# liruiw/GA-DDPG

Measured on AMD Instinct MI355X. Metric: DDPG grad-steps/sec (B=256, N=1024 pts), higher is better.
Workload: dtype f32 (3xbf16-split products, f32 accumulate)

## Files before the change

ga-ddpg_amd/csrc/gemm.hip:

```cpp
#include "gemm_common.hpp"
#include <mutex>
#include <string.h>

GemmOptions g_opt;

bool split_on(int family) {
    return !g_opt.deterministic && (g_opt.mfma_split == GAD_SPLIT_ALL || (g_opt.mfma_split & family) != 0);
}

bool fits_i32_bytes(long long rows, int pitch_a, int pitch_b, int pitch_c, int pitch_d) {
    int p = pitch_a > pitch_b ? pitch_a : pitch_b;
    p = p > pitch_c ? p : pitch_c;
    p = p > pitch_d ? p : pitch_d;
    return rows * (long long)p * 4 <= (1ll << 31);
}

int gad_deterministic() { return g_opt.deterministic; }

namespace {
struct DetBuf { void* stream; int kind; void* p; size_t bytes; };
std::mutex g_det_mu;
DetBuf g_det_bufs[64];
int g_det_n = 0;
}

void* gad_det_scratch(void* stream, int kind, size_t bytes) {
    std::lock_guard<std::mutex> lk(g_det_mu);
    DetBuf* b = nullptr;
    for (int i = 0; i < g_det_n; ++i)
        if (g_det_bufs[i].stream == stream && g_det_bufs[i].kind == kind) b = &g_det_bufs[i];
    if (!b) {
        if (g_det_n == 64) { gad_set_error("deterministic mode: more than 64 scratch buffers (streams x kinds)"); return nullptr; }
        b = &g_det_bufs[g_det_n++];
        b->stream = stream; b->kind = kind; b->p = nullptr; b->bytes = 0;
    }
    if (b->bytes >= bytes) return b->p;
    if (b->p) {
        if (hipStreamSynchronize((hipStream_t)stream) != hipSuccess || hipFree(b->p) != hipSuccess) {
            gad_set_error("deterministic mode: releasing a scratch buffer failed");
            b->p = nullptr; b->bytes = 0;
            return nullptr;
        }
        b->p = nullptr; b->bytes = 0;
    }
    size_t want = bytes + bytes / 4;
    want = (want + 4095) & ~(size_t)4095;
    if (hipMalloc(&b->p, want) != hipSuccess) {
        (void)hipGetLastError();
        gad_set_error("deterministic mode: cannot allocate %zu bytes of scratch", want);
        b->p = nullptr;
        return nullptr;
    }
    b->bytes = want;
    return b->p;
}

static void det_scratch_release() {
    std::lock_guard<std::mutex> lk(g_det_mu);
    for (int i = 0; i < g_det_n; ++i)
        if (g_det_bufs[i].p) (void)hipFree(g_det_bufs[i].p);
    g_det_n = 0;
}

template <typename T>
__global__ __launch_bounds__(256) void ordered_reduce_kernel(const T* __restrict__ slots, long long slot_stride, int nslots,
                                                             long long ncols, double* __restrict__ out) {
    const long long c = (long long)blockIdx.x * 256 + threadIdx.x;
    if (c >= ncols) return;
    const T* p = slots + c;
    double s = 0.0;
    for (int i = 0; i < nslots; ++i) s += (double)p[(size_t)i * slot_stride];
    atomic_add_f64(out + c, s);
}

template <typename T>
__global__ __launch_bounds__(256) void ordered_reduce_tree_kernel(const T* __restrict__ slots, long long slot_stride, int nslots,
                                                                  double* __restrict__ out) {
    __shared__ double red[256];
    const long long c = blockIdx.x;
    double s = 0.0;
    for (int i = threadIdx.x; i < nslots; i += 256) s += (double)slots[(size_t)i * slot_stride + c];
    red[threadIdx.x] = s;
    __syncthreads();
    for (int w = 128; w > 0; w >>= 1) {
        if ((int)threadIdx.x < w) red[threadIdx.x] += red[threadIdx.x + w];
        __syncthreads();
    }
    if (threadIdx.x == 0) atomic_add_f64(out + c, red[0]);
}

template <typename T>
static int ordered_reduce_launch(const T* slots, long long slot_stride, int nslots, long long ncols, double* out, void* stream) {
    if (ncols <= 0 || nslots <= 0) return GAD_OK;
    if (ncols <= 4096 && nslots > 256)
        hipLaunchKernelGGL(ordered_reduce_tree_kernel<T>, dim3((unsigned)ncols), dim3(256), 0, (hipStream_t)stream, slots, slot_stride,
                           nslots, out);
    else
        hipLaunchKernelGGL(ordered_reduce_kernel<T>, dim3(gad_cdiv(ncols, 256)), dim3(256), 0, (hipStream_t)stream, slots, slot_stride,
                           nslots, ncols, out);
    GAD_CHECK_LAUNCH("ordered_reduce");
    return GAD_OK;
}
int gad_ordered_reduce(const float* slots, long long slot_stride, int nslots, long long ncols, double* out, void* stream) {
    return ordered_reduce_launch(slots, slot_stride, nslots, ncols, out, stream);
}
int gad_ordered_reduce(const double* slots, long long slot_stride, int nslots, long long ncols, double* out, void* stream) {
    return ordered_reduce_launch(slots, slot_stride, nslots, ncols, out, stream);
}

constexpr int ANY_LO = -2147483647 - 1, ANY_HI = 2147483647;
static const struct { const char* name; int GemmOptions::*member; int lo, hi, fallback; } k_options[] = {
    {"deterministic", &GemmOptions::deterministic, 0, 0, 1},
    {"mfma_split", &GemmOptions::mfma_split, ANY_LO, ANY_HI, 0},
    {"fwd_stream", &GemmOptions::fwd_stream, ANY_LO, ANY_HI, 0},
    {"fwd_wide", &GemmOptions::fwd_wide, ANY_LO, ANY_HI, 0},
    {"dx_wide", &GemmOptions::dx_wide, ANY_LO, ANY_HI, 0},
    {"dw_wide", &GemmOptions::dw_wide, ANY_LO, ANY_HI, 0},
    {"bwd_fused", &GemmOptions::bwd_fused, ANY_LO, ANY_HI, 0},
    {"bwd_wide", &GemmOptions::bwd_wide, ANY_LO, ANY_HI, 0},
    {"fwd_bn_prologue", &GemmOptions::fwd_bn_prologue, ANY_LO, ANY_HI, 0},
    {"fwd_skinny", &GemmOptions::fwd_skinny, ANY_LO, ANY_HI, 0},
    {"dx_skinny", &GemmOptions::dx_skinny, ANY_LO, ANY_HI, 0},
    {"dx_stream", &GemmOptions::dx_stream, ANY_LO, ANY_HI, 0},
    {"dw_skinny", &GemmOptions::dw_skinny, ANY_LO, ANY_HI, 0},
    {"dw_stream", &GemmOptions::dw_stream, ANY_LO, ANY_HI, 0},
    {"bwd_stream_wgs", &GemmOptions::bwd_stream_wgs, 1, DW_STREAM_SPLITS, DW_STREAM_SPLITS},
    {"fwd_stream_wgs", &GemmOptions::fwd_stream_wgs, 1, 2147483647, 256},
    {"fwd_stream_l1_wgs", &GemmOptions::fwd_stream_l1_wgs, 1, 2147483647, 256},
    {"dw_wide_wgs", &GemmOptions::dw_wide_wgs, 1, 2147483647, 256},
    {"bwd_wide_slab", &GemmOptions::bwd_wide_slab, 1, 2147483647, 4},
    {"skinny_nw", &GemmOptions::skinny_nw, 4, 4, SK_NW},
};

extern "C" int gad_set_option(const char* name, int value) {
    GAD_REQUIRE(name, GAD_ERR_NULL, "set_option: null name");
    for (const auto& o : k_options) {
        if (strcmp(name, o.name)) continue;
        const int v = (value >= o.lo && value <= o.hi) ? value : o.fallback;
        if (o.member == &GemmOptions::deterministic && !v && g_opt.deterministic) det_scratch_release();
        g_opt.*o.member = v;
        return GAD_OK;
    }
    int found = 0;
    gad_geometry_set_option(name, value, &found);
    if (found) return GAD_OK;
    GAD_REQUIRE(false, GAD_ERR_SHAPE, "set_option: unknown option '%s'", name);
    return GAD_OK;
}

int check_input(const gad_gemm_fwd_args& a, const char* who) {
    if (a.mode == 2) {
        GAD_REQUIRE(!g_opt.deterministic, GAD_ERR_UNSUPPORTED, "%s: mode 2 (recomputed 64-channel input) has no deterministic form "
                    "(option \"deterministic\"): store the 64-channel input instead", who);
        GAD_REQUIRE(a.src_xyz && a.row_pt && a.row_grp && a.feat && a.pre_W, GAD_ERR_NULL, "%s: recomputed input needs the gather inputs and pre_W", who);
        GAD_REQUIRE(a.act_c == 0 || a.action, GAD_ERR_NULL, "%s: action", who);
        GAD_REQUIRE(fwd_streamable(a), GAD_ERR_SHAPE, "%s: mode 2 (recomputed 64-channel input) is a streaming-kernel form: SA1 rows, "
                    "Kp = c_in = n_out = 64, rows >= 32768, pre_Kp 8 / 16, scale / shift, relu", who);
        return GAD_OK;
    }
    if (a.mode == 0) {
        GAD_REQUIRE(a.zin && a.c_in % 4 == 0 && a.c_in >= 4 && a.c_in <= VMAX && a.zin_pitch % 4 == 0, GAD_ERR_SHAPE,
                    "%s: ACT input needs 4 <= c_in <= %d, c_in and pitch multiples of 4", who, VMAX);
        for (int i = 0; i < a.n_groups; ++i)
            GAD_REQUIRE(a.zin_off[i] % 4 == 0, GAD_ERR_SHAPE, "%s: zin_off must be a multiple of 4", who);
    } else {
        GAD_REQUIRE(a.src_xyz && a.row_pt && a.row_grp && a.feat, GAD_ERR_NULL, "%s: gather inputs", who);
        GAD_REQUIRE(a.feat_c % 4 == 0 && a.feat_c >= 4, GAD_ERR_SHAPE, "%s: feat_c must be a positive multiple of 4", who);
        GAD_REQUIRE(a.act_c == 0 || a.action, GAD_ERR_NULL, "%s: action", who);
    }
    return GAD_OK;
}

int coef_fallback(gad_dz_src& dz, void* stream) {
    if (!dz.bn_dbeta) return GAD_OK;
    GAD_REQUIRE(dz.coefP && dz.coefQ && dz.coefS && dz.scale && dz.bn_dgamma && dz.bn_mean && dz.bn_istd, GAD_ERR_NULL,
                "BatchNorm-backward block on a route without a prologue needs coefP / Q / S scratch");
    if (int e = gad_bn_bwd_coef(dz.bn_dbeta, dz.bn_dgamma, dz.bn_stride, dz.scale, dz.bn_mean, dz.bn_istd, dz.c, dz.bn_count,
                                const_cast<float*>(dz.coefP), const_cast<float*>(dz.coefQ), const_cast<float*>(dz.coefS), dz.gacc_gamma,
                                dz.gacc_beta, stream)) return e;
    dz.bn_dbeta = nullptr; dz.bn_dgamma = nullptr; dz.gacc_gamma = nullptr; dz.gacc_beta = nullptr;
    return GAD_OK;
}

double* det_stat_slots(int gx, int ncol, void* stream) {
    const size_t n = 2 * (size_t)gx * ncol;
    double* p = static_cast<double*>(gad_det_scratch(stream, GAD_DET_SLOTS, n * sizeof(double)));
    if (p && hipMemsetAsync(p, 0, n * sizeof(double), (hipStream_t)stream) != hipSuccess) {
        gad_set_error("deterministic mode: clearing the statistic slots failed");
        return nullptr;
    }
    return p;
}
int det_stat_reduce(const double* slots, int gx, int ncol, double* sum, double* sq, void* stream) {
    if (int e = gad_ordered_reduce(slots, ncol, gx, ncol, sum, stream)) return e;
    return gad_ordered_reduce(slots + (size_t)gx * ncol, ncol, gx, ncol, sq, stream);
}
```

ga-ddpg_amd/csrc/gemm_common.hpp:

```cpp
#pragma once
#include "common.hpp"
#include <type_traits>

typedef float f32x16 __attribute__((ext_vector_type(16)));

__device__ __forceinline__ __attribute__((used)) int gad_cdiv_dev(int a, int b) { return (a + b - 1) / b; }

#ifndef GAD_STREAM_STORE_AUX
#define GAD_STREAM_STORE_AUX 0
#endif

#define KT 32

__device__ __forceinline__ float4 f4zero() { return make_float4(0.f, 0.f, 0.f, 0.f); }
__device__ __forceinline__ float4 f4sel(bool c, float4 a, float4 b) {
    return make_float4(c ? a.x : b.x, c ? a.y : b.y, c ? a.z : b.z, c ? a.w : b.w);
}
__device__ __forceinline__ float4 ldg4(const float* p) { return *reinterpret_cast<const float4*>(p); }

typedef unsigned gad_u32x4 __attribute__((ext_vector_type(4)));
__device__ __forceinline__ float4 buf_ld4(__amdgpu_buffer_rsrc_t r, int vo, int so) {
    const gad_u32x4 u = __builtin_amdgcn_raw_buffer_load_b128(r, vo, so, 0);
    return make_float4(__uint_as_float(u.x), __uint_as_float(u.y), __uint_as_float(u.z), __uint_as_float(u.w));
}
__device__ __forceinline__ float buf_ld(__amdgpu_buffer_rsrc_t r, int vo, int so) {
    return __uint_as_float(__builtin_amdgcn_raw_buffer_load_b32(r, vo, so, 0));
}
#define GAD_BUF_MAX ((int)0x80000000u)
__device__ __forceinline__ int gad_nbytes(int rows, int row_bytes) { return (int)((unsigned)rows * (unsigned)row_bytes); }

#define VMAX 1024

struct XSrc {
    int mode;
    const float* zin; int zin_pitch; int c_in;
    const float* scale; const float* shift; int relu;
    const float* extra; int ones_col;
    const float* src_xyz; const float* ctr_xyz; const float* feat; int feat_c;
    const float* action; int act_c; int gps;
    const int32_t* row_pt; const int32_t* row_grp;
    int affine;
    const float* pre_W; int pre_Kp;
    gad_bn_fin bn;
};

static XSrc make_xsrc(const gad_gemm_fwd_args& a) {
    XSrc x;
    x.mode = a.mode; x.zin = a.zin; x.zin_pitch = a.zin_pitch; x.c_in = a.c_in;
    x.scale = a.scale; x.shift = a.shift; x.relu = a.relu; x.extra = a.extra; x.ones_col = a.ones_col;
    x.src_xyz = a.src_xyz; x.ctr_xyz = a.ctr_xyz; x.feat = a.feat; x.feat_c = a.feat_c;
    x.action = a.action; x.act_c = a.act_c; x.gps = a.grp_per_sample > 0 ? a.grp_per_sample : 1;
    x.row_pt = a.row_pt; x.row_grp = a.row_grp;
    x.affine = (x.scale && x.shift) ? 1 : 0;
    x.pre_W = a.pre_W; x.pre_Kp = a.pre_Kp;
    x.bn.stat_sum = a.in_stat_sum; x.bn.stat_sq = a.in_stat_sq; x.bn.stat_stride = a.in_stat_stride; x.bn.count = a.in_count;
    x.bn.gamma = a.in_gamma; x.bn.beta = a.in_beta; x.bn.eps = a.in_eps; x.bn.momentum = a.in_momentum;
    x.bn.running_mean = a.in_running_mean; x.bn.running_var = a.in_running_var;
    x.bn.scale = const_cast<float*>(a.scale); x.bn.shift = const_cast<float*>(a.shift); x.bn.mean = a.in_mean; x.bn.istd = a.in_istd;
    return x;
}

template <int NT>
__device__ __forceinline__ void stage_affine(float* sv, float* tv, const XSrc& x, int off, int n) {
    for (int i = threadIdx.x; i < n; i += NT) { sv[i] = x.scale[off + i]; tv[i] = x.shift[off + i]; }
}

#ifdef GAD_X_PHASES
#define GAD_PH_STAMP(t) t = (long long)__builtin_readcyclecounter()
#else
#define GAD_PH_STAMP(t)
#endif
#ifdef GAD_W_PHASES
#define GAD_WPH_DECL long long wph_[6] = {0, 0, 0, 0, 0, 0}; wph_[0] = (long long)wall_clock64()
#define GAD_WPH(i) do { if (wph_[i] == 0) wph_[i] = (long long)wall_clock64(); } while (0)
#define GAD_WPH_STORE(ts)                                                                                                     \
    do {                                                                                                                      \
        unsigned long long* q_ = reinterpret_cast<unsigned long long*>(reinterpret_cast<size_t>(ts) & ~(size_t)7);            \
        const unsigned blk_ = blockIdx.x + gridDim.x * blockIdx.y;                                                            \
        if (q_ && threadIdx.x == 0 && blk_ < 4096) {                                                                          \
            auto c_ = [&](int i) { const long long d_ = wph_[i] ? wph_[i] - wph_[0] : 0; return (unsigned long long)(d_ > 65535 ? 65535 : d_); }; \
            q_[2 * (8192 + blk_)] = (unsigned long long)wph_[0];                                                              \
            q_[2 * (8192 + blk_) + 1] = c_(1) | (c_(2) << 16) | (c_(3) << 32) | (c_(4) << 48);                                \
            q_[2 * (12288 + blk_)] = c_(5);                                                                                    \
        }                                                                                                                     \
    } while (0)
#define GAD_WKL_DECL long long wkl_[4] = {0, 0, 0, 0}; long long wkt_ = 0, wkp_ = 0
#define GAD_WKL(i)                                                                   \
    do {                                                                             \
        wkt_ = (long long)__builtin_readcyclecounter();                              \
        if (i > 0) wkl_[i] += wkt_ - wkp_;                                           \
        wkp_ = wkt_;                                                                 \
    } while (0)
#define GAD_WKL_STORE(ts)                                                                                                     \
    do {                                                                                                                      \
        unsigned long long* q_ = reinterpret_cast<unsigned long long*>(reinterpret_cast<size_t>(ts) & ~(size_t)7);            \
        const unsigned blk_ = blockIdx.x + gridDim.x * blockIdx.y;                                                            \
        if (q_ && (threadIdx.x & 63) == 0 && blk_ < 512) {                                                                    \
            const unsigned e_ = 4096 + 8 * blk_ + (threadIdx.x >> 6);                                                         \
            q_[2 * e_] = ((unsigned long long)wkl_[1] << 32) | (unsigned long long)(wkl_[2] & 0xffffffffu);                   \
            q_[2 * e_ + 1] = (unsigned long long)wkl_[3];                                                                     \
        }                                                                                                                     \
    } while (0)
#else
#define GAD_WPH_DECL
#define GAD_WPH(i)
#define GAD_WPH_STORE(ts)
#define GAD_WKL_DECL
#define GAD_WKL(i)
#define GAD_WKL_STORE(ts)
#endif
struct XRaw { float4 a; float4 s; };

__device__ __forceinline__ int x_bulk(const XSrc& x) { return x.mode == 0 ? x.c_in : x.feat_c; }

template <int XM>
__device__ __forceinline__ XRaw x_raw(const XSrc& x, int r, bool valid, int zoff, int c, bool tail, int pt, int grp_pre = -1) {
    XRaw o;
    o.s = f4zero();
    const int rr = valid ? r : 0;
    if (XM == 0) {
        const int cc = c < x.c_in ? c : x.c_in - 4;
        o.a = ldg4(x.zin + (size_t)rr * x.zin_pitch + zoff + cc);
        if (tail) {
            float e = 0.f;
            if (x.extra) e = x.extra[rr];
            o.s.x = (c + 0 == x.c_in && x.extra) ? e : (c + 0 == x.ones_col ? 1.f : 0.f);
            o.s.y = (c + 1 == x.c_in && x.extra) ? e : (c + 1 == x.ones_col ? 1.f : 0.f);
            o.s.z = (c + 2 == x.c_in && x.extra) ? e : (c + 2 == x.ones_col ? 1.f : 0.f);
            o.s.w = (c + 3 == x.c_in && x.extra) ? e : (c + 3 == x.ones_col ? 1.f : 0.f);
        }
    } else {
        const int cc = c < x.feat_c ? c : x.feat_c - 4;
        o.a = ldg4(x.feat + (size_t)pt * x.feat_c + cc);
        if (tail) {
            const int grp = grp_pre >= 0 ? grp_pre : x.row_grp[rr];
            const float* p = x.src_xyz + (size_t)pt * 3;
            float q0 = p[0], q1 = p[1], q2 = p[2];
            if (x.ctr_xyz) {
                const float* cp = x.ctr_xyz + (size_t)grp * 3;
                q0 = __fsub_rn(q0, cp[0]); q1 = __fsub_rn(q1, cp[1]); q2 = __fsub_rn(q2, cp[2]);
            }
            float a[4] = {0.f, 0.f, 0.f, 0.f};
            const int t0 = c - x.feat_c;
            if (x.action) {
                const float* ap = x.action + (size_t)(grp / x.gps) * x.act_c;
#pragma unroll
                for (int j = 0; j < 4; ++j) {
                    const int ai = t0 + j - 3;
                    const int aic = ai < 0 ? 0 : (ai >= x.act_c ? x.act_c - 1 : ai);
                    const float av = ap[aic];
                    a[j] = (ai >= 0 && ai < x.act_c) ? av : 0.f;
                }
            }
            float* spv = &o.s.x;
#pragma unroll
            for (int j = 0; j < 4; ++j) {
                const int t = t0 + j;
                spv[j] = t == 0 ? q0 : (t == 1 ? q1 : (t == 2 ? q2 : a[j]));
            }
        }
    }
    return o;
}

template <int XM>
__device__ __forceinline__ float4 x_finish(const XSrc& x, const XRaw& raw, bool valid, int c, const float* sv,
                                           const float* tv) {
    const int bulk = XM == 0 ? x.c_in : x.feat_c;
    const bool inside = c < bulk;
    float4 v = raw.a;
    if (XM == 0) {
        const int cc = inside ? c : x.c_in - 4;
        if (x.affine) {
            const float4 s = *reinterpret_cast<const float4*>(sv + cc), t = *reinterpret_cast<const float4*>(tv + cc);
            v.x = fmaf(v.x, s.x, t.x); v.y = fmaf(v.y, s.y, t.y); v.z = fmaf(v.z, s.z, t.z); v.w = fmaf(v.w, s.w, t.w);
        }
        if (x.relu) { v.x = fmaxf(v.x, 0.f); v.y = fmaxf(v.y, 0.f); v.z = fmaxf(v.z, 0.f); v.w = fmaxf(v.w, 0.f); }
    }
    return f4sel(valid, f4sel(inside, v, raw.s), f4zero());
}

__device__ __forceinline__ void stage_vec(float* dst, const float* src, int off, int n, float fill) {
    for (int i = threadIdx.x; i < n; i += 256) dst[i] = src ? src[off + i] : fill;
}

struct DzSrc {
    const float* z; int z_pitch; const float* scale; const float* shift; int relu;
    const float* P; const float* Q; const float* S; const float* row_w;
    int gmode; const float* G; int g_pitch; const int32_t* argmax; const float* dout;
    const int32_t* row_grp; int c;
    int coef;
    int premasked;
    gad_bn_bwd bw;
};

static DzSrc make_dzsrc(const gad_dz_src& d) {
    DzSrc s;
    s.z = d.z; s.z_pitch = d.z_pitch; s.scale = d.scale; s.shift = d.shift; s.relu = d.relu;
    s.P = d.coefP; s.Q = d.coefQ; s.S = d.coefS; s.row_w = d.row_w;
    s.gmode = d.gmode; s.G = d.G; s.g_pitch = d.g_pitch; s.argmax = d.argmax; s.dout = d.dout;
    s.row_grp = d.row_grp; s.c = d.c;
    s.premasked = d.premasked;
    s.bw.dbeta = d.bn_dbeta; s.bw.dgamma = d.bn_dgamma; s.bw.stat_stride = d.bn_stride; s.bw.count = d.bn_count;
    s.bw.mean = d.bn_mean; s.bw.istd = d.bn_istd; s.bw.gacc_gamma = d.gacc_gamma; s.bw.gacc_beta = d.gacc_beta;
    s.bw.accumulate = (d.gacc_gamma || d.gacc_beta) ? 1 : 0;
    s.coef = (d.coefP != nullptr || d.bn_dbeta != nullptr) ? 1 : 0;
    return s;
}

__device__ __forceinline__ void dz_coef(const DzSrc& d, int ch, float& P, float& Q, float& S, bool writer = false) {
    if (d.bw.dbeta) gad_bn_bwd_channel(d.bw, d.scale, ch, writer, P, Q, S);
    else if (d.P) { P = d.P[ch]; Q = d.Q[ch]; S = d.S[ch]; }
    else { P = 1.f; Q = 0.f; S = 0.f; }
}
__device__ __forceinline__ bool first_workgroup() { return blockIdx.x == 0 && blockIdx.y == 0 && blockIdx.z == 0; }

struct DzRaw { float4 z; float4 g; int4 a; };

__device__ __forceinline__ float4 dz_scalar4(const DzSrc& d, int r, bool valid, int off, int n, int nmax) {
    float v[4];
#pragma unroll
    for (int j = 0; j < 4; ++j) {
        const int nn = n + j;
        const bool ok = valid && nn < nmax;
        const int rr = ok ? r : 0;
        const int ch = off + (ok ? nn : 0);
        float z = 0.f;
        if (d.z) z = d.z[(size_t)rr * d.z_pitch + ch];
        float g;
        if (d.gmode == 0) {
            g = d.G[(size_t)rr * d.g_pitch + ch];
        } else {
            const int grp = d.row_grp[rr];
            g = d.argmax[(size_t)grp * d.c + ch] == r ? d.dout[(size_t)grp * d.c + ch] : 0.f;
        }
        if (d.relu && !d.premasked) {
            const float y = d.scale ? fmaf(z, d.scale[ch], d.shift[ch]) : z;
            g = y > 0.f ? g : 0.f;
        }
        if (d.P) {
            const float w = d.row_w ? d.row_w[rr] : 1.f;
            g = d.P[ch] * g - w * fmaf(d.S[ch], z, d.Q[ch]);
        }
        v[j] = ok ? g : 0.f;
    }
    return make_float4(v[0], v[1], v[2], v[3]);
}

template <bool VEC>
__device__ __forceinline__ DzRaw dz_raw(const DzSrc& d, int r, bool valid, int off, int n, int nmax, int grp) {
    DzRaw o;
    o.z = f4zero(); o.a = make_int4(0, 0, 0, 0);
    if (!VEC) { o.g = dz_scalar4(d, r, valid, off, n, nmax); return o; }
    const int rr = valid ? r : 0;
    const int ch = off + (n < nmax ? n : 0);
    if (d.z) o.z = ldg4(d.z + (size_t)rr * d.z_pitch + ch);
    if (d.gmode == 0) {
        o.g = ldg4(d.G + (size_t)rr * d.g_pitch + ch);
    } else {
        o.a = *reinterpret_cast<const int4*>(d.argmax + (size_t)grp * d.c + ch);
        o.g = ldg4(d.dout + (size_t)grp * d.c + ch);
    }
    return o;
}

template <bool VEC, int VM = VMAX>
__device__ __forceinline__ float4 dz_finish(const DzSrc& d, const DzRaw& raw, int r, bool valid, int n, int nmax, float w,
                                            const float* vec) {
    if (!VEC) return raw.g;
    const bool inside = n < nmax;
    const int nn = inside ? n : 0;
    float4 g = raw.g;
    const float4 z = raw.z;
    if (d.gmode != 0) {
        g.x = raw.a.x == r ? g.x : 0.f; g.y = raw.a.y == r ? g.y : 0.f;
        g.z = raw.a.z == r ? g.z : 0.f; g.w = raw.a.w == r ? g.w : 0.f;
    }
    if (d.relu && !d.premasked) {
        float4 y = z;
        if (d.scale) {
            const float4 s = *reinterpret_cast<const float4*>(vec + nn), t = *reinterpret_cast<const float4*>(vec + VM + nn);
            y.x = fmaf(z.x, s.x, t.x); y.y = fmaf(z.y, s.y, t.y); y.z = fmaf(z.z, s.z, t.z); y.w = fmaf(z.w, s.w, t.w);
        }
        g.x = y.x > 0.f ? g.x : 0.f; g.y = y.y > 0.f ? g.y : 0.f;
        g.z = y.z > 0.f ? g.z : 0.f; g.w = y.w > 0.f ? g.w : 0.f;
    }
    if (d.coef) {
        const float4 P = *reinterpret_cast<const float4*>(vec + 2 * VM + nn);
        const float4 Q = *reinterpret_cast<const float4*>(vec + 3 * VM + nn);
        const float4 S = *reinterpret_cast<const float4*>(vec + 4 * VM + nn);
        g.x = P.x * g.x - w * fmaf(S.x, z.x, Q.x); g.y = P.y * g.y - w * fmaf(S.y, z.y, Q.y);
        g.z = P.z * g.z - w * fmaf(S.z, z.z, Q.z); g.w = P.w * g.w - w * fmaf(S.w, z.w, Q.w);
    }
    return f4sel(valid && inside, g, f4zero());
}

template <int VM = VMAX>
__device__ __forceinline__ void stage_dz_vecs(float* vec, const DzSrc& d, int off, int n) {
    if (!d.premasked) {
        stage_vec(vec, d.scale, off, n, 1.f);
        stage_vec(vec + VM, d.shift, off, n, 0.f);
    }
    for (int i = threadIdx.x; i < n; i += 256) {
        float P, Q, S;
        dz_coef(d, off + i, P, Q, S, first_workgroup());
        vec[2 * VM + i] = P; vec[3 * VM + i] = Q; vec[4 * VM + i] = S;
    }
}

static bool dz_vectorizable(const gad_dz_src& d, const int32_t* off, const int32_t* n_out, int ng) {
    bool ok = (d.z == nullptr || d.z_pitch % 4 == 0) && (d.gmode != 0 || d.g_pitch % 4 == 0) && (d.gmode == 0 || d.c % 4 == 0);
    for (int i = 0; i < ng; ++i) ok = ok && off[i] % 4 == 0 && n_out[i] % 4 == 0 && n_out[i] <= VMAX;
    return ok;
}

template <int DIM> struct PitchT { static constexpr int v = DIM + 1; };
template <int DIM> struct PitchD { static constexpr int v = DIM + 4; };

template <int DIM> __device__ __forceinline__ void unit_T(int u, int& i, int& kk) { i = u >> 3; kk = (u & 7) << 2; }
template <int DIM> __device__ __forceinline__ void unit_D(int u, int& kk, int& i) { kk = u / (DIM / 4); i = (u % (DIM / 4)) << 2; }

template <int DIM> __device__ __forceinline__ void store_T(float* t, int i, int kk, float4 v) {
    constexpr int P = PitchT<DIM>::v;
    t[(kk + 0) * P + i] = v.x; t[(kk + 1) * P + i] = v.y; t[(kk + 2) * P + i] = v.z; t[(kk + 3) * P + i] = v.w;
}
template <int DIM> __device__ __forceinline__ void store_D(float* t, int kk, int i, float4 v) {
    constexpr int P = PitchD<DIM>::v;
    *reinterpret_cast<float4*>(t + kk * P + i) = v;
}

template <int TM, int TN, int PA, int PB>
__device__ __forceinline__ void mfma_ktile(const float* __restrict__ As, const float* __restrict__ Bs, int am0,
                                           int bn0, int lane, f32x16 (&acc)[TM][TN]) {
    const int l31 = lane & 31, half = lane >> 5;
    constexpr int CH = 4, NCH = KT / 2 / CH;
    const float* ap = As + half * PA + am0 + l31;
    const float* bp = Bs + half * PB + bn0 + l31;
    float a[2][CH][TM], b[2][CH][TN];
    auto fetch = [&](int c, int buf) {
#pragma unroll
        for (int s = 0; s < CH; ++s) {
#pragma unroll
            for (int tm = 0; tm < TM; ++tm) a[buf][s][tm] = ap[(2 * (c * CH + s)) * PA + tm * 32];
#pragma unroll
            for (int tn = 0; tn < TN; ++tn) b[buf][s][tn] = bp[(2 * (c * CH + s)) * PB + tn * 32];
        }
    };
    fetch(0, 0);
#pragma unroll
    for (int c = 0; c < NCH; ++c) {
        if (c + 1 < NCH) fetch(c + 1, (c + 1) & 1);
        __builtin_amdgcn_sched_barrier(0);
#pragma unroll
        for (int s = 0; s < CH; ++s)
#pragma unroll
            for (int tm = 0; tm < TM; ++tm)
#pragma unroll
                for (int tn = 0; tn < TN; ++tn)
                    acc[tm][tn] = __builtin_amdgcn_mfma_f32_32x32x2f32(a[c & 1][s][tm], b[c & 1][s][tn], acc[tm][tn], 0, 0, 0);
    }
}

__device__ __forceinline__ int acc_row(int v, int half) { return (v & 3) + 8 * (v >> 2) + 4 * half; }

struct PoolEpi {
    unsigned long long* key;
    const int32_t* row_grp;
    const float* gamma;
    int C;
};

__device__ __forceinline__ unsigned pool_ord(float f) {
    const unsigned u = __float_as_uint(f);
    return u ^ ((unsigned)((int)u >> 31) | 0x80000000u);
}

__device__ __forceinline__ void pool_put(unsigned long long* keycol, int g, int C, float v, int row, bool partial) {
    const unsigned long long k = ((unsigned long long)pool_ord(v) << 32) | (unsigned long long)(0xffffffffu - (unsigned)row);
    if (partial) atomicMax(keycol + (size_t)g * C, k);
    else keycol[(size_t)g * C] = k;
}

struct PoolRun { int g; int part; float v; int row; };

template <int NC>
__device__ __forceinline__ void pool_rows(const float* zt, int pitch, int cstride, int i, int e, int row_base, const float (&sgn)[NC],
                                          float (&best)[NC], int (&brow)[NC]) {
    int r = i;
    for (; r + 2 <= e; r += 2) {
        float z0[NC], z1[NC];
#pragma unroll
        for (int c = 0; c < NC; ++c) { z0[c] = zt[r * pitch + c * cstride] * sgn[c]; z1[c] = zt[(r + 1) * pitch + c * cstride] * sgn[c]; }
#pragma unroll
        for (int c = 0; c < NC; ++c) {
            bool t = z0[c] > best[c]; best[c] = t ? z0[c] : best[c]; brow[c] = t ? row_base + r : brow[c];
            t = z1[c] > best[c]; best[c] = t ? z1[c] : best[c]; brow[c] = t ? row_base + r + 1 : brow[c];
        }
    }
    if (r < e) {
#pragma unroll
        for (int c = 0; c < NC; ++c) {
            const float z0 = zt[r * pitch + c * cstride] * sgn[c];
            const bool t = z0 > best[c]; best[c] = t ? z0 : best[c]; brow[c] = t ? row_base + r : brow[c];
        }
    }
}

__device__ __forceinline__ void pool_scan32(const float* zt, int pitch, int gl, int row_base, float sgn, PoolRun& c,
                                            unsigned long long* keycol, int C) {
    const int lane = threadIdx.x & 63;
    const int prev = __shfl_up(gl, 1, 64);
    const bool st = lane == 0 ? gl != c.g : gl != prev;
    const unsigned m = (unsigned)__ballot(st);
    int i = 0;
    while (i < 32) {
        if ((m >> i) & 1u) {
            if (c.g >= 0) pool_put(keycol, c.g, C, c.v, c.row, c.part != 0);
            c.g = __builtin_amdgcn_readlane(gl, i); c.part = 0; c.v = -INFINITY; c.row = row_base + i;
        }
        const unsigned rest = i < 31 ? m >> (i + 1) : 0u;
        const int e = rest ? i + 1 + __builtin_ctz(rest) : 32;
        if (c.g >= 0) {
            const float sg1[1] = {sgn};
            float bv[1] = {c.v};
            int br[1] = {c.row};
            pool_rows<1>(zt, pitch, 0, i, e, row_base, sg1, bv, br);
            c.v = bv[0]; c.row = br[0];
        }
        i = e;
    }
}

template <int NC>
__device__ __forceinline__ void pool_tile64(const float* zt, int pitch, int cstride, int gl, int row0, int n_live,
                                            const float (&sgn)[NC], int wave, int nw, int g_before, int g_after,
                                            unsigned long long* keycol, int C) {
    const int lane = threadIdx.x & 63;
    const int prev = __shfl_up(gl, 1, 64);
    const bool st = (lane == 0 || gl != prev) && lane < n_live;
    unsigned long long m = __ballot(st);
    int k = 0;
    while (m) {
        const int i = __builtin_ctzll(m);
        m &= m - 1;
        const int e = m ? __builtin_ctzll(m) : n_live;
        if ((k++ % nw) != wave) continue;
        const int g = __builtin_amdgcn_readlane(gl, i);
        float best[NC];
        int brow[NC];
#pragma unroll
        for (int c = 0; c < NC; ++c) { best[c] = -INFINITY; brow[c] = row0 + i; }
        pool_rows<NC>(zt, pitch, cstride, i, e, row0, sgn, best, brow);
        const bool partial = (i == 0 && g == g_before) || (e == n_live && g == g_after);
#pragma unroll
        for (int c = 0; c < NC; ++c) pool_put(keycol + c * cstride, g, C, best[c], brow[c], partial);
    }
}

struct Groups {
    int n; int aoff[GAD_MAX_GROUPS]; int woff[GAD_MAX_GROUPS]; int ooff[GAD_MAX_GROUPS]; int nout[GAD_MAX_GROUPS];
};

template <int WM, int WN, int TN, bool STORE = false>
__device__ __forceinline__ void block_column_atomics(float* red, const float (&c0)[TN], const float (&c1)[TN], int lane,
                                                     int wm, int wn, int col0, int col_limit, double* out0,
                                                     double* out1) {
    constexpr int BN = WN * TN * 32;
    __syncthreads();
#pragma unroll
    for (int tn = 0; tn < TN; ++tn) {
        const float s0 = c0[tn] + __shfl_xor(c0[tn], 32, 64);
        const float s1 = c1[tn] + __shfl_xor(c1[tn], 32, 64);
        if (lane < 32) {
            const int cl = wn * TN * 32 + tn * 32 + lane;
            red[wm * BN + cl] = s0;
            red[(WM + wm) * BN + cl] = s1;
        }
    }
    __syncthreads();
    const int tid = threadIdx.x;
    if (tid < BN && col0 + tid < col_limit) {
        float s0 = 0.f, s1 = 0.f;
#pragma unroll
        for (int w = 0; w < WM; ++w) { s0 += red[w * BN + tid]; s1 += red[(WM + w) * BN + tid]; }
        if (STORE) {
            out0[col0 + tid] = (double)s0;
            out1[col0 + tid] = (double)s1;
        } else {
            atomic_add_f64(out0 + col0 + tid, (double)s0);
            atomic_add_f64(out1 + col0 + tid, (double)s1);
        }
    }
}

typedef float f32x2 __attribute__((ext_vector_type(2)));

typedef __bf16 gad_bf16x8 __attribute__((ext_vector_type(8)));
__device__ __forceinline__ unsigned gad_cvt_pk_bf16(float lo, float hi) {
    unsigned r;
    __asm__("v_cvt_pk_bf16_f32 %0, %1, %2" : "=v"(r) : "v"(lo), "v"(hi));
    return r;
}
__device__ __forceinline__ void gad_split2(float a, float b, unsigned& H, unsigned& M, unsigned& L) {
    H = gad_cvt_pk_bf16(a, b);
    const f32x2 r = f32x2{a, b} - f32x2{__uint_as_float(H << 16), __uint_as_float(H & 0xffff0000u)};
    M = gad_cvt_pk_bf16(r.x, r.y);
    const f32x2 q = r - f32x2{__uint_as_float(M << 16), __uint_as_float(M & 0xffff0000u)};
    L = gad_cvt_pk_bf16(q.x, q.y);
}
__device__ __forceinline__ gad_bf16x8 gad_as_bf16x8(gad_u32x4 u) { return *reinterpret_cast<gad_bf16x8*>(&u); }

namespace spw {
constexpr int APL = 64 * 64, BPL = 128 * 64, STAGE = 3 * (APL + BPL);
struct BRegs { gad_u32x4 r[2][3]; };
__device__ __forceinline__ void load_b(BRegs& b, __amdgpu_buffer_rsrc_t rs, const int (&vb)[2], int plane_bytes, int kt) {
#pragma unroll
    for (int u = 0; u < 2; ++u)
#pragma unroll
        for (int p = 0; p < 3; ++p) b.r[u][p] = __builtin_amdgcn_raw_buffer_load_b128(rs, vb[u], p * plane_bytes + kt * 64, 0);
}
__device__ __forceinline__ void store_b(unsigned char* stage, const BRegs& b, int tid) {
    const int row = tid >> 2;
    unsigned char* q = stage + 3 * APL + row * 64 + ((((tid & 3) ^ ((row >> 2) & 3))) << 4);
#pragma unroll
    for (int u = 0; u < 2; ++u)
#pragma unroll
        for (int p = 0; p < 3; ++p) *reinterpret_cast<gad_u32x4*>(q + p * BPL + u * (64 * 64)) = b.r[u][p];
}
__device__ __forceinline__ void store_a4(unsigned char* stage, int row, int tid, float4 v, unsigned sg) {
    unsigned h0, m0, l0, h1, m1, l1;
    gad_split2(__uint_as_float(__float_as_uint(v.x) ^ sg), __uint_as_float(__float_as_uint(v.y) ^ sg), h0, m0, l0);
    gad_split2(__uint_as_float(__float_as_uint(v.z) ^ sg), __uint_as_float(__float_as_uint(v.w) ^ sg), h1, m1, l1);
    unsigned char* q = stage + row * 64 + (((((tid & 7) >> 1) ^ ((row >> 2) & 3))) << 4) + ((tid & 1) << 3);
    *reinterpret_cast<uint2*>(q) = make_uint2(h0, h1);
    *reinterpret_cast<uint2*>(q + APL) = make_uint2(m0, m1);
    *reinterpret_cast<uint2*>(q + 2 * APL) = make_uint2(l0, l1);
}
__device__ __forceinline__ void ktile(const unsigned char* stage, int arow, int brow, int fo, f32x16 (&acc)[2], f32x16 (&an)[2]) {
#pragma unroll
    for (int s = 0; s < 2; ++s) {
        const int off = fo ^ (s << 5);
        const unsigned char* ap = stage + arow + off;
        const unsigned char* bp = stage + 3 * APL + brow + off;
        const gad_u32x4 AH = *reinterpret_cast<const gad_u32x4*>(ap), AM = *reinterpret_cast<const gad_u32x4*>(ap + APL);
        const gad_u32x4 AL = *reinterpret_cast<const gad_u32x4*>(ap + 2 * APL);
        gad_u32x4 BH[2], BM[2], BL[2];
#pragma unroll
        for (int t = 0; t < 2; ++t) {
            BH[t] = *reinterpret_cast<const gad_u32x4*>(bp + t * (32 * 64));
            BM[t] = *reinterpret_cast<const gad_u32x4*>(bp + BPL + t * (32 * 64));
            BL[t] = *reinterpret_cast<const gad_u32x4*>(bp + 2 * BPL + t * (32 * 64));
        }
#define GAD_SPW(A, B)                                                                                                          \
        _Pragma("unroll") for (int t = 0; t < 2; ++t) {                                                                        \
            if (s) an[t] = __builtin_amdgcn_mfma_f32_32x32x16_bf16(gad_as_bf16x8(A), gad_as_bf16x8(B[t]), an[t], 0, 0, 0);     \
            else acc[t] = __builtin_amdgcn_mfma_f32_32x32x16_bf16(gad_as_bf16x8(A), gad_as_bf16x8(B[t]), acc[t], 0, 0, 0);     \
        }
        GAD_SPW(AL, BH) GAD_SPW(AH, BL) GAD_SPW(AM, BM) GAD_SPW(AM, BH) GAD_SPW(AH, BM) GAD_SPW(AH, BH)
#undef GAD_SPW
    }
}
}

#define SK_NW 8
#define SK_CH 6
#define SK_SP 36
#define SK_KCAP (8 * SK_NW * SK_CH * SK_MAXCH)
#define SK_MAXCH 3
#define GAD_GX_CAP 2048
#define DW_STREAM_SPLITS 256

struct GemmOptions {
    int mfma_split = 0;
    int deterministic = 0;
    int fwd_wide = 1, dx_wide = 1, dw_wide = 1;
    int bwd_fused = 1;
    int fwd_bn_prologue = 1;
    int bwd_wide = 0;
    int bwd_wide_slab = 4;
    int dw_wide_wgs = 256;
    int skinny_nw = SK_NW;
    int fwd_skinny = 1, dx_skinny = 1, dx_stream = 1, dw_skinny = 1, dw_stream = 1, fwd_stream = 1;
    int bwd_stream_wgs = DW_STREAM_SPLITS;
    int fwd_stream_wgs = 256;
    int fwd_stream_l1_wgs = 256;
};
extern GemmOptions g_opt;
bool split_on(int family);

#define GAD_LAUNCH_SKINNY(kernel, grid, st, ...)                                                                               \
    do {                                                                                                                       \
        if (g_opt.skinny_nw == 4) hipLaunchKernelGGL(kernel<4>, grid, dim3(64 * 4), 0, st, __VA_ARGS__);                       \
        else hipLaunchKernelGGL(kernel<SK_NW>, grid, dim3(64 * SK_NW), 0, st, __VA_ARGS__);                                    \
    } while (0)

static Groups make_groups(int n, const int32_t* a, const int32_t* w, const int32_t* o, const int32_t* no) {
    Groups g;
    g.n = n;
    for (int i = 0; i < GAD_MAX_GROUPS; ++i) {
        g.aoff[i] = (i < n && a) ? a[i] : 0; g.woff[i] = (i < n && w) ? w[i] : 0;
        g.ooff[i] = (i < n && o) ? o[i] : 0; g.nout[i] = i < n ? no[i] : 0;
    }
    return g;
}

static int max_nout(const Groups& g) { int m = 0; for (int i = 0; i < g.n; ++i) m = g.nout[i] > m ? g.nout[i] : m; return m; }

struct DxEpi {
    int mode; float* gout; int gout_pitch; int k_valid;
    const float* zprev; int zprev_pitch; const float* ps; const float* pt; const float* pm; const float* pi;
    double* dbeta; double* dgamma; int stat_stride; int store_masked;
    float* dfeat; int feat_c; const int32_t* row_pt; const int32_t* row_grp; double* daction; int act_c; int gps;
};

static DxEpi make_dxepi(const gad_gemm_dx_args& a) {
    DxEpi e;
    e.mode = a.epilogue; e.gout = a.gout; e.gout_pitch = a.gout_pitch; e.k_valid = a.k_valid;
    e.zprev = a.zprev; e.zprev_pitch = a.zprev_pitch; e.ps = a.prev_scale; e.pt = a.prev_shift;
    e.pm = a.prev_mean; e.pi = a.prev_istd; e.dbeta = a.prev_dbeta; e.dgamma = a.prev_dgamma;
    e.stat_stride = a.stat_stride;
    e.store_masked = (a.store_masked && a.prev_dbeta) ? 1 : 0;
    e.dfeat = a.dfeat; e.feat_c = a.feat_c; e.row_pt = a.row_pt; e.row_grp = a.row_grp;
    e.daction = a.daction; e.act_c = a.act_c; e.gps = a.grp_per_sample > 0 ? a.grp_per_sample : 1;
    return e;
}

int check_input(const gad_gemm_fwd_args& a, const char* who);
int coef_fallback(gad_dz_src& dz, void* stream);
bool fits_i32_bytes(long long rows, int pitch_a, int pitch_b, int pitch_c, int pitch_d);
double* det_stat_slots(int gx, int ncol, void* stream);
int det_stat_reduce(const double* slots, int gx, int ncol, double* sum, double* sq, void* stream);
bool fwd_streamable(const gad_gemm_fwd_args& a);
bool dx_streamable(const gad_gemm_dx_args& a, bool vec);
int dx_stream_launch(const gad_gemm_dx_args* a, const DzSrc& d, const DxEpi& e, unsigned long long* ts, void* stream);
bool dw_streamable(const gad_gemm_dw_args& a, int k_used);
int dw_reduce_launch(const float* partial, const Groups& gr, int nmax, const int32_t* n_rows_dev, int rows, int splits, int Kp,
                     int k_used, double* gacc, int all_active, hipStream_t st);
```

ga-ddpg_amd/csrc/gemm_dx.hip:

```cpp
#include "gemm_common.hpp"

template <int WM, int WN, int TM, int TN, bool VEC, int VM, bool DET = false>
__global__ __launch_bounds__(256) __attribute__((amdgpu_waves_per_eu(4, 4))) void gemm_dx_kernel(DzSrc d, Groups gr, const int32_t* __restrict__ n_rows_dev,
                                                       int n_rows_static, const float* __restrict__ W, int Kp,
                                                       DxEpi e, unsigned long long* __restrict__ ts) {
    KTimer kt(ts);
    constexpr int BM = WM * TM * 32, BN = WN * TN * 32;
    constexpr int PA = PitchT<BM>::v, PB = PitchD<BN>::v;
    constexpr int UA = BM * 8 / 256, UB = BN * 8 / 256;
    constexpr int OFFB = (KT * PA + 3) & ~3;
    constexpr int TILE = OFFB + KT * PB;
    constexpr int SM = TILE + 3 * BM + (VEC ? 5 * VM : 4);
    static_assert(TILE >= 2 * WM * BN, "reduction scratch must fit in the tile LDS");
    __shared__ __attribute__((aligned(16))) float smem[SM];
    float* As = smem;
    float* Bs = smem + OFFB;
    int32_t* ptS = reinterpret_cast<int32_t*>(smem + TILE);
    int32_t* grS = ptS + BM;
    float* wS = reinterpret_cast<float*>(grS + BM);
    float* vec = wS + BM;

    const int tid = threadIdx.x, lane = tid & 63, wave = tid >> 6;
    const int wm = wave / WN, wn = wave % WN;
    const int g = blockIdx.z;
    const int doff = gr.aoff[g], n_out = gr.nout[g], goff = gr.ooff[g];
    const float* Wg = W + gr.woff[g];
    const int k0out = blockIdx.y * BN;
    if (k0out >= e.k_valid) return;
    const int n_rows = n_rows_dev ? min(*n_rows_dev, n_rows_static) : n_rows_static;
    if ((int)(blockIdx.x * BM) >= n_rows) return;
    const int nk = gad_cdiv_dev(n_out, KT);
    if (VEC) stage_dz_vecs<VM>(vec, d, doff, n_out);
    const bool need_grp = e.mode == 1 || d.gmode != 0;

    float cb[TN], cg[TN];
#pragma unroll
    for (int t = 0; t < TN; ++t) { cb[t] = 0.f; cg[t] = 0.f; }

    for (int row0 = blockIdx.x * BM; row0 < n_rows; row0 += gridDim.x * BM) {
        f32x16 acc[TM][TN];
#pragma unroll
        for (int a = 0; a < TM; ++a)
#pragma unroll
            for (int b = 0; b < TN; ++b)
#pragma unroll
                for (int v = 0; v < 16; ++v) acc[a][b][v] = 0.f;
        if (tid < BM) {
            const int r = row0 + tid;
            const bool ok = r < n_rows;
            wS[tid] = (ok && d.row_w) ? d.row_w[r] : 1.f;
            if (e.mode == 1) ptS[tid] = ok ? e.row_pt[r] : 0;
            if (need_grp) grS[tid] = ok ? (e.mode == 1 ? e.row_grp[r] : d.row_grp[r]) : 0;
        }
        __syncthreads();

        DzRaw ra[UA];
        float4 rb[UB];
        auto load_tile = [&](int kt) {
            const int nb = kt * KT;
#pragma unroll
            for (int it = 0; it < UA; ++it) {
                int i, kk; unit_T<BM>(it * 256 + tid, i, kk);
                const int r = row0 + i;
                ra[it] = dz_raw<VEC>(d, r, r < n_rows, doff, nb + kk, n_out, need_grp ? grS[i] : 0);
            }
#pragma unroll
            for (int it = 0; it < UB; ++it) {
                int kk, j; unit_D<BN>(it * 256 + tid, kk, j);
                const int n = nb + kk, k = k0out + j;
                const bool ok = n < n_out && k < Kp;
                rb[it] = ldg4(Wg + (size_t)(ok ? n : 0) * Kp + (ok ? k : 0));
            }
        };
        auto store_tile = [&](int kt) {
            const int nb = kt * KT;
#pragma unroll
            for (int it = 0; it < UA; ++it) {
                int i, kk; unit_T<BM>(it * 256 + tid, i, kk);
                const int r = row0 + i;
                store_T<BM>(As, i, kk, dz_finish<VEC, VM>(d, ra[it], r, r < n_rows, nb + kk, n_out, wS[i], vec));
            }
#pragma unroll
            for (int it = 0; it < UB; ++it) {
                int kk, j; unit_D<BN>(it * 256 + tid, kk, j);
                const bool ok = (nb + kk) < n_out && (k0out + j) < Kp;
                store_D<BN>(Bs, kk, j, f4sel(ok, rb[it], f4zero()));
            }
        };
        load_tile(0);
        for (int kt = 0; kt < nk; ++kt) {
            store_tile(kt);
            __syncthreads();
            if (kt + 1 < nk) load_tile(kt + 1);
            mfma_ktile<TM, TN, PA, PB>(As, Bs, wm * TM * 32, wn * TN * 32, lane, acc);
            __syncthreads();
        }
        const int l31 = lane & 31, half = lane >> 5;
#pragma unroll
        for (int tn = 0; tn < TN; ++tn) {
            const int k = k0out + wn * TN * 32 + tn * 32 + l31;
            const bool kok = k < e.k_valid;
            float sc = 0.f, sh = 0.f, mu = 0.f, is = 0.f;
            const bool stats = e.dbeta != nullptr && kok;
            if (stats) { sc = e.ps[goff + k]; sh = e.pt[goff + k]; mu = e.pm[goff + k]; is = e.pi[goff + k]; }
            float sb = 0.f, sg = 0.f;
            int run_smp = -1;
            double run_sum = 0.0;
#pragma unroll
            for (int tm = 0; tm < TM; ++tm)
#pragma unroll
                for (int v = 0; v < 16; ++v) {
                    const int il = wm * TM * 32 + tm * 32 + acc_row(v, half);
                    const int r = row0 + il;
                    if (r >= n_rows || !kok) continue;
                    const float gv = acc[tm][tn][v];
                    if (e.mode == 0) {
                        float outv = gv;
                        if (stats) {
                            const float zp = e.zprev[(size_t)r * e.zprev_pitch + goff + k];
                            if (fmaf(zp, sc, sh) > 0.f) { sb += gv; sg = fmaf(gv, (zp - mu) * is, sg); }
                            else if (e.store_masked) outv = 0.f;
                        }
                        e.gout[(size_t)r * e.gout_pitch + goff + k] = outv;
                    } else {
                        if (k < e.feat_c) {
                            if (e.dfeat) atomic_add_f32(e.dfeat + (size_t)ptS[il] * e.feat_c + k, gv);
                        } else if (k >= e.feat_c + 3 && k < e.feat_c + 3 + e.act_c) {
                            if (e.daction) {
                                const int smp = grS[il] / e.gps;
                                if (smp != run_smp) {
                                    if (run_smp >= 0) atomic_add_f64(e.daction + (size_t)run_smp * e.act_c + (k - e.feat_c - 3), run_sum);
                                    run_smp = smp; run_sum = 0.0;
                                }
                                run_sum += (double)gv;
                            }
                        }
                    }
                }
            if (run_smp >= 0) atomic_add_f64(e.daction + (size_t)run_smp * e.act_c + (k - e.feat_c - 3), run_sum);
            cb[tn] += sb; cg[tn] += sg;
        }
        __syncthreads();
    }
    if (e.dbeta) {
        const int rep = DET ? blockIdx.x : blockIdx.x % GAD_STAT_REPLICAS;
        block_column_atomics<WM, WN, TN, DET>(smem, cb, cg, lane, wm, wn, k0out, e.k_valid,
                                              e.dbeta + (size_t)rep * e.stat_stride + goff,
                                              e.dgamma + (size_t)rep * e.stat_stride + goff);
    }
}

template <int GM, int SC, bool SP = false>
__global__ __launch_bounds__(256, 2) void gemm_dx_wide_kernel(DzSrc d, const int32_t* __restrict__ n_rows_dev, int n_rows_static,
                                                              const float* __restrict__ W, int Kp, int n_out, DxEpi e,
                                                              const uint16_t* __restrict__ wsp, int wsp_plane,
                                                              unsigned long long* __restrict__ ts) {
    KTimer kt_(ts);
    constexpr int BM = 64, BN = 128, P = KT + 4, PB = BN + 4, STAGE = SP ? spw::STAGE / 4 : BM * P + KT * PB, VM = 512;
    __shared__ __attribute__((aligned(16))) float smem[2 * STAGE + 3 * VM + BM];
    __shared__ int32_t ptS[BM];
    float* vP = smem + 2 * STAGE;
    float* wS = vP + 3 * VM;
    int32_t* grS = reinterpret_cast<int32_t*>(wS);
    const int tid = threadIdx.x, lane = tid & 63;
    const int wave = __builtin_amdgcn_readfirstlane(tid >> 6);
    const int wm = wave >> 1, wn = wave & 1;
    const int l31 = lane & 31, half = lane >> 5;
    const int k0out = blockIdx.y * BN;
    const int n_rows = n_rows_dev ? min(*n_rows_dev, n_rows_static) : n_rows_static;
    if ((int)(blockIdx.x * BM) >= n_rows) return;
    const int nk = n_out / KT;
    const int gpitch = GM == 0 ? d.g_pitch : d.c;
    const __amdgpu_buffer_rsrc_t zr = __builtin_amdgcn_make_buffer_rsrc(const_cast<float*>(d.z), 0, GAD_BUF_MAX, 0x00020000);
    const __amdgpu_buffer_rsrc_t gr_ = __builtin_amdgcn_make_buffer_rsrc(const_cast<float*>(GM == 0 ? d.G : d.dout), 0, GAD_BUF_MAX, 0x00020000);
    const __amdgpu_buffer_rsrc_t ar = __builtin_amdgcn_make_buffer_rsrc(const_cast<int32_t*>(GM == 0 ? d.row_grp : d.argmax), 0, GAD_BUF_MAX, 0x00020000);
    const __amdgpu_buffer_rsrc_t wr = __builtin_amdgcn_make_buffer_rsrc(const_cast<float*>(W), 0, GAD_BUF_MAX, 0x00020000);
    const int zp_pitch4 = SC ? 0 : e.zprev_pitch * 4, go_pitch4 = SC ? 0 : e.gout_pitch * 4;
    const __amdgpu_buffer_rsrc_t pr = __builtin_amdgcn_make_buffer_rsrc(const_cast<float*>(SC ? W : e.zprev), 0, SC ? 0 : gad_nbytes(n_rows, zp_pitch4), 0x00020000);
    const __amdgpu_buffer_rsrc_t or_ = __builtin_amdgcn_make_buffer_rsrc(SC ? const_cast<float*>(W) : e.gout, 0, SC ? 0 : gad_nbytes(n_rows, go_pitch4), 0x00020000);
    const int c4 = (tid & 7) * 4, ur = tid >> 3;
    const int bk4 = (tid & 31) * 4, bn = tid >> 5;
    int vw[4];
#pragma unroll
    for (int u = 0; u < 4; ++u) vw[u] = ((bn + 8 * u) * Kp + k0out + bk4) * 4;
    const __amdgpu_buffer_rsrc_t ws_ = __builtin_amdgcn_make_buffer_rsrc(const_cast<uint16_t*>(SP ? wsp : reinterpret_cast<const uint16_t*>(W)), 0, GAD_BUF_MAX, 0x00020000);
    int vbs[2];
#pragma unroll
    for (int u = 0; u < 2; ++u) vbs[u] = ((k0out + (tid >> 2) + 64 * u) * n_out + (tid & 3) * 8) * 2;
    unsigned char* const smem_b = reinterpret_cast<unsigned char*>(smem);
    const int sp_fo = ((half ^ ((l31 >> 2) & 3)) << 4);
    for (int i = tid; i < n_out; i += 256) {
        float Pc, Qc, Sc;
        dz_coef(d, i, Pc, Qc, Sc, first_workgroup());
        vP[i] = Pc; vP[VM + i] = Qc; vP[2 * VM + i] = Sc;
    }
    (void)grS;
    float ps[2] = {0.f, 0.f}, pt[2] = {0.f, 0.f}, pm[2] = {0.f, 0.f}, pi[2] = {0.f, 0.f};
#pragma unroll
    for (int t = 0; t < 2; ++t) {
        const int k = k0out + wn * 64 + t * 32 + l31;
        if (!SC) { ps[t] = e.ps[k]; pt[t] = e.pt[k]; pm[t] = e.pm[k]; pi[t] = e.pi[k]; }
    }
    float cb[2] = {0.f, 0.f}, cg[2] = {0.f, 0.f};
    for (int row0 = blockIdx.x * BM; row0 < n_rows; row0 += gridDim.x * BM) {
        f32x16 acc[2];
        f32x16 an[2];
#pragma unroll
        for (int t = 0; t < 2; ++t)
#pragma unroll
            for (int v = 0; v < 16; ++v) { acc[t][v] = 0.f; if (SP) an[t][v] = 0.f; }
        int vz[2], vg[2];
        float wrow[2];
        bool live[2];
#pragma unroll
        for (int u = 0; u < 2; ++u) {
            const int r = row0 + ur + 32 * u;
            live[u] = r < n_rows;
            const int rr = live[u] ? r : max(n_rows - 1, 0);
            wrow[u] = d.row_w ? d.row_w[rr] : 1.f;
            vz[u] = (rr * d.z_pitch + c4) * 4;
            vg[u] = ((GM == 1 ? d.row_grp[rr] : rr) * gpitch + c4) * 4;
        }
        float4 rz[2], rg[2], rb[SP ? 1 : 4];
        gad_u32x4 ra[2];
        spw::BRegs rbs;
        auto load_regs = [&](int kt) {
#pragma unroll
            for (int u = 0; u < 2; ++u) {
                rz[u] = buf_ld4(zr, vz[u], kt * (KT * 4));
                rg[u] = buf_ld4(gr_, vg[u], kt * (KT * 4));
                if (GM == 1) ra[u] = __builtin_amdgcn_raw_buffer_load_b128(ar, vg[u], kt * (KT * 4), 0);
            }
            if (SP) { spw::load_b(rbs, ws_, vbs, wsp_plane * 2, kt); return; }
#pragma unroll
            for (int u = 0; u < (SP ? 1 : 4); ++u) rb[u] = buf_ld4(wr, vw[u], kt * (KT * 4) * Kp);
        };
        auto write_lds = [&](int kt) {
            float* As = smem + (kt & 1) * STAGE;
            float* Bs = As + BM * P;
            const int nb = kt * KT + c4;
            const float4 P4 = *reinterpret_cast<const float4*>(vP + nb), Q4 = *reinterpret_cast<const float4*>(vP + VM + nb);
            const float4 S4 = *reinterpret_cast<const float4*>(vP + 2 * VM + nb);
#pragma unroll
            for (int u = 0; u < 2; ++u) {
                float4 g = rg[u];
                const float4 z = rz[u];
                if (GM == 1) {
                    const unsigned r = row0 + ur + 32 * u;
                    g.x = ra[u].x == r ? g.x : 0.f; g.y = ra[u].y == r ? g.y : 0.f;
                    g.z = ra[u].z == r ? g.z : 0.f; g.w = ra[u].w == r ? g.w : 0.f;
                }
                const float w = wrow[u];
                float4 v;
                v.x = P4.x * g.x - w * fmaf(S4.x, z.x, Q4.x); v.y = P4.y * g.y - w * fmaf(S4.y, z.y, Q4.y);
                v.z = P4.z * g.z - w * fmaf(S4.z, z.z, Q4.z); v.w = P4.w * g.w - w * fmaf(S4.w, z.w, Q4.w);
                if (!live[u]) v = f4zero();
                if (SP) spw::store_a4(smem_b + (kt & 1) * spw::STAGE, ur + 32 * u, tid, v, (ur & 1) ? 0x80000000u : 0u);
                else *reinterpret_cast<float4*>(As + (ur + 32 * u) * P + c4) = v;
            }
            if (SP) { spw::store_b(smem_b + (kt & 1) * spw::STAGE, rbs, tid); return; }
#pragma unroll
            for (int u = 0; u < (SP ? 1 : 4); ++u)
                *reinterpret_cast<float4*>(Bs + (bn + 8 * u) * PB + bk4) = rb[u];
        };
        load_regs(0);
        __syncthreads();
        if (SC && tid < BM) ptS[tid] = e.row_pt[min(row0 + tid, max(n_rows - 1, 0))];
        write_lds(0);
        if (nk > 1) load_regs(1);
        __syncthreads();
        for (int kt = 0; kt < nk; ++kt) {
            if (SP) {
                spw::ktile(smem_b + (kt & 1) * spw::STAGE, (wm * 32 + l31) * 64, (wn * 64 + l31) * 64, sp_fo, acc, an);
                if (kt + 1 < nk) write_lds(kt + 1);
                if (kt + 2 < nk) load_regs(kt + 2);
                __syncthreads();
                continue;
            }
            const float* As = smem + (kt & 1) * STAGE + (wm * 32 + l31) * P + 4 * half;
            const float* Bs = smem + (kt & 1) * STAGE + BM * P + (4 * half) * PB + wn * 64 + l31;
            float4 a4 = *reinterpret_cast<const float4*>(As);
            float4 b0 = make_float4(Bs[0], Bs[PB], Bs[2 * PB], Bs[3 * PB]);
            float4 b1 = make_float4(Bs[32], Bs[PB + 32], Bs[2 * PB + 32], Bs[3 * PB + 32]);
#pragma unroll
            for (int j = 0; j < KT / 8; ++j) {
                float4 an = a4, bn0 = b0, bn1 = b1;
                if (j + 1 < KT / 8) {
                    an = *reinterpret_cast<const float4*>(As + 8 * (j + 1));
                    const float* bq = Bs + 8 * (j + 1) * PB;
                    bn0 = make_float4(bq[0], bq[PB], bq[2 * PB], bq[3 * PB]);
                    bn1 = make_float4(bq[32], bq[PB + 32], bq[2 * PB + 32], bq[3 * PB + 32]);
                }
                acc[0] = __builtin_amdgcn_mfma_f32_32x32x2f32(a4.x, b0.x, acc[0], 0, 0, 0);
                acc[1] = __builtin_amdgcn_mfma_f32_32x32x2f32(a4.x, b1.x, acc[1], 0, 0, 0);
                acc[0] = __builtin_amdgcn_mfma_f32_32x32x2f32(a4.y, b0.y, acc[0], 0, 0, 0);
                acc[1] = __builtin_amdgcn_mfma_f32_32x32x2f32(a4.y, b1.y, acc[1], 0, 0, 0);
                acc[0] = __builtin_amdgcn_mfma_f32_32x32x2f32(a4.z, b0.z, acc[0], 0, 0, 0);
                acc[1] = __builtin_amdgcn_mfma_f32_32x32x2f32(a4.z, b1.z, acc[1], 0, 0, 0);
                acc[0] = __builtin_amdgcn_mfma_f32_32x32x2f32(a4.w, b0.w, acc[0], 0, 0, 0);
                acc[1] = __builtin_amdgcn_mfma_f32_32x32x2f32(a4.w, b1.w, acc[1], 0, 0, 0);
                a4 = an; b0 = bn0; b1 = bn1;
            }
            if (kt + 1 < nk) write_lds(kt + 1);
            if (kt + 2 < nk) load_regs(kt + 2);
            __syncthreads();
        }
        if (SP) {
#pragma unroll
            for (int t = 0; t < 2; ++t)
#pragma unroll
                for (int v = 0; v < 16; ++v) acc[t][v] = (v & 1) ? an[t][v] - acc[t][v] : acc[t][v] - an[t][v];
        }
        if (SC) {
#pragma unroll
            for (int t = 0; t < 2; ++t) {
                const int k = k0out + wn * 64 + t * 32 + l31;
#pragma unroll
                for (int v = 0; v < 16; ++v) {
                    const int il = wm * 32 + acc_row(v, half);
                    if (row0 + il < n_rows) atomic_add_f32(e.dfeat + (size_t)ptS[il] * e.feat_c + k, acc[t][v]);
                }
            }
            continue;
        }
        const int rb0 = row0 + wm * 32;
#pragma unroll
        for (int t = 0; t < 2; ++t) {
            const int kcol = k0out + wn * 64 + t * 32 + l31;
            const int vzp = (4 * half * e.zprev_pitch + kcol) * 4, vgo = (4 * half * e.gout_pitch + kcol) * 4;
            float zp[16];
#pragma unroll
            for (int v = 0; v < 16; ++v) zp[v] = buf_ld(pr, vzp, (rb0 + (v & 3) + 8 * (v >> 2)) * zp_pitch4);
            const float npm = -pm[t] * pi[t];
            float sb = 0.f, sg = 0.f;
#pragma unroll
            for (int v = 0; v < 16; ++v) {
                const float ga = fmaf(zp[v], ps[t], pt[t]) > 0.f ? acc[t][v] : 0.f;
                __builtin_amdgcn_raw_buffer_store_b32(__float_as_uint(ga), or_, vgo, (rb0 + (v & 3) + 8 * (v >> 2)) * go_pitch4, 0);
                sb += ga;
                sg = fmaf(ga, fmaf(zp[v], pi[t], npm), sg);
            }
            cb[t] += sb; cg[t] += sg;
        }
    }
    if (SC) return;
    const int rep = blockIdx.x % GAD_STAT_REPLICAS;
    block_column_atomics<2, 2, 2>(smem, cb, cg, lane, wm, wn, k0out, e.k_valid, e.dbeta + (size_t)rep * e.stat_stride,
                                  e.dgamma + (size_t)rep * e.stat_stride);
}

__global__ __launch_bounds__(256) void dx_action_stream_kernel(DzSrc d, const int32_t* __restrict__ n_rows_dev, int n_rows_static,
                                                               const float* __restrict__ W, int Kp, int c0, DxEpi e,
                                                               unsigned long long* __restrict__ ts) {
    KTimer kt(ts);
    const int tid = threadIdx.x, lane = tid & 63;
    const int n_rows = n_rows_dev ? min(*n_rows_dev, n_rows_static) : n_rows_static;
    const int n_waves = gridDim.x * 4;
    const int gw = blockIdx.x * 4 + (tid >> 6);
    int chunk = (n_rows + n_waves - 1) / n_waves;
    chunk = (chunk + 3) & ~3;
    const int r0 = gw * chunk, r1 = min(n_rows, r0 + chunk);
    if (r0 >= r1) return;
    const int sub = lane >> 4, c4 = (lane & 15) * 4;
    float4 P, Q, S;
    dz_coef(d, c4 + 0, P.x, Q.x, S.x); dz_coef(d, c4 + 1, P.y, Q.y, S.y);
    dz_coef(d, c4 + 2, P.z, Q.z, S.z); dz_coef(d, c4 + 3, P.w, Q.w, S.w);
    float4 wa[6];
#pragma unroll
    for (int a = 0; a < 6; ++a)
        wa[a] = make_float4(W[(size_t)(c4 + 0) * Kp + c0 + a], W[(size_t)(c4 + 1) * Kp + c0 + a], W[(size_t)(c4 + 2) * Kp + c0 + a],
                            W[(size_t)(c4 + 3) * Kp + c0 + a]);
    double run[6] = {0.0, 0.0, 0.0, 0.0, 0.0, 0.0};
    int cur = -1;
    auto flush = [&]() {
        if (cur >= 0 && lane == 0)
#pragma unroll
            for (int a = 0; a < 6; ++a) atomic_add_f64(e.daction + (size_t)cur * 6 + a, run[a]);
#pragma unroll
        for (int a = 0; a < 6; ++a) run[a] = 0.0;
    };
    for (int rb = r0; rb < r1; rb += 4) {
        const int r = rb + sub;
        const bool live = r < r1;
        const int rr = live ? r : r1 - 1;
        const float4 z = ldg4(d.z + (size_t)rr * d.z_pitch + c4);
        const float4 g = ldg4(d.G + (size_t)rr * d.g_pitch + c4);
        const float w = d.row_w ? d.row_w[rr] : 1.f;
        const int smp = e.row_grp[rr] / e.gps;
        float4 dz;
        dz.x = P.x * g.x - w * fmaf(S.x, z.x, Q.x); dz.y = P.y * g.y - w * fmaf(S.y, z.y, Q.y);
        dz.z = P.z * g.z - w * fmaf(S.z, z.z, Q.z); dz.w = P.w * g.w - w * fmaf(S.w, z.w, Q.w);
        float p[6];
#pragma unroll
        for (int a = 0; a < 6; ++a) {
            p[a] = fmaf(dz.x, wa[a].x, fmaf(dz.y, wa[a].y, fmaf(dz.z, wa[a].z, dz.w * wa[a].w)));
            p[a] = live ? p[a] : 0.f;
#pragma unroll
            for (int m = 8; m >= 1; m >>= 1) p[a] += __shfl_xor(p[a], m, 16);
        }
        const int s0 = __builtin_amdgcn_readlane(smp, 0), s1 = __builtin_amdgcn_readlane(smp, 16);
        const int s2 = __builtin_amdgcn_readlane(smp, 32), s3 = __builtin_amdgcn_readlane(smp, 48);
        if (s0 == s1 && s1 == s2 && s2 == s3) {
            if (s0 != cur) { flush(); cur = s0; }
#pragma unroll
            for (int a = 0; a < 6; ++a) {
                float t = p[a] + __shfl_xor(p[a], 16, 64);
                t += __shfl_xor(t, 32, 64);
                run[a] += (double)t;
            }
        } else {
            flush();
            cur = -1;
            if ((lane & 15) == 0 && live)
#pragma unroll
                for (int a = 0; a < 6; ++a) atomic_add_f64(e.daction + (size_t)smp * 6 + a, (double)p[a]);
        }
    }
    flush();
}

static bool dx_action_streamable(const gad_gemm_dx_args& a, bool vec) {
    if (g_opt.deterministic || !g_opt.dx_stream || !vec || a.n_groups != 1 || a.dz_off[0] != 0 || a.w_off[0] != 0) return false;
    if (a.epilogue != 1 || a.dfeat || !a.daction || a.act_c != 6 || !a.row_grp || a.n_rows < 32768 || a.n_out[0] != 64) return false;
    const gad_dz_src& d = a.dz;
    return d.gmode == 0 && d.G && d.z && d.z_pitch % 4 == 0 && d.g_pitch % 4 == 0 && d.premasked && d.coefP && d.coefQ && d.coefS &&
           a.feat_c + 3 + a.act_c <= a.Kp;
}

static bool dx_wideable(const gad_gemm_dx_args& a, bool vec) {
    if (g_opt.deterministic || !g_opt.dx_wide || !vec || a.n_groups != 1 || a.dz_off[0] != 0 || a.w_off[0] != 0 || a.gout_off[0] != 0) return false;
    if (a.n_rows < 2048 || a.k_valid % 128 != 0 || a.k_valid > a.Kp) return false;
    if (a.n_out[0] % 32 != 0 || a.n_out[0] < 32 || a.n_out[0] > 512) return false;
    if (a.epilogue == 1) {
        if (g_opt.dx_wide == 2 || !a.dfeat || a.daction || !a.row_pt || a.k_valid != a.feat_c || a.prev_dbeta) return false;
    } else if (!a.prev_dbeta || !a.store_masked || !(a.zprev && a.prev_scale && a.prev_shift && a.prev_mean && a.prev_istd && a.prev_dgamma)) return false;
    const gad_dz_src& d = a.dz;
    if (!d.z || d.z_pitch % 4 != 0 || !d.relu || !d.premasked || !(d.coefP && d.coefQ && d.coefS)) return false;
    if (!fits_i32_bytes(a.n_rows, d.z_pitch, d.gmode == 0 ? d.g_pitch : d.c, a.epilogue == 0 ? a.gout_pitch : 0, a.epilogue == 0 ? a.zprev_pitch : 0)) return false;
    return d.gmode == 0 ? (d.g_pitch % 4 == 0 && d.G) : (d.c % 4 == 0);
}

template <int NW>
__global__ __launch_bounds__(64 * NW) void gemm_dx_skinny_kernel(DzSrc d, Groups gr, int n_rows,
                                                                    const float* __restrict__ W, int Kp, DxEpi e, unsigned long long* __restrict__ ts) {
    KTimer kt(ts);
    __shared__ __attribute__((aligned(16))) float stZ[NW * 32 * SK_SP], stG[NW * 32 * SK_SP];
    float* const part = stZ;
    __shared__ __attribute__((aligned(16))) float vec[5 * VMAX];
    const int tid = threadIdx.x, lane = tid & 63;
    const int wave = __builtin_amdgcn_readfirstlane(tid >> 6);
    const int l31 = lane & 31, half = lane >> 5;
    const int g = blockIdx.z;
    const int doff = gr.aoff[g], n_out = gr.nout[g], goff = gr.ooff[g];
    const int k0 = blockIdx.x * 32, row0 = blockIdx.y * 32;
    for (int i = tid; i < n_out; i += 64 * NW) {
        vec[i] = d.scale ? d.scale[doff + i] : 1.f;
        vec[VMAX + i] = d.shift ? d.shift[doff + i] : 0.f;
        float P, Q, S;
        dz_coef(d, doff + i, P, Q, S, first_workgroup());
        vec[2 * VMAX + i] = P; vec[3 * VMAX + i] = Q; vec[4 * VMAX + i] = S;
    }
    __syncthreads();
    const int r = min(row0 + l31, max(n_rows - 1, 0));
    const int k = min(k0 + l31, Kp - 1);
    const float* Wg = W + gr.woff[g] + k;
    const float wrow = d.row_w ? d.row_w[r] : 1.f;
    const int nj = (n_out + 7) >> 3;
    const int per = (nj + NW - 1) / NW;
    const int j0 = wave * per, j1 = min(nj, j0 + per);

    f32x16 acc;
#pragma unroll
    for (int v = 0; v < 16; ++v) acc[v] = 0.f;
    float* const myZ = stZ + wave * (32 * SK_SP);
    float* const myG = stG + wave * (32 * SK_SP);
    const int rsub = lane >> 3, chunk = lane & 7;
    const float* pz[4];
    const float* pg[4];
#pragma unroll
    for (int i = 0; i < 4; ++i) {
        const size_t rr = (size_t)min(row0 + rsub + 8 * i, max(n_rows - 1, 0));
        pz[i] = d.z ? d.z + rr * d.z_pitch + doff + 4 * chunk : nullptr;
        pg[i] = d.G + rr * d.g_pitch + doff + 4 * chunk;
    }
    auto staged = [&](int jb) { return d.z != nullptr && jb + 4 <= j1 && 8 * (jb + 4) <= n_out; };
    float4 gz[4], gg[4], rb[2][4];
    auto load_blk = [&](int jb) {
#pragma unroll
        for (int i = 0; i < 4; ++i) { gz[i] = ldg4(pz[i] + 8 * jb); gg[i] = ldg4(pg[i] + 8 * jb); }
    };
    auto load_w = [&](int jb, auto bufc) {
        constexpr int B = decltype(bufc)::value;
#pragma unroll
        for (int u = 0; u < 4; ++u) {
            const int n = 8 * min(jb + u, nj - 1) + 4 * half;
            const int nc = n < n_out ? n : 0;
            const float* wp = Wg + (size_t)nc * Kp;
            rb[B][u] = make_float4(wp[0], wp[Kp], wp[2 * (size_t)Kp], wp[3 * (size_t)Kp]);
        }
    };
    auto block = [&](int jb, auto bufc) {
        constexpr int B = decltype(bufc)::value;
        const bool more = jb + 4 < j1;
        float4 rz[4], rg[4];
        const bool st = staged(jb);
        if (st) {
#pragma unroll
            for (int i = 0; i < 4; ++i) {
                *reinterpret_cast<float4*>(myZ + (rsub + 8 * i) * SK_SP + 4 * chunk) = gz[i];
                *reinterpret_cast<float4*>(myG + (rsub + 8 * i) * SK_SP + 4 * chunk) = gg[i];
            }
        } else {
#pragma unroll
            for (int u = 0; u < 4; ++u) {
                const int n = 8 * min(jb + u, nj - 1) + 4 * half;
                const int nc = n < n_out ? n : 0;
                rz[u] = d.z ? ldg4(d.z + (size_t)r * d.z_pitch + doff + nc) : f4zero();
                rg[u] = ldg4(d.G + (size_t)r * d.g_pitch + doff + nc);
            }
        }
        if (more) {
            if (staged(jb + 4)) load_blk(jb + 4);
            load_w(jb + 4, std::integral_constant<int, B ^ 1>{});
        }
        if (st) {
            __builtin_amdgcn_fence(__ATOMIC_RELEASE, "wavefront");
            __builtin_amdgcn_wave_barrier();
            __builtin_amdgcn_fence(__ATOMIC_ACQUIRE, "wavefront");
#pragma unroll
            for (int u = 0; u < 4; ++u) {
                rz[u] = *reinterpret_cast<const float4*>(myZ + l31 * SK_SP + 8 * u + 4 * half);
                rg[u] = *reinterpret_cast<const float4*>(myG + l31 * SK_SP + 8 * u + 4 * half);
            }
        }
        const int je = min(jb + 4, j1);
#pragma unroll
        for (int u = 0; u < 4; ++u) {
            if (jb + u < je) {
                DzRaw raw;
                raw.z = rz[u]; raw.g = rg[u]; raw.a = make_int4(0, 0, 0, 0);
                const float4 a4 = dz_finish<true>(d, raw, r, true, 8 * (jb + u) + 4 * half, n_out, wrow, vec);
                const float4 b4 = rb[B][u];
                acc = __builtin_amdgcn_mfma_f32_32x32x2f32(a4.x, b4.x, acc, 0, 0, 0);
                acc = __builtin_amdgcn_mfma_f32_32x32x2f32(a4.y, b4.y, acc, 0, 0, 0);
                acc = __builtin_amdgcn_mfma_f32_32x32x2f32(a4.z, b4.z, acc, 0, 0, 0);
                acc = __builtin_amdgcn_mfma_f32_32x32x2f32(a4.w, b4.w, acc, 0, 0, 0);
            }
        }
        if (st) {
            __builtin_amdgcn_fence(__ATOMIC_RELEASE, "wavefront");
            __builtin_amdgcn_wave_barrier();
        }
    };
    if (j0 < j1) {
        if (staged(j0)) load_blk(j0);
        load_w(j0, std::integral_constant<int, 0>{});
    }
    for (int jb = j0; jb < j1; jb += 8) {
        block(jb, std::integral_constant<int, 0>{});
        if (jb + 4 < j1) block(jb + 4, std::integral_constant<int, 1>{});
    }
#pragma unroll
    for (int v = 0; v < 16; ++v) part[wave * (32 * SK_SP) + v * 64 + lane] = acc[v];
    __syncthreads();
    if (wave != 0) return;
#pragma unroll
    for (int w = 1; w < NW; ++w)
#pragma unroll
        for (int v = 0; v < 16; ++v) acc[v] += part[w * (32 * SK_SP) + v * 64 + lane];
    const int kk = k0 + l31;
    const bool kok = kk < e.k_valid;
    const bool stats = e.dbeta != nullptr && kok;
    float sc = 0.f, sh = 0.f, mu = 0.f, is = 0.f;
    if (stats) { sc = e.ps[goff + kk]; sh = e.pt[goff + kk]; mu = e.pm[goff + kk]; is = e.pi[goff + kk]; }
    float sb = 0.f, sg = 0.f;
#pragma unroll
    for (int v = 0; v < 16; ++v) {
        const int rr = row0 + acc_row(v, half);
        if (rr >= n_rows || !kok) continue;
        const float gv = acc[v];
        float outv = gv;
        if (stats) {
            const float zp = e.zprev[(size_t)rr * e.zprev_pitch + goff + kk];
            if (fmaf(zp, sc, sh) > 0.f) { sb += gv; sg = fmaf(gv, (zp - mu) * is, sg); }
            else if (e.store_masked) outv = 0.f;
        }
        e.gout[(size_t)rr * e.gout_pitch + goff + kk] = outv;
    }
    if (e.dbeta) {
        sb += __shfl_xor(sb, 32, 64);
        sg += __shfl_xor(sg, 32, 64);
        if (lane < 32 && kok) {
            const int rep = blockIdx.y % GAD_STAT_REPLICAS;
            atomic_add_f64(e.dbeta + (size_t)rep * e.stat_stride + goff + kk, (double)sb);
            atomic_add_f64(e.dgamma + (size_t)rep * e.stat_stride + goff + kk, (double)sg);
        }
    }
}

__device__ __forceinline__ int rows_lower_bound(const int32_t* __restrict__ row_grp, int n, int key) {
    int lo = 0, hi = n;
    while (lo < hi) {
        const int mid = (lo + hi) >> 1;
        if (row_grp[mid] < key) lo = mid + 1; else hi = mid;
    }
    return lo;
}

__global__ __launch_bounds__(256) void scatter_group_bounds_kernel(const int32_t* __restrict__ row_pt, const int32_t* __restrict__ row_grp,
                                                                   const int32_t* __restrict__ n_rows_dev, int n_rows_static, int gcap,
                                                                   int32_t* __restrict__ gmin, int32_t* __restrict__ gmax) {
    const int n_rows = n_rows_dev ? min(*n_rows_dev, n_rows_static) : n_rows_static;
    if (n_rows <= 0) return;
    const int G = min(row_grp[n_rows - 1] + 1, gcap);
    const int g = blockIdx.x * 256 + threadIdx.x;
    if (g >= G) return;
    const int r0 = rows_lower_bound(row_grp, n_rows, g), r1 = rows_lower_bound(row_grp, n_rows, g + 1);
    int lo = INT_MAX, hi = -1;
    for (int r = r0; r < r1; ++r) { const int p = row_pt[r]; lo = min(lo, p); hi = max(hi, p); }
    gmin[g] = lo;
    gmax[g] = hi;
}
__global__ __launch_bounds__(256) void scatter_run_heads_kernel(const int32_t* __restrict__ row_grp, const int32_t* __restrict__ n_rows_dev,
                                                                int n_rows_static, int gcap, const int32_t* __restrict__ gmin,
                                                                const int32_t* __restrict__ gmax, int32_t* __restrict__ head) {
    __shared__ int32_t lmax[256], lmin[256];
    const int n_rows = n_rows_dev ? min(*n_rows_dev, n_rows_static) : n_rows_static;
    if (n_rows <= 0) return;
    const int Gall = row_grp[n_rows - 1] + 1;
    const int G = min(Gall, gcap);
    const int t = threadIdx.x, chunk = (G + 255) / 256;
    const int g0 = min(G, t * chunk), g1 = min(G, g0 + chunk);
    int mx = -1, mn = INT_MAX;
    for (int g = g0; g < g1; ++g) { mx = max(mx, gmax[g]); mn = min(mn, gmin[g]); }
    lmax[t] = mx; lmin[t] = mn;
    __syncthreads();
    if (t == 0) {
        int run = -1;
        for (int i = 0; i < 256; ++i) { const int v = lmax[i]; lmax[i] = run; run = max(run, v); }
        run = INT_MAX;
        for (int i = 255; i >= 0; --i) { const int v = lmin[i]; lmin[i] = run; run = min(run, v); }
    }
    __syncthreads();
    int sm = lmin[t];
    for (int g = g1 - 1; g >= g0; --g) { sm = min(sm, gmin[g]); head[g] = sm; }
    int pm = lmax[t];
    for (int g = g0; g < g1; ++g) {
        const int suf = head[g];
        head[g] = (g == 0 || pm < suf) && Gall <= gcap ? 1 : 0;
        pm = max(pm, gmax[g]);
    }
    if (Gall > gcap && t == 0) head[0] = 1;
}
__global__ __launch_bounds__(256) void scatter_runs_kernel(const float* __restrict__ rowbuf, int pitch, const int32_t* __restrict__ row_pt,
                                                           const int32_t* __restrict__ row_grp, const int32_t* __restrict__ n_rows_dev,
                                                           int n_rows_static, int gcap, const int32_t* __restrict__ head, int feat_c,
                                                           float* dfeat) {
    const int n_rows = n_rows_dev ? min(*n_rows_dev, n_rows_static) : n_rows_static;
    if (n_rows <= 0) return;
    const int Gall = row_grp[n_rows - 1] + 1;
    const int G = min(Gall, gcap);
    for (int g = blockIdx.x; g < G; g += gridDim.x) {
        if (!head[g]) continue;
        int ge = g + 1;
        while (ge < G && !head[ge]) ++ge;
        const int r0 = rows_lower_bound(row_grp, n_rows, g);
        const int r1 = ge < G ? rows_lower_bound(row_grp, n_rows, ge) : n_rows;
        for (int c = threadIdx.x; c < feat_c; c += 256)
            for (int r = r0; r < r1; ++r) {
                float* p = dfeat + (size_t)row_pt[r] * feat_c + c;
                *p = *p + rowbuf[(size_t)r * pitch + c];
            }
    }
}

__global__ __launch_bounds__(256) void gather_action_ordered_kernel(const float* __restrict__ rowbuf, int pitch,
                                                                    const int32_t* __restrict__ row_grp, const int32_t* __restrict__ n_rows_dev,
                                                                    int n_rows_static, int gps, int act_off, int act_c, double* daction) {
    const int n_rows = n_rows_dev ? min(*n_rows_dev, n_rows_static) : n_rows_static;
    if (n_rows <= 0) return;
    const int n_smp = row_grp[n_rows - 1] / gps + 1;
    for (int s = blockIdx.x; s < n_smp; s += gridDim.x) {
        const int r0 = rows_lower_bound(row_grp, n_rows, s * gps), r1 = rows_lower_bound(row_grp, n_rows, (s + 1) * gps);
        for (int j = threadIdx.x; j < act_c; j += 256) {
            double acc = 0.0;
            for (int r = r0; r < r1; ++r) acc += (double)rowbuf[(size_t)r * pitch + act_off + j];
            daction[(size_t)s * act_c + j] += acc;
        }
    }
}

template <int WM, int WN, int TM, int TN, bool V>
static int det_dx_launch(const gad_gemm_dx_args* a, const DzSrc& d, Groups gr, DxEpi e, int gx, int nmax_dx, unsigned long long* ts,
                         void* stream) {
    constexpr int BN = WN * TN * 32;
    hipStream_t st = (hipStream_t)stream;
    const int rows = a->n_rows, kv = a->k_valid;
    const dim3 grid(gx, gad_cdiv(kv, BN), gr.n);
    double* slots = nullptr;
    int ncol = 0;
    if (e.mode == 1) {
        GAD_REQUIRE(gr.n == 1 && !e.dbeta, GAD_ERR_UNSUPPORTED, "gemm_dx: the deterministic scatter epilogue takes one group and no "
                    "previous-layer statistics");
        GAD_REQUIRE(kv >= (a->daction && a->act_c > 0 ? a->feat_c + 3 + a->act_c : a->feat_c), GAD_ERR_SHAPE,
                    "gemm_dx: k_valid=%d does not cover the scattered columns", kv);
        float* rowbuf = static_cast<float*>(gad_det_scratch(stream, GAD_DET_ROWS, (size_t)rows * kv * sizeof(float)));
        if (!rowbuf) return GAD_ERR_LAUNCH;
        e.mode = 0; e.gout = rowbuf; e.gout_pitch = kv; e.store_masked = 0;
        gr.ooff[0] = 0;
    } else if (e.dbeta) {
        for (int i = 0; i < gr.n; ++i) ncol = gr.ooff[i] + kv > ncol ? gr.ooff[i] + kv : ncol;
        slots = det_stat_slots(gx, ncol, stream);
        if (!slots) return GAD_ERR_LAUNCH;
        e.dbeta = slots; e.dgamma = slots + (size_t)gx * ncol; e.stat_stride = ncol;
    }
    if (slots) {
        if (nmax_dx <= 512) hipLaunchKernelGGL((gemm_dx_kernel<WM, WN, TM, TN, V, 512, true>), grid, dim3(256), 0, st, d, gr, a->n_rows_dev, rows, a->W, a->Kp, e, ts);
        else                hipLaunchKernelGGL((gemm_dx_kernel<WM, WN, TM, TN, V, VMAX, true>), grid, dim3(256), 0, st, d, gr, a->n_rows_dev, rows, a->W, a->Kp, e, ts);
    } else {
        if (nmax_dx <= 512) hipLaunchKernelGGL((gemm_dx_kernel<WM, WN, TM, TN, V, 512>), grid, dim3(256), 0, st, d, gr, a->n_rows_dev, rows, a->W, a->Kp, e, ts);
        else                hipLaunchKernelGGL((gemm_dx_kernel<WM, WN, TM, TN, V, VMAX>), grid, dim3(256), 0, st, d, gr, a->n_rows_dev, rows, a->W, a->Kp, e, ts);
    }
    GAD_CHECK_LAUNCH("gemm_dx");
    if (slots) return det_stat_reduce(slots, gx, ncol, a->prev_dbeta, a->prev_dgamma, stream);
    if (a->epilogue == 1 && a->dfeat) {
        const int gcap = rows;
        int32_t* b = static_cast<int32_t*>(gad_det_scratch(stream, GAD_DET_RUNS, 3 * (size_t)gcap * sizeof(int32_t)));
        if (!b) return GAD_ERR_LAUNCH;
        int32_t *gmin = b, *gmax = b + gcap, *head = b + 2 * (size_t)gcap;
        hipLaunchKernelGGL(scatter_group_bounds_kernel, dim3(gad_cdiv(gcap, 256)), dim3(256), 0, st, a->row_pt, a->row_grp, a->n_rows_dev,
                           rows, gcap, gmin, gmax);
        hipLaunchKernelGGL(scatter_run_heads_kernel, dim3(1), dim3(256), 0, st, a->row_grp, a->n_rows_dev, rows, gcap, gmin, gmax, head);
        hipLaunchKernelGGL(scatter_runs_kernel, dim3(1024), dim3(256), 0, st, e.gout, kv, a->row_pt, a->row_grp, a->n_rows_dev, rows, gcap,
                           head, a->feat_c, a->dfeat);
        GAD_CHECK_LAUNCH("scatter_runs");
    }
    if (a->epilogue == 1 && a->daction && a->act_c > 0) {
        hipLaunchKernelGGL(gather_action_ordered_kernel, dim3(1024), dim3(256), 0, st, e.gout, kv, a->row_grp, a->n_rows_dev, rows, e.gps,
                           a->feat_c + 3, a->act_c, a->daction);
        GAD_CHECK_LAUNCH("gather_action_ordered");
    }
    return GAD_OK;
}

extern "C" int gad_gemm_dx(const gad_gemm_dx_args* a, void* stream) {
    unsigned long long* ts = gad_take_timing_slot(stream);
    const int rows_hint = gad_take_grid_rows();
    GAD_REQUIRE(a && a->W, GAD_ERR_NULL, "gemm_dx: null pointer");
    GAD_REQUIRE(a->n_groups >= 1 && a->n_groups <= GAD_MAX_GROUPS, GAD_ERR_SHAPE, "gemm_dx: n_groups");
    GAD_REQUIRE(a->Kp % 8 == 0, GAD_ERR_SHAPE, "gemm_dx: Kp must be a multiple of 8");
    GAD_REQUIRE(a->epilogue == 1 || a->gout, GAD_ERR_NULL, "gemm_dx: gout");
    GAD_REQUIRE(a->accumulate == 0 || a->n_groups == 1, GAD_ERR_UNSUPPORTED, "gemm_dx: accumulate=%d with %d groups is not implemented "
                "(groups store, they do not add: concatenate the groups into one, or give each its own gout_off)", a->accumulate, a->n_groups);
    GAD_REQUIRE(a->dz.gmode == 0 ? a->dz.G != nullptr : (a->dz.argmax && a->dz.dout && a->dz.row_grp), GAD_ERR_NULL,
                "gemm_dx: gradient source");
    if (a->n_rows <= 0) return GAD_OK;
    DzSrc d = make_dzsrc(a->dz);
    Groups gr = make_groups(a->n_groups, a->dz_off, a->w_off, a->gout_off, a->n_out);
    DxEpi e = make_dxepi(*a);
    GAD_REQUIRE(e.mode == 0 || (e.row_pt && e.row_grp), GAD_ERR_NULL, "gemm_dx: scatter epilogue needs row maps");
    GAD_REQUIRE(!e.dbeta || (e.zprev && e.ps && e.pt && e.pm && e.pi && e.dgamma), GAD_ERR_NULL, "gemm_dx: prev BN stats inputs");
    hipStream_t st = (hipStream_t)stream;
    const int rows = a->n_rows, kv = a->k_valid;
    const int grid_rows = (a->n_rows_dev && rows_hint > 0 && rows_hint < rows) ? rows_hint : rows;
    const bool vec = dz_vectorizable(a->dz, a->dz_off, a->n_out, a->n_groups);
    if (dx_streamable(*a, vec)) return dx_stream_launch(a, d, e, ts, stream);
    if (dx_action_streamable(*a, vec)) {
        if (a->dz.bn_dbeta) {
            gad_dz_src dz2 = a->dz;
            if (int e2 = coef_fallback(dz2, stream)) return e2;
            d = make_dzsrc(dz2);
        }
        hipLaunchKernelGGL(dx_action_stream_kernel, dim3(1024), dim3(256), 0, st, d, a->n_rows_dev, rows, a->W, a->Kp, a->feat_c + 3, e, ts);
        GAD_CHECK_LAUNCH("gemm_dx(action stream)");
        return GAD_OK;
    }
    if (dx_wideable(*a, vec)) {
        int gx = gad_cdiv(grid_rows, 64); if (gx > GAD_GX_CAP) gx = GAD_GX_CAP;
        const dim3 grid(gx, kv / 128);
        const bool sp = split_on(GAD_SPLIT_DX_WIDE) && a->W_split_t && a->W_split_t_pitch == a->n_out[0] && a->n_out[0] % 32 == 0 &&
                        a->W_split_t_plane >= kv * a->n_out[0];
#define LAUNCH_DXW(GM, SC, SP)                                                                                                 \
        hipLaunchKernelGGL((gemm_dx_wide_kernel<GM, SC, SP>), grid, dim3(256), 0, st, d, a->n_rows_dev, rows, a->W, a->Kp, a->n_out[0], e, \
                           a->W_split_t, a->W_split_t_plane, ts)
        if (a->epilogue == 1 && a->dz.gmode == 0) { if (sp) LAUNCH_DXW(0, 1, true); else LAUNCH_DXW(0, 1, false); }
        else if (a->dz.gmode == 0) { if (sp) LAUNCH_DXW(0, 0, true); else LAUNCH_DXW(0, 0, false); }
        else { if (sp) LAUNCH_DXW(1, 0, true); else LAUNCH_DXW(1, 0, false); }
#undef LAUNCH_DXW
        if (sp) GAD_CHECK_LAUNCH("gemm_dx(wide split)"); else GAD_CHECK_LAUNCH("gemm_dx(wide)");
        return GAD_OK;
    }
    int nmax_dx = 0;
    for (int i = 0; i < a->n_groups; ++i) nmax_dx = a->n_out[i] > nmax_dx ? a->n_out[i] : nmax_dx;
    if (!g_opt.deterministic && g_opt.dx_skinny && vec && e.mode == 0 && a->dz.gmode == 0 && !a->n_rows_dev && rows <= 1024 &&
        nmax_dx <= VMAX) {
        GAD_LAUNCH_SKINNY(gemm_dx_skinny_kernel, dim3(gad_cdiv(kv, 32), gad_cdiv(rows, 32), gr.n), st, d, gr, rows, a->W, a->Kp, e, ts);
        GAD_CHECK_LAUNCH("gemm_dx(skinny)");
        return GAD_OK;
    }
#define LAUNCH_DX2(WM, WN, TM, TN, V)                                                                    \
    do {                                                                                                 \
        constexpr int BM = WM * TM * 32, BN = WN * TN * 32;                                              \
        int gx = gad_cdiv(grid_rows, BM); if (gx > GAD_GX_CAP) gx = GAD_GX_CAP;                                      \
        if (g_opt.deterministic) {                                                                       \
            if (int e_ = det_dx_launch<WM, WN, TM, TN, V>(a, d, gr, e, gx, nmax_dx, ts, stream)) return e_; \
            return GAD_OK;                                                                               \
        }                                                                                                \
        if (nmax_dx <= 512)                                                                              \
            hipLaunchKernelGGL((gemm_dx_kernel<WM, WN, TM, TN, V, 512>), dim3(gx, gad_cdiv(kv, BN), gr.n), dim3(256), 0, \
                               st, d, gr, a->n_rows_dev, rows, a->W, a->Kp, e, ts);                          \
        else                                                                                             \
            hipLaunchKernelGGL((gemm_dx_kernel<WM, WN, TM, TN, V, VMAX>), dim3(gx, gad_cdiv(kv, BN), gr.n), dim3(256), 0, \
                               st, d, gr, a->n_rows_dev, rows, a->W, a->Kp, e, ts);                          \
    } while (0)
#define LAUNCH_DX(WM, WN, TM, TN) do { if (vec) LAUNCH_DX2(WM, WN, TM, TN, true); else LAUNCH_DX2(WM, WN, TM, TN, false); } while (0)
    if (kv <= 32) LAUNCH_DX(4, 1, 1, 1); else LAUNCH_DX(2, 2, 1, 1);
#undef LAUNCH_DX
#undef LAUNCH_DX2
    GAD_CHECK_LAUNCH("gemm_dx");
    return GAD_OK;
}
```

ga-ddpg_amd/csrc/gemm_fwd.hip:

```cpp
#include "gemm_common.hpp"

template <int WM, int WN, int TM, int TN, int XM, bool POOL, bool DET = false>
__global__ __launch_bounds__(256) void gemm_fwd_kernel(XSrc x, Groups gr, const int32_t* __restrict__ n_rows_dev,
                                                        int n_rows_static, const float* __restrict__ row_w,
                                                        const float* __restrict__ W, int Kp,
                                                        float* __restrict__ zout, int zout_pitch,
                                                        double* __restrict__ stat_sum,
                                                        double* __restrict__ stat_sq, int stat_stride, PoolEpi pe,
                                                        unsigned long long* __restrict__ ts) {
    KTimer kt(ts);
    constexpr int BM = WM * TM * 32, BN = WN * TN * 32;
    constexpr int PA = PitchT<BM>::v, PB = PitchT<BN>::v;
    constexpr int UA = BM * 8 / 256, UB = BN * 8 / 256;
    constexpr int TILE = KT * PA + KT * PB;
    constexpr int SM = ((TILE + 3) & ~3) + 2 * BM + 2 * VMAX;
    static_assert(TILE >= 2 * WM * BN, "reduction scratch must fit in the tile LDS");
    __shared__ __attribute__((aligned(16))) float smem[SM];
    float* As = smem;
    float* Bs = smem + KT * PA;
    float* wS = smem + ((TILE + 3) & ~3);
    int32_t* ptS = reinterpret_cast<int32_t*>(wS + BM);
    float* sv = wS + 2 * BM;
    float* tv = sv + VMAX;

    const int tid = threadIdx.x, lane = tid & 63, wave = tid >> 6;
    const int wm = wave / WN, wn = wave % WN;
    const int g = blockIdx.z;
    const int zoff = gr.aoff[g], n_out = gr.nout[g], ooff = gr.ooff[g];
    const float* Wg = W + gr.woff[g];
    const int n0 = blockIdx.y * BN;
    if (n0 >= n_out) return;
    const int n_rows = n_rows_dev ? min(*n_rows_dev, n_rows_static) : n_rows_static;
    if ((int)(blockIdx.x * BM) >= n_rows) return;
    const int nk = (Kp + KT - 1) / KT;
    const int bulk = XM == 0 ? x.c_in : x.feat_c;

    float csum[TN], csq[TN];
#pragma unroll
    for (int t = 0; t < TN; ++t) { csum[t] = 0.f; csq[t] = 0.f; }

    int row0 = blockIdx.x * BM;
    XRaw ra[UA];
    float4 rb[UB];
    auto load_tile = [&](int kt) {
        const int k0 = kt * KT;
        const bool tail = k0 + KT > bulk;
#pragma unroll
        for (int it = 0; it < UA; ++it) {
            int i, kk; unit_T<BM>(it * 256 + tid, i, kk);
            const int r = row0 + i;
            const bool ok = r < n_rows && (k0 + kk < Kp);
            ra[it] = x_raw<XM>(x, r, ok, zoff, k0 + kk, tail, XM == 1 ? ptS[i] : 0);
        }
#pragma unroll
        for (int it = 0; it < UB; ++it) {
            int j, kk; unit_T<BN>(it * 256 + tid, j, kk);
            const int n = n0 + j;
            const bool ok = n < n_out && (k0 + kk < Kp);
            rb[it] = ldg4(Wg + (size_t)(ok ? n : 0) * Kp + (ok ? k0 + kk : 0));
        }
    };
    auto store_tile = [&](int kt) {
        const int k0 = kt * KT;
#pragma unroll
        for (int it = 0; it < UA; ++it) {
            int i, kk; unit_T<BM>(it * 256 + tid, i, kk);
            const int r = row0 + i;
            const bool ok = r < n_rows && (k0 + kk < Kp);
            store_T<BM>(As, i, kk, x_finish<XM>(x, ra[it], ok, k0 + kk, sv, tv));
        }
#pragma unroll
        for (int it = 0; it < UB; ++it) {
            int j, kk; unit_T<BN>(it * 256 + tid, j, kk);
            const bool ok = (n0 + j) < n_out && (k0 + kk < Kp);
            store_T<BN>(Bs, j, kk, f4sel(ok, rb[it], f4zero()));
        }
    };
    bool preloaded = false;
    if (XM == 0) { load_tile(0); preloaded = true; }
    if (XM == 0 && x.affine) stage_affine<256>(sv, tv, x, zoff, x.c_in);
    for (; row0 < n_rows; row0 += gridDim.x * BM) {
        f32x16 acc[TM][TN];
#pragma unroll
        for (int a = 0; a < TM; ++a)
#pragma unroll
            for (int b = 0; b < TN; ++b)
#pragma unroll
                for (int v = 0; v < 16; ++v) acc[a][b][v] = 0.f;
        if (tid < BM) {
            const int r = row0 + tid;
            wS[tid] = r < n_rows ? (row_w ? row_w[r] : 1.f) : 0.f;
            if (XM == 1) ptS[tid] = r < n_rows ? x.row_pt[r] : 0;
        }
        int pgl = -1, pg_before = -1, pg_after = -1;
        float psgn = 1.f;
        if (POOL) {
            const int r = row0 + lane;
            pgl = r < n_rows ? pe.row_grp[r] : -1;
            pg_before = row0 > 0 ? pe.row_grp[row0 - 1] : -1;
            pg_after = row0 + BM < n_rows ? pe.row_grp[row0 + BM] : -1;
            psgn = pe.gamma[n0 + lane] < 0.f ? -1.f : 1.f;
        }
        __syncthreads();
        if (!preloaded) load_tile(0);
        preloaded = false;
        for (int kt = 0; kt < nk; ++kt) {
            store_tile(kt);
            __syncthreads();
            if (kt + 1 < nk) load_tile(kt + 1);
            mfma_ktile<TM, TN, PA, PB>(As, Bs, wm * TM * 32, wn * TN * 32, lane, acc);
            __syncthreads();
        }
        const int l31 = lane & 31, half = lane >> 5;
        if (POOL) {
            static_assert(!POOL || (BM == 64 && BN == 64 && TM == 1 && TN == 1 && TILE >= 64 * 65), "pooled epilogue: 64 x 64 tiles");
            float* zt = smem;
#pragma unroll
            for (int v = 0; v < 16; ++v) zt[(wm * 32 + acc_row(v, half)) * 65 + wn * 32 + l31] = acc[0][0][v];
            __syncthreads();
            {
                const float sg1[1] = {psgn};
                pool_tile64<1>(zt + lane, 65, 0, pgl, row0, min(64, n_rows - row0), sg1, __builtin_amdgcn_readfirstlane(wave), 4,
                               __builtin_amdgcn_readfirstlane(pg_before), __builtin_amdgcn_readfirstlane(pg_after),
                               pe.key + n0 + lane, pe.C);
            }
        }
#pragma unroll
        for (int tn = 0; tn < TN; ++tn) {
            const int n = n0 + wn * TN * 32 + tn * 32 + l31;
            float s1 = 0.f, s2 = 0.f;
#pragma unroll
            for (int tm = 0; tm < TM; ++tm)
#pragma unroll
                for (int v = 0; v < 16; ++v) {
                    const int il = wm * TM * 32 + tm * 32 + acc_row(v, half);
                    const int r = row0 + il;
                    const float zv = acc[tm][tn][v];
                    if (zout && r < n_rows && n < n_out) zout[(size_t)r * zout_pitch + ooff + n] = zv;
                    const float w = wS[il];
                    s1 = fmaf(w, zv, s1);
                    s2 = fmaf(w * zv, zv, s2);
                }
            csum[tn] += s1;
            csq[tn] += s2;
        }
        __syncthreads();
    }
    if (stat_sum) {
        const int rep = DET ? blockIdx.x : blockIdx.x % GAD_STAT_REPLICAS;
        block_column_atomics<WM, WN, TN, DET>(smem, csum, csq, lane, wm, wn, n0, n_out,
                                              stat_sum + (size_t)rep * stat_stride + ooff,
                                              stat_sq + (size_t)rep * stat_stride + ooff);
    }
}
template <int XM, bool POOL, bool SP = false>
__global__ __launch_bounds__(256, 2) void gemm_fwd_wide_kernel(XSrc x, const int32_t* __restrict__ n_rows_dev, int n_rows_static,
                                                               const float* __restrict__ row_w, const float* __restrict__ W,
                                                               int Kp, int n_out, float* __restrict__ zout, int zout_pitch,
                                                               double* __restrict__ stat_sum, double* __restrict__ stat_sq,
                                                               int stat_stride, PoolEpi pe, const uint16_t* __restrict__ wsp,
                                                               int wsp_pitch, int wsp_plane, unsigned long long* __restrict__ ts) {
    KTimer kt_(ts);
    GAD_WPH_DECL;
    GAD_WKL_DECL;
    constexpr int BM = 64, BN = 128, P = KT + 4, STAGE = SP ? spw::STAGE / 4 : (BM + BN) * P, VM = 512;
    static_assert(2 * STAGE >= 64 * 129, "the pooled epilogue's tile lives in the operand buffers");
    __shared__ __attribute__((aligned(16))) float smem[2 * STAGE + 2 * VM + BM + 4 * BM];
    float* sv = smem + 2 * STAGE;
    float* tv = sv + VM;
    float* wS = tv + VM;
    float* dxS = wS + BM;
    const int tid = threadIdx.x, lane = tid & 63;
    const int wave = __builtin_amdgcn_readfirstlane(tid >> 6);
    const int wm = wave >> 1, wn = wave & 1;
    const int l31 = lane & 31, half = lane >> 5;
    const int n0 = blockIdx.y * BN;
    const int n_rows = n_rows_dev ? min(*n_rows_dev, n_rows_static) : n_rows_static;
    if ((int)(blockIdx.x * BM) >= n_rows) return;
    const int nk = (XM == 0 ? Kp : x.feat_c) / KT;
    const int c4 = (tid & 7) * 4;
    const int ur = tid >> 3;
    const __amdgpu_buffer_rsrc_t ar_ = __builtin_amdgcn_make_buffer_rsrc(const_cast<float*>(XM == 0 ? x.zin : x.feat), 0, GAD_BUF_MAX, 0x00020000);
    const __amdgpu_buffer_rsrc_t wr_ = __builtin_amdgcn_make_buffer_rsrc(const_cast<float*>(W), 0, GAD_BUF_MAX, 0x00020000);
    const int zo_pitch4 = zout_pitch * 4;
    const __amdgpu_buffer_rsrc_t zo_ = __builtin_amdgcn_make_buffer_rsrc(zout ? zout : const_cast<float*>(W), 0, zout ? gad_nbytes(n_rows, zo_pitch4) : 0, 0x00020000);
    int vb[4];
#pragma unroll
    for (int u = 0; u < 4; ++u) vb[u] = ((n0 + ur + 32 * u) * Kp + c4) * 4;
    const __amdgpu_buffer_rsrc_t ws_ = __builtin_amdgcn_make_buffer_rsrc(const_cast<uint16_t*>(SP ? wsp : reinterpret_cast<const uint16_t*>(W)), 0, GAD_BUF_MAX, 0x00020000);
    int vbs[2];
#pragma unroll
    for (int u = 0; u < 2; ++u) vbs[u] = ((n0 + (tid >> 2) + 64 * u) * wsp_pitch + (tid & 3) * 8) * 2;
    unsigned char* const smem_b = reinterpret_cast<unsigned char*>(smem);
    const int sp_fo = ((half ^ ((l31 >> 2) & 3)) << 4);
    if (XM == 0) {
        if (x.bn.stat_sum) {
            const bool writer = blockIdx.x == 0 && blockIdx.y == 0;
            for (int i = tid; i < Kp; i += 256) {
                float sc, sh;
                gad_bn_fin_channel(x.bn, i, writer, sc, sh);
                sv[i] = sc; tv[i] = sh;
            }
        } else {
            stage_affine<256>(sv, tv, x, 0, Kp);
        }
    }

    float csum[2] = {0.f, 0.f}, csq[2] = {0.f, 0.f};
    for (int row0 = blockIdx.x * BM; row0 < n_rows; row0 += gridDim.x * BM) {
        f32x16 acc[2];
        f32x16 an[2];
#pragma unroll
        for (int t = 0; t < 2; ++t)
#pragma unroll
            for (int v = 0; v < 16; ++v) { acc[t][v] = 0.f; if (SP) an[t][v] = 0.f; }
        int pgl = -1, pg_before = -1, pg_after = -1;
        float psgn[2] = {1.f, 1.f};
        if (POOL) {
            const int r = row0 + lane;
            pgl = r < n_rows ? pe.row_grp[r] : -1;
            pg_before = row0 > 0 ? pe.row_grp[row0 - 1] : -1;
            pg_after = row0 + BM < n_rows ? pe.row_grp[row0 + BM] : -1;
            psgn[0] = pe.gamma[n0 + lane] < 0.f ? -1.f : 1.f;
            psgn[1] = pe.gamma[n0 + 64 + lane] < 0.f ? -1.f : 1.f;
        }
        const int ra0 = min(row0 + ur, max(n_rows - 1, 0)), ra1 = min(row0 + ur + 32, max(n_rows - 1, 0));
        const int va0 = ((XM == 0 ? ra0 * x.zin_pitch : x.row_pt[ra0] * x.feat_c) + c4) * 4;
        const int va1 = ((XM == 0 ? ra1 * x.zin_pitch : x.row_pt[ra1] * x.feat_c) + c4) * 4;
        float4 ra2[2][2], rb2[2][SP ? 1 : 4];
        spw::BRegs rbs[SP ? 2 : 1];
        auto load_regs = [&](int kt, auto setc) {
            constexpr int S = decltype(setc)::value;
            const int k0 = kt * (KT * 4);
            ra2[S][0] = buf_ld4(ar_, va0, k0); ra2[S][1] = buf_ld4(ar_, va1, k0);
            if (SP) { spw::load_b(rbs[SP ? S : 0], ws_, vbs, wsp_plane * 2, kt); return; }
#pragma unroll
            for (int u = 0; u < (SP ? 1 : 4); ++u) rb2[S][u] = buf_ld4(wr_, vb[u], k0);
        };
        auto write_lds = [&](int kt, auto setc) {
            constexpr int S = decltype(setc)::value;
            const float4* ra = ra2[S];
            const float4* rb = rb2[S];
            float* As = smem + (kt & 1) * STAGE;
            float* Bs = As + BM * P;
            float4 s4 = make_float4(1.f, 1.f, 1.f, 1.f), t4 = f4zero();
            if (XM == 0) {
                s4 = *reinterpret_cast<const float4*>(sv + kt * KT + c4);
                t4 = *reinterpret_cast<const float4*>(tv + kt * KT + c4);
            }
#pragma unroll
            for (int u = 0; u < 2; ++u) {
                float4 v = ra[u];
                if (XM == 0) {
                    v.x = fmaxf(fmaf(v.x, s4.x, t4.x), 0.f); v.y = fmaxf(fmaf(v.y, s4.y, t4.y), 0.f);
                    v.z = fmaxf(fmaf(v.z, s4.z, t4.z), 0.f); v.w = fmaxf(fmaf(v.w, s4.w, t4.w), 0.f);
                }
                if (SP) spw::store_a4(smem_b + (kt & 1) * spw::STAGE, ur + 32 * u, tid, v, (ur & 1) ? 0x80000000u : 0u);
                else *reinterpret_cast<float4*>(As + (ur + 32 * u) * P + c4) = v;
            }
            if (SP) { spw::store_b(smem_b + (kt & 1) * spw::STAGE, rbs[SP ? S : 0], tid); return; }
#pragma unroll
            for (int u = 0; u < (SP ? 1 : 4); ++u) *reinterpret_cast<float4*>(Bs + (ur + 32 * u) * P + c4) = rb[u];
        };
        const std::integral_constant<int, 0> S0;
        const std::integral_constant<int, 1> S1;
        load_regs(0, S0);
        if (nk > 1) load_regs(1, S1);
        __syncthreads();
        if (tid < BM) {
            const int r = row0 + tid;
            wS[tid] = r < n_rows ? (row_w ? row_w[r] : 1.f) : 0.f;
            if (XM == 1) {
                const int rr = min(r, max(n_rows - 1, 0));
                const float* p = x.src_xyz + (size_t)x.row_pt[rr] * 3;
                float q0 = p[0], q1 = p[1], q2 = p[2];
                if (x.ctr_xyz) {
                    const float* cp = x.ctr_xyz + (size_t)x.row_grp[rr] * 3;
                    q0 = __fsub_rn(q0, cp[0]); q1 = __fsub_rn(q1, cp[1]); q2 = __fsub_rn(q2, cp[2]);
                }
                *reinterpret_cast<float4*>(dxS + 4 * tid) = make_float4(q0, q1, q2, 0.f);
            }
        }
        GAD_WPH(1);
        write_lds(0, S0);
        if (nk > 2) load_regs(2, S0);
        __syncthreads();
        GAD_WPH(2);
        auto ktile = [&](int kt, auto nxtc) {
            if (SP) {
                GAD_WKL(0);
                spw::ktile(smem_b + (kt & 1) * spw::STAGE, (wm * 32 + l31) * 64, (wn * 64 + l31) * 64, sp_fo, acc, an);
                GAD_WKL(1);
                if (kt + 1 < nk) write_lds(kt + 1, nxtc);
                if (kt + 3 < nk) load_regs(kt + 3, nxtc);
                GAD_WKL(2);
                __syncthreads();
                GAD_WKL(3);
                return;
            }
            const float* As = smem + (kt & 1) * STAGE + (wm * 32 + l31) * P + 4 * half;
            const float* Bs = smem + (kt & 1) * STAGE + BM * P + (wn * 64 + l31) * P + 4 * half;
            float4 a4 = *reinterpret_cast<const float4*>(As);
            float4 b0 = *reinterpret_cast<const float4*>(Bs), b1 = *reinterpret_cast<const float4*>(Bs + 32 * P);
#pragma unroll
            for (int j = 0; j < KT / 8; ++j) {
                float4 an = a4, bn0 = b0, bn1 = b1;
                if (j + 1 < KT / 8) {
                    an = *reinterpret_cast<const float4*>(As + 8 * (j + 1));
                    bn0 = *reinterpret_cast<const float4*>(Bs + 8 * (j + 1));
                    bn1 = *reinterpret_cast<const float4*>(Bs + 32 * P + 8 * (j + 1));
                }
                acc[0] = __builtin_amdgcn_mfma_f32_32x32x2f32(a4.x, b0.x, acc[0], 0, 0, 0);
                acc[1] = __builtin_amdgcn_mfma_f32_32x32x2f32(a4.x, b1.x, acc[1], 0, 0, 0);
                acc[0] = __builtin_amdgcn_mfma_f32_32x32x2f32(a4.y, b0.y, acc[0], 0, 0, 0);
                acc[1] = __builtin_amdgcn_mfma_f32_32x32x2f32(a4.y, b1.y, acc[1], 0, 0, 0);
                acc[0] = __builtin_amdgcn_mfma_f32_32x32x2f32(a4.z, b0.z, acc[0], 0, 0, 0);
                acc[1] = __builtin_amdgcn_mfma_f32_32x32x2f32(a4.z, b1.z, acc[1], 0, 0, 0);
                acc[0] = __builtin_amdgcn_mfma_f32_32x32x2f32(a4.w, b0.w, acc[0], 0, 0, 0);
                acc[1] = __builtin_amdgcn_mfma_f32_32x32x2f32(a4.w, b1.w, acc[1], 0, 0, 0);
                a4 = an; b0 = bn0; b1 = bn1;
            }
            if (kt + 1 < nk) write_lds(kt + 1, nxtc);
            if (kt + 3 < nk) load_regs(kt + 3, nxtc);
            __syncthreads();
        };
        for (int kt = 0; kt < nk; kt += 2) {
            ktile(kt, S1);
            if (kt + 1 < nk) ktile(kt + 1, S0);
        }
        GAD_WPH(3);
        if (SP) {
#pragma unroll
            for (int t = 0; t < 2; ++t)
#pragma unroll
                for (int v = 0; v < 16; ++v) acc[t][v] = (v & 1) ? an[t][v] - acc[t][v] : acc[t][v] - an[t][v];
        }
        if (XM == 1) {
#pragma unroll
            for (int t = 0; t < 2; ++t) {
                const float* wx = W + (size_t)(n0 + wn * 64 + t * 32 + l31) * Kp + x.feat_c;
                const float w0 = wx[0], w1 = wx[1], w2 = wx[2];
#pragma unroll
                for (int v = 0; v < 16; ++v) {
                    const float4 q = *reinterpret_cast<const float4*>(dxS + 4 * (wm * 32 + acc_row(v, half)));
                    acc[t][v] = fmaf(q.x, w0, fmaf(q.y, w1, fmaf(q.z, w2, acc[t][v])));
                }
            }
        }
        if (POOL) {
            float* zt = smem;
#pragma unroll
            for (int t = 0; t < 2; ++t)
#pragma unroll
                for (int v = 0; v < 16; ++v) zt[(wm * 32 + acc_row(v, half)) * 129 + wn * 64 + t * 32 + l31] = acc[t][v];
            __syncthreads();
            const int gb = __builtin_amdgcn_readfirstlane(pg_before), ga = __builtin_amdgcn_readfirstlane(pg_after);
            pool_tile64<2>(zt + lane, 129, 64, pgl, row0, min(64, n_rows - row0), psgn, wave, 4, gb, ga, pe.key + n0 + lane, pe.C);
        }
        if (SP) {
#pragma unroll
        for (int t = 0; t < 2; ++t) {
            const int n = n0 + wn * 64 + t * 32 + l31;
            const int vzo = (4 * half * zout_pitch + n) * 4;
#pragma unroll
            for (int v = 0; v < 16; ++v)
                __builtin_amdgcn_raw_buffer_store_b32(__float_as_uint(acc[t][v]), zo_, vzo, (row0 + wm * 32 + (v & 3) + 8 * (v >> 2)) * zo_pitch4, 0);
        }
        __builtin_amdgcn_sched_barrier(0);
#pragma unroll
        for (int t = 0; t < 2; ++t) {
            float s1 = 0.f, s2 = 0.f;
#pragma unroll
            for (int v = 0; v < 16; ++v) {
                const float w = wS[wm * 32 + acc_row(v, half)];
                const float zv = acc[t][v];
                s1 = fmaf(w, zv, s1);
                s2 = fmaf(w * zv, zv, s2);
            }
            csum[t] += s1;
            csq[t] += s2;
        }
        } else {
#pragma unroll
        for (int t = 0; t < 2; ++t) {
            const int n = n0 + wn * 64 + t * 32 + l31;
            const int vzo = (4 * half * zout_pitch + n) * 4;
            float s1 = 0.f, s2 = 0.f;
#pragma unroll
            for (int v = 0; v < 16; ++v) {
                const int il = wm * 32 + acc_row(v, half);
                const float zv = acc[t][v];
                __builtin_amdgcn_raw_buffer_store_b32(__float_as_uint(zv), zo_, vzo, (row0 + wm * 32 + (v & 3) + 8 * (v >> 2)) * zo_pitch4, 0);
                const float w = wS[il];
                s1 = fmaf(w, zv, s1);
                s2 = fmaf(w * zv, zv, s2);
            }
            csum[t] += s1;
            csq[t] += s2;
        }
        }
        GAD_WPH(4);
    }
    if (stat_sum) {
        const int rep = blockIdx.x % GAD_STAT_REPLICAS;
        block_column_atomics<2, 2, 2>(smem, csum, csq, lane, wm, wn, n0, n_out, stat_sum + (size_t)rep * stat_stride,
                                      stat_sq + (size_t)rep * stat_stride);
    }
#ifdef GAD_W_PHASES
    __asm__ volatile("s_waitcnt vmcnt(0)" ::: "memory");
    GAD_WPH(5);
    GAD_WPH_STORE(ts);
    GAD_WKL_STORE(ts);
#endif
}

static bool fwd_wideable(const gad_gemm_fwd_args& a) {
    if (g_opt.deterministic || !g_opt.fwd_wide || a.n_groups != 1 || a.zin_off[0] != 0 || a.w_off[0] != 0 || a.out_off[0] != 0) return false;
    if (!fits_i32_bytes(a.n_rows, a.mode == 1 ? a.feat_c : a.zin_pitch, a.zout ? a.zout_pitch : 0, 0, 0)) return false;
    if (a.n_rows < 2048 || a.n_out[0] % 128 != 0 || a.ones_col >= 0) return false;
    if (a.mode == 2) return false;
    if (a.mode == 1)
        return g_opt.fwd_wide != 2 && !a.pool_key && a.act_c == 0 && a.feat_c % 32 == 0 && a.feat_c >= 32 && a.feat_c <= 512 &&
               a.Kp == ((a.feat_c + 3 + 7) & ~7);
    if (a.Kp % 32 != 0 || a.Kp > 512 || a.Kp != a.c_in) return false;
    return !a.extra && a.scale && a.shift && a.relu;
}

template <int KJ, int TN, int XM, bool POOL, bool SP = false>
__global__ __launch_bounds__(512, 2) void gemm_fwd_stream_kernel(XSrc x, const int32_t* __restrict__ n_rows_dev,
                                                                  int n_rows_static, const float* __restrict__ row_w,
                                                                  const float* __restrict__ W, float* __restrict__ zout,
                                                                  double* __restrict__ stat_sum,
                                                                  double* __restrict__ stat_sq, int stat_stride, PoolEpi pe,
                                                                  unsigned long long* __restrict__ ts) {
#ifdef GAD_X_PHASES
    const long long kt_start = __builtin_readcyclecounter();
#else
    KTimer kt(ts);
#endif
    constexpr int KP = 8 * KJ, NO = 32 * TN, PW = KP + 4;
    constexpr bool RE = XM >= 2;
    constexpr int PK = RE ? XM - 1 : 0;
    constexpr bool ACT = XM == 0 || RE, GATHER = XM == 1 || RE;
    constexpr int NG = RE ? PK : KJ;
    static_assert(!RE || (KJ == 8 && !POOL), "recomputed input: 64 channels");
    static_assert(!SP || (XM == 0 && KJ == 8), "split-bf16: ACT input, 64 channels");
    constexpr int PB = 2 * KP + 16;
    __shared__ __attribute__((aligned(16))) float Ws[SP ? 3 * NO * PB / 4 : NO * PW];
    __shared__ __attribute__((aligned(16))) float sv[KP], tv[KP];
    __shared__ float red[2 * 8 * NO];
    __shared__ float pz[POOL ? 8 * 32 * 64 : 1];
    static_assert(!POOL || TN == 4, "pooled epilogue: 128 output columns");
    const int tid = threadIdx.x, lane = tid & 63;
    const int wave = __builtin_amdgcn_readfirstlane(tid >> 6);
    const int l31 = lane & 31, half = lane >> 5;
    const int n_rows = n_rows_dev ? min(*n_rows_dev, n_rows_static) : n_rows_static;
    const int n_slabs = (n_rows + 31) >> 5;
#if GAD_X_PHASES == 2
    long long st1, st2, st3, st4;
    __asm__ volatile("s_waitcnt lgkmcnt(0)" ::: "memory");
    GAD_PH_STAMP(st1);
#endif
    int stride = gridDim.x * 8;
    int slab = wave * gridDim.x + blockIdx.x;
    int slab_end = n_slabs;
    if (POOL) {
        const int nw = gridDim.x * 8, base = n_slabs / nw, rem = n_slabs - base * nw;
        slab_end = slab * base + min(slab, rem) + base + (slab < rem ? 1 : 0);
        slab = slab * base + min(slab, rem);
        stride = 1;
    }
    const bool store_z = zout != nullptr;
    const __amdgpu_buffer_rsrc_t zrsrc =
        __builtin_amdgcn_make_buffer_rsrc(store_z ? zout : const_cast<float*>(W), 0, store_z ? gad_nbytes(n_rows, NO * 4) : 0, 0x00020000);
    const int zlane = (4 * half * NO + l31) * 4;
    float psgn[2];
    PoolRun prun[2];
    const int range0 = slab * 32;
    int g_after = -1;
    if (POOL && slab < slab_end) {
        const int g0 = pe.row_grp[range0];
        const int part0 = range0 > 0 && pe.row_grp[range0 - 1] == g0;
        if (slab_end * 32 < n_rows) g_after = pe.row_grp[slab_end * 32];
#pragma unroll
        for (int p = 0; p < 2; ++p) {
            psgn[p] = pe.gamma[p * 64 + lane] < 0.f ? -1.f : 1.f;
            prun[p].g = g0; prun[p].part = part0; prun[p].v = -INFINITY; prun[p].row = range0;
        }
    }

    f32x2 csum[TN], csq[TN];
#pragma unroll
    for (int t = 0; t < TN; ++t) { csum[t] = f32x2{0.f, 0.f}; csq[t] = f32x2{0.f, 0.f}; }

    XRaw ra[NG], rn[NG];
    float4 w1f[RE ? 2 : 1][RE ? PK : 1];
    if (RE) {
#pragma unroll
        for (int b = 0; b < 2; ++b)
#pragma unroll
            for (int j = 0; j < PK; ++j) w1f[b][j] = ldg4(x.pre_W + (size_t)(32 * b + l31) * x.pre_Kp + 8 * j + 4 * half);
    }
    int pt_nxt = 0;
    auto load_pt = [&](int sl) {
        const int r = min(sl * 32 + l31, max(n_rows - 1, 0));
        return (GATHER && sl < n_slabs) ? x.row_pt[r] : 0;
    };
    auto load_slab = [&](int sl, int pt, XRaw (&dst)[NG]) {
        const int r = min(sl < n_slabs ? sl * 32 + l31 : 0, max(n_rows - 1, 0));
        if (GATHER) {
            struct F3 { float x, y, z; } __attribute__((packed, aligned(4)));
            const float4 f = ldg4(x.feat + (size_t)pt * 4);
            const F3 p = *reinterpret_cast<const F3*>(x.src_xyz + (size_t)pt * 3);
            const int grp = x.row_grp[r];
            float q0 = p.x, q1 = p.y, q2 = p.z;
            if (x.ctr_xyz) {
                const F3 c = *reinterpret_cast<const F3*>(x.ctr_xyz + (size_t)grp * 3);
                q0 = __fsub_rn(q0, c.x); q1 = __fsub_rn(q1, c.y); q2 = __fsub_rn(q2, c.z);
            }
            float a0 = 0.f, a1 = 0.f, a2 = 0.f, a3 = 0.f, a4 = 0.f, a5 = 0.f;
            if (x.action) {
                const float* ap = x.action + (size_t)(grp / x.gps) * 6;
                const F3 u = *reinterpret_cast<const F3*>(ap), v = *reinterpret_cast<const F3*>(ap + 3);
                a0 = u.x; a1 = u.y; a2 = u.z; a3 = v.x; a4 = v.y; a5 = v.z;
            }
#pragma unroll
            for (int j = 0; j < NG; ++j) {
                dst[j].a = f;
                if (j == 0) dst[j].s = make_float4(q0, q1, q2, a0);
                else dst[j].s = half ? make_float4(a5, 0.f, 0.f, 0.f) : make_float4(a1, a2, a3, a4);
            }
            return;
        }
#pragma unroll
        for (int j = 0; j < NG; ++j)
            dst[j] = x_raw<GATHER ? 1 : 0>(x, r, true, 0, SP ? 16 * (j >> 1) + 8 * half + 4 * (j & 1) : 8 * j + 4 * half, GATHER, pt);
    };
    auto lds_b = [&](int j, float4 (&b4)[TN]) {
#pragma unroll
        for (int t = 0; t < TN; ++t) b4[t] = *reinterpret_cast<const float4*>(Ws + (t * 32 + l31) * PW + 8 * j + 4 * half);
    };
    {
        const int pt0 = load_pt(slab);
        load_slab(slab, pt0, ra);
        pt_nxt = load_pt(slab + stride);
    }
    {
        constexpr int UNITS = NO * KJ * 2, UW = (UNITS + 511) / 512;
        float4 wr[UW];
#pragma unroll
        for (int it = 0; it < UW; ++it) {
            const int u = it * 512 + tid;
            wr[it] = ldg4(W + (size_t)(u < UNITS ? u : 0) * 4);
        }
#if GAD_X_PHASES == 2
        GAD_PH_STAMP(st2);
        __asm__ volatile("s_waitcnt vmcnt(0)" ::: "memory");
        GAD_PH_STAMP(st3);
#endif
        if (ACT && tid < KP) {
            float sc, sh;
            if (x.bn.stat_sum) gad_bn_fin_channel(x.bn, tid, blockIdx.x == 0, sc, sh);
            else { sc = x.scale[tid]; sh = x.shift[tid]; }
            sv[tid] = sc; tv[tid] = sh;
        }
#pragma unroll
        for (int it = 0; it < UW; ++it) {
            const int u = it * 512 + tid;
            const int n = u / (KJ * 2), c = (u % (KJ * 2)) * 4;
            if (SP) {
                unsigned h0, m0, l0, h1, m1, l1;
                gad_split2(wr[it].x, wr[it].y, h0, m0, l0);
                gad_split2(wr[it].z, wr[it].w, h1, m1, l1);
                unsigned char* wp = reinterpret_cast<unsigned char*>(Ws) + n * PB + c * 2;
                if (u < UNITS) {
                    *reinterpret_cast<uint2*>(wp) = make_uint2(h0, h1);
                    *reinterpret_cast<uint2*>(wp + NO * PB) = make_uint2(m0, m1);
                    *reinterpret_cast<uint2*>(wp + 2 * NO * PB) = make_uint2(l0, l1);
                }
            } else if (u < UNITS) *reinterpret_cast<float4*>(Ws + n * PW + c) = wr[it];
        }
    }
    __syncthreads();
#if GAD_X_PHASES == 2
    GAD_PH_STAMP(st4);
    if (ts && lane == 0) {
        auto c16 = [&](long long t) { const long long d = (t - kt_start) >> 2; return (unsigned long long)(d > 65535 ? 65535 : d); };
        ts[2 * (blockIdx.x * 8 + wave)] = c16(st1) | (c16(st2) << 16) | (c16(st3) << 32) | (c16(st4) << 48);
    }
#endif

#ifdef GAD_X_PHASES
    long long tA = 0, tB = 0, tC = 0, ph_top = 0, ph_mfma = 0, ph_epi = 0;
    int ph_n = 0;
    long long tP, tS;
    GAD_PH_STAMP(tP);
    tS = (long long)kt_start;
#endif
    for (; slab < slab_end; slab += stride) {
        load_slab(slab + stride, pt_nxt, rn);
        pt_nxt = load_pt(slab + 2 * stride);
        float4 w4[4];
#pragma unroll
        for (int q = 0; q < 4; ++q) {
            const int r0 = slab * 32 + 8 * q + 4 * half;
            w4[q] = row_w ? ldg4(row_w + (r0 + 3 < n_rows_static ? r0 : 0)) : make_float4(1.f, 1.f, 1.f, 1.f);
        }
        if (slab * 32 + 32 > n_rows) {
#pragma unroll
            for (int q = 0; q < 4; ++q) {
                float* wq = &w4[q].x;
#pragma unroll
                for (int e = 0; e < 4; ++e) wq[e] = (slab * 32 + 8 * q + 4 * half + e < n_rows) ? wq[e] : 0.f;
            }
        }
        int gl = -1;
        if (POOL) { const int rr = slab * 32 + l31; gl = rr < n_rows ? pe.row_grp[rr] : -1; }
        __asm__ volatile("" ::: "memory");
        f32x16 acc[TN];
#pragma unroll
        for (int t = 0; t < TN; ++t)
#pragma unroll
            for (int v = 0; v < 16; ++v) acc[t][v] = 0.f;
        float4 bn[TN];
        if (!SP) lds_b(0, bn);
        GAD_PH_STAMP(tA);
        if (SP) {
            const unsigned char* wp = reinterpret_cast<const unsigned char*>(Ws) + l31 * PB + 16 * half;
            constexpr int NS = SP ? KJ / 2 : 1;
            gad_u32x4 AH[NS], AM[NS], AL[NS];
#pragma unroll
            for (int sg = 0; sg < NS; ++sg) {
                unsigned ah[4], am[4], al[4];
#pragma unroll
                for (int e = 0; e < 2; ++e) {
                    const int c = 16 * sg + 8 * half + 4 * e;
                    const float4 s4 = *reinterpret_cast<const float4*>(sv + c), t4 = *reinterpret_cast<const float4*>(tv + c);
                    const float4 zr = ra[SP ? 2 * sg + e : 0].a;
                    const float a0 = __builtin_fmaxf(fmaf(zr.x, s4.x, t4.x), 0.f), a1 = __builtin_fmaxf(fmaf(zr.y, s4.y, t4.y), 0.f);
                    const float a2 = __builtin_fmaxf(fmaf(zr.z, s4.z, t4.z), 0.f), a3 = __builtin_fmaxf(fmaf(zr.w, s4.w, t4.w), 0.f);
                    gad_split2(a0, a1, ah[2 * e], am[2 * e], al[2 * e]);
                    gad_split2(a2, a3, ah[2 * e + 1], am[2 * e + 1], al[2 * e + 1]);
                }
                const unsigned sgn = ((sg ^ l31) & 1) ? 0x80008000u : 0u;
                AH[sg] = gad_u32x4{ah[0] ^ sgn, ah[1] ^ sgn, ah[2] ^ sgn, ah[3] ^ sgn};
                AM[sg] = gad_u32x4{am[0] ^ sgn, am[1] ^ sgn, am[2] ^ sgn, am[3] ^ sgn};
                AL[sg] = gad_u32x4{al[0] ^ sgn, al[1] ^ sgn, al[2] ^ sgn, al[3] ^ sgn};
            }
#pragma unroll
            for (int pp = 0; pp < TN / 2; ++pp) {
                f32x16 an[2];
#pragma unroll
                for (int i = 0; i < 2; ++i)
#pragma unroll
                    for (int v = 0; v < 16; ++v) an[i][v] = 0.f;
#pragma unroll
                for (int sg = 0; sg < NS; ++sg) {
                    gad_u32x4 BH[2], BM[2], BL[2];
#pragma unroll
                    for (int i = 0; i < 2; ++i) {
                        const unsigned char* q = wp + (2 * pp + i) * 32 * PB + 32 * sg;
                        BH[i] = *reinterpret_cast<const gad_u32x4*>(q);
                        BM[i] = *reinterpret_cast<const gad_u32x4*>(q + NO * PB);
                        BL[i] = *reinterpret_cast<const gad_u32x4*>(q + 2 * NO * PB);
                    }
#define GAD_SPLIT_MFMA(A, B)                                                                                                   \
                    _Pragma("unroll") for (int i = 0; i < 2; ++i) {                                                             \
                        if (sg & 1) an[i] = __builtin_amdgcn_mfma_f32_32x32x16_bf16(gad_as_bf16x8(A[sg]), gad_as_bf16x8(B[i]), an[i], 0, 0, 0); \
                        else acc[2 * pp + i] = __builtin_amdgcn_mfma_f32_32x32x16_bf16(gad_as_bf16x8(A[sg]), gad_as_bf16x8(B[i]), acc[2 * pp + i], 0, 0, 0); \
                    }
                    GAD_SPLIT_MFMA(AL, BH) GAD_SPLIT_MFMA(AH, BL) GAD_SPLIT_MFMA(AM, BM)
                    GAD_SPLIT_MFMA(AM, BH) GAD_SPLIT_MFMA(AH, BM) GAD_SPLIT_MFMA(AH, BH)
#undef GAD_SPLIT_MFMA
                }
#pragma unroll
                for (int i = 0; i < 2; ++i)
#pragma unroll
                    for (int v = 0; v < 16; ++v) acc[2 * pp + i][v] = (v & 1) ? an[i][v] - acc[2 * pp + i][v] : acc[2 * pp + i][v] - an[i][v];
            }
        }
        f32x16 zacc[RE ? 2 : 1];
        if (RE) {
#pragma unroll
            for (int b = 0; b < 2; ++b)
#pragma unroll
                for (int v = 0; v < 16; ++v) zacc[b][v] = 0.f;
#pragma unroll
            for (int j = 0; j < PK; ++j) {
                const float4 xb = x_finish<1>(x, ra[j], true, 8 * j + 4 * half, sv, tv);
#pragma unroll
                for (int b = 0; b < 2; ++b) zacc[b] = __builtin_amdgcn_mfma_f32_32x32x2f32(w1f[b][j].x, xb.x, zacc[b], 0, 0, 0);
#pragma unroll
                for (int b = 0; b < 2; ++b) zacc[b] = __builtin_amdgcn_mfma_f32_32x32x2f32(w1f[b][j].y, xb.y, zacc[b], 0, 0, 0);
#pragma unroll
                for (int b = 0; b < 2; ++b) zacc[b] = __builtin_amdgcn_mfma_f32_32x32x2f32(w1f[b][j].z, xb.z, zacc[b], 0, 0, 0);
#pragma unroll
                for (int b = 0; b < 2; ++b) zacc[b] = __builtin_amdgcn_mfma_f32_32x32x2f32(w1f[b][j].w, xb.w, zacc[b], 0, 0, 0);
            }
        }
#pragma unroll
        for (int j = 0; j < (SP ? 0 : KJ); ++j) {
            float4 b4[TN];
#pragma unroll
            for (int t = 0; t < TN; ++t) b4[t] = bn[t];
            float4 a4;
            if (ACT) {
                const float4 s4 = *reinterpret_cast<const float4*>(sv + 8 * j + 4 * half);
                const float4 t4 = *reinterpret_cast<const float4*>(tv + 8 * j + 4 * half);
                float4 zr;
                if (RE) zr = make_float4(zacc[j >> 2][4 * (j & 3)], zacc[j >> 2][4 * (j & 3) + 1], zacc[j >> 2][4 * (j & 3) + 2],
                                         zacc[j >> 2][4 * (j & 3) + 3]);
                else zr = ra[RE ? 0 : j].a;
                const f32x2 lo = f32x2{zr.x, zr.y} * f32x2{s4.x, s4.y} + f32x2{t4.x, t4.y};
                const f32x2 hi = f32x2{zr.z, zr.w} * f32x2{s4.z, s4.w} + f32x2{t4.z, t4.w};
                a4 = make_float4(__builtin_fmaxf(lo.x, 0.f), __builtin_fmaxf(lo.y, 0.f), __builtin_fmaxf(hi.x, 0.f),
                                 __builtin_fmaxf(hi.y, 0.f));
            } else {
                a4 = x_finish<1>(x, ra[RE ? 0 : j], true, 8 * j + 4 * half, sv, tv);
            }
            if (j + 1 < KJ) lds_b(j + 1, bn);
#pragma unroll
            for (int t = 0; t < TN; ++t) acc[t] = __builtin_amdgcn_mfma_f32_32x32x2f32(a4.x, b4[t].x, acc[t], 0, 0, 0);
#pragma unroll
            for (int t = 0; t < TN; ++t) acc[t] = __builtin_amdgcn_mfma_f32_32x32x2f32(a4.y, b4[t].y, acc[t], 0, 0, 0);
#pragma unroll
            for (int t = 0; t < TN; ++t) acc[t] = __builtin_amdgcn_mfma_f32_32x32x2f32(a4.z, b4[t].z, acc[t], 0, 0, 0);
#pragma unroll
            for (int t = 0; t < TN; ++t) acc[t] = __builtin_amdgcn_mfma_f32_32x32x2f32(a4.w, b4[t].w, acc[t], 0, 0, 0);
        }
        GAD_PH_STAMP(tB);
        const int zrow = slab * 32 * NO * 4;
        if (POOL) {
            float* zt = pz + wave * (32 * 64);
#pragma unroll
            for (int p = 0; p < 2; ++p) {
#pragma unroll
                for (int v = 0; v < 16; ++v) {
                    zt[acc_row(v, half) * 64 + l31] = acc[2 * p][v];
                    zt[acc_row(v, half) * 64 + 32 + l31] = acc[2 * p + 1][v];
                }
                pool_scan32(zt + lane, 64, gl, slab * 32, psgn[p], prun[p], pe.key + p * 64 + lane, pe.C);
            }
        }
#pragma unroll
        for (int v = 0; v < 16; v += 2) {
            const int rb = ((v & 3) + 8 * (v >> 2)) * NO * 4;
            const f32x2 wr = f32x2{(&w4[v >> 2].x)[v & 3], (&w4[v >> 2].x)[(v & 3) + 1]};
#pragma unroll
            for (int t = 0; t < TN; ++t) {
                const f32x2 zv = f32x2{acc[t][v], acc[t][v + 1]};
                if (store_z) {
                    __builtin_amdgcn_raw_buffer_store_b32(__float_as_uint(acc[t][v]), zrsrc, zlane + t * 128, zrow + rb, GAD_STREAM_STORE_AUX);
                    __builtin_amdgcn_raw_buffer_store_b32(__float_as_uint(acc[t][v + 1]), zrsrc, zlane + t * 128, zrow + rb + NO * 4, GAD_STREAM_STORE_AUX);
                }
                const f32x2 wz = wr * zv;
                csum[t] += wz;
                csq[t] += wz * zv;
            }
        }
#pragma unroll
        for (int j = 0; j < NG; ++j) ra[j] = rn[j];
#ifdef GAD_X_PHASES
        GAD_PH_STAMP(tC);
        ph_top += tA - tP; ph_mfma += tB - tA; ph_epi += tC - tB; tP = tC; ++ph_n;
#endif
    }
#ifdef GAD_X_PHASES
    if (ts && lane == 0) {
        const unsigned w = blockIdx.x * 8 + wave;
        if (GAD_X_PHASES != 2) ts[2 * w] = ((unsigned long long)ph_mfma << 32) | (unsigned long long)(ph_epi & 0xffffffffu);
        ts[2 * w + 1] = ((unsigned long long)ph_top << 32) | ((unsigned long long)(tP - tS) & 0xffffff00u) | (unsigned long long)ph_n;
    }
#endif
    if (POOL && range0 < slab_end * 32) {
#pragma unroll
        for (int p = 0; p < 2; ++p)
            if (prun[p].g >= 0)
                pool_put(pe.key + p * 64 + lane, prun[p].g, pe.C, prun[p].v, prun[p].row, prun[p].part != 0 || prun[p].g == g_after);
    }
    if (stat_sum) {
#pragma unroll
        for (int t = 0; t < TN; ++t) {
            const float c0 = csum[t].x + csum[t].y, c1 = csq[t].x + csq[t].y;
            const float s0 = c0 + __shfl_xor(c0, 32, 64);
            const float s1 = c1 + __shfl_xor(c1, 32, 64);
            if (lane < 32) { red[wave * NO + t * 32 + lane] = s0; red[(8 + wave) * NO + t * 32 + lane] = s1; }
        }
        __syncthreads();
        if (tid < NO) {
            float s0 = 0.f, s1 = 0.f;
#pragma unroll
            for (int w = 0; w < 8; ++w) { s0 += red[w * NO + tid]; s1 += red[(8 + w) * NO + tid]; }
            const int rep = blockIdx.x % GAD_STAT_REPLICAS;
            atomic_add_f64(stat_sum + (size_t)rep * stat_stride + tid, (double)s0);
            atomic_add_f64(stat_sq + (size_t)rep * stat_stride + tid, (double)s1);
        }
    }
}

template <int NW>
__global__ __launch_bounds__(64 * NW) void gemm_fwd_skinny_kernel(XSrc x, Groups gr, int n_rows,
                                                                     const float* __restrict__ row_w,
                                                                     const float* __restrict__ W, int Kp,
                                                                     float* __restrict__ zout, int zout_pitch,
                                                                     double* __restrict__ stat_sum,
                                                                     double* __restrict__ stat_sq, int stat_stride, unsigned long long* __restrict__ ts) {
    KTimer kt(ts);
    __shared__ __attribute__((aligned(16))) float stA[NW * 32 * SK_SP], stW[NW * 32 * SK_SP];
    __shared__ __attribute__((aligned(16))) float sv[SK_KCAP], tv[SK_KCAP];
    float* const part = stA;
    static_assert(32 * SK_SP >= 16 * 64, "partial tile must fit the wavefront's stage");
    const int tid = threadIdx.x, lane = tid & 63;
    const int wave = __builtin_amdgcn_readfirstlane(tid >> 6);
    const int l31 = lane & 31, half = lane >> 5;
    const int g = blockIdx.z;
    const int zoff = gr.aoff[g], n_out = gr.nout[g], ooff = gr.ooff[g];
    const int n0 = blockIdx.x * 32, row0 = blockIdx.y * 32;
    if (n0 >= n_out) return;
    const float* Wg = W + gr.woff[g] + (size_t)min(n0 + l31, n_out - 1) * Kp + 4 * half;
    const int r = min(row0 + l31, max(n_rows - 1, 0));
    const int nj = Kp >> 3;
    const int per = (nj + NW - 1) / NW;
    const int j0 = wave * per, j1 = min(nj, j0 + per);

    f32x16 acc;
#pragma unroll
    for (int v = 0; v < 16; ++v) acc[v] = 0.f;
    float* const myA = stA + wave * (32 * SK_SP);
    float* const myW = stW + wave * (32 * SK_SP);
    const int rsub = lane >> 3, chunk = lane & 7;
    const float* pa[4];
    const float* pw[4];
#pragma unroll
    for (int i = 0; i < 4; ++i) {
        pa[i] = x.zin + (size_t)min(row0 + rsub + 8 * i, max(n_rows - 1, 0)) * x.zin_pitch + zoff + 4 * chunk;
        pw[i] = W + gr.woff[g] + (size_t)min(n0 + rsub + 8 * i, n_out - 1) * Kp + 4 * chunk;
    }
    auto staged = [&](int jb) { return jb + 4 <= j1 && 8 * (jb + 4) <= x.c_in; };
    float4 ga[4], gw[4];
    auto load_blk = [&](int jb) {
#pragma unroll
        for (int i = 0; i < 4; ++i) { ga[i] = ldg4(pa[i] + 8 * jb); gw[i] = ldg4(pw[i] + 8 * jb); }
    };
    if (j0 < j1 && staged(j0)) load_blk(j0);
    if (x.bn.stat_sum) {
        const bool writer = blockIdx.x == 0 && blockIdx.y == 0;
        for (int i = tid; i < x.c_in; i += 64 * NW) {
            float sc, sh;
            gad_bn_fin_channel(x.bn, i, writer, sc, sh);
            sv[i] = sc;
            tv[i] = sh;
        }
    } else if (x.affine) stage_affine<64 * NW>(sv, tv, x, zoff, x.c_in);
    __syncthreads();
    for (int jb = j0; jb < j1; jb += 4) {
        if (staged(jb)) {
#pragma unroll
            for (int i = 0; i < 4; ++i) {
                *reinterpret_cast<float4*>(myA + (rsub + 8 * i) * SK_SP + 4 * chunk) = ga[i];
                *reinterpret_cast<float4*>(myW + (rsub + 8 * i) * SK_SP + 4 * chunk) = gw[i];
            }
            if (jb + 4 < j1 && staged(jb + 4)) load_blk(jb + 4);
            __builtin_amdgcn_fence(__ATOMIC_RELEASE, "wavefront");
            __builtin_amdgcn_wave_barrier();
            __builtin_amdgcn_fence(__ATOMIC_ACQUIRE, "wavefront");
#pragma unroll
            for (int u = 0; u < 4; ++u) {
                XRaw raw;
                raw.a = *reinterpret_cast<const float4*>(myA + l31 * SK_SP + 8 * u + 4 * half);
                raw.s = f4zero();
                const float4 a4 = x_finish<0>(x, raw, true, 8 * (jb + u) + 4 * half, sv, tv);
                const float4 b4 = *reinterpret_cast<const float4*>(myW + l31 * SK_SP + 8 * u + 4 * half);
                acc = __builtin_amdgcn_mfma_f32_32x32x2f32(a4.x, b4.x, acc, 0, 0, 0);
                acc = __builtin_amdgcn_mfma_f32_32x32x2f32(a4.y, b4.y, acc, 0, 0, 0);
                acc = __builtin_amdgcn_mfma_f32_32x32x2f32(a4.z, b4.z, acc, 0, 0, 0);
                acc = __builtin_amdgcn_mfma_f32_32x32x2f32(a4.w, b4.w, acc, 0, 0, 0);
            }
            __builtin_amdgcn_fence(__ATOMIC_RELEASE, "wavefront");
            __builtin_amdgcn_wave_barrier();
        } else {
            const int je = min(jb + 4, j1);
            XRaw ra[4];
            float4 rb[4];
#pragma unroll
            for (int u = 0; u < 4; ++u) {
                const int j = min(jb + u, nj - 1);
                const int col = 8 * j + 4 * half;
                ra[u] = x_raw<0>(x, r, true, zoff, col, col + 4 > x.c_in, 0);
                rb[u] = ldg4(Wg + 8 * j);
            }
            if (jb + 4 < j1 && staged(jb + 4)) load_blk(jb + 4);
#pragma unroll
            for (int u = 0; u < 4; ++u) {
                if (jb + u < je) {
                    const float4 a4 = x_finish<0>(x, ra[u], true, 8 * (jb + u) + 4 * half, sv, tv);
                    const float4 b4 = rb[u];
                    acc = __builtin_amdgcn_mfma_f32_32x32x2f32(a4.x, b4.x, acc, 0, 0, 0);
                    acc = __builtin_amdgcn_mfma_f32_32x32x2f32(a4.y, b4.y, acc, 0, 0, 0);
                    acc = __builtin_amdgcn_mfma_f32_32x32x2f32(a4.z, b4.z, acc, 0, 0, 0);
                    acc = __builtin_amdgcn_mfma_f32_32x32x2f32(a4.w, b4.w, acc, 0, 0, 0);
                }
            }
        }
    }
#pragma unroll
    for (int v = 0; v < 16; ++v) part[wave * (32 * SK_SP) + v * 64 + lane] = acc[v];
    __syncthreads();
    if (wave != 0) return;
#pragma unroll
    for (int w = 1; w < NW; ++w)
#pragma unroll
        for (int v = 0; v < 16; ++v) acc[v] += part[w * (32 * SK_SP) + v * 64 + lane];
    const int n = n0 + l31;
    float s1 = 0.f, s2 = 0.f;
#pragma unroll
    for (int v = 0; v < 16; ++v) {
        const int rr = row0 + acc_row(v, half);
        const float zv = acc[v];
        const bool live = rr < n_rows;
        if (live && n < n_out) zout[(size_t)rr * zout_pitch + ooff + n] = zv;
        const float w = live ? (row_w ? row_w[rr] : 1.f) : 0.f;
        s1 = fmaf(w, zv, s1);
        s2 = fmaf(w * zv, zv, s2);
    }
    if (stat_sum) {
        s1 += __shfl_xor(s1, 32, 64);
        s2 += __shfl_xor(s2, 32, 64);
        if (lane < 32 && n < n_out) {
            const int rep = blockIdx.y % GAD_STAT_REPLICAS;
            atomic_add_f64(stat_sum + (size_t)rep * stat_stride + ooff + n, (double)s1);
            atomic_add_f64(stat_sq + (size_t)rep * stat_stride + ooff + n, (double)s2);
        }
    }
}

static bool fwd_skinny(const gad_gemm_fwd_args& a) {
    return !g_opt.deterministic && g_opt.fwd_skinny && a.mode == 0 && !a.n_rows_dev && a.n_rows <= 1024 && a.Kp <= SK_KCAP;
}

bool fwd_streamable(const gad_gemm_fwd_args& a) {
    if (g_opt.deterministic || !g_opt.fwd_stream) return false;
    if (a.pool_key && !(a.mode == 0 && a.n_out[0] == 128)) return false;
    if (a.n_groups != 1 || a.zin_off[0] != 0 || a.w_off[0] != 0 || a.out_off[0] != 0) return false;
    if (a.n_rows < 32768 || (a.n_out[0] != 64 && a.n_out[0] != 128) || (a.zout && a.zout_pitch != a.n_out[0])) return false;
    if ((long long)a.n_rows * a.n_out[0] * 4 > (1ll << 31)) return false;
    if (a.mode == 0) return a.Kp == 64 && a.c_in == 64 && a.ones_col < 0 && !a.extra && (a.scale && a.shift) && a.relu;
    const bool sa1_rows = a.feat_c == 4 && (a.action ? a.act_c == 6 : a.act_c == 0);
    if (a.mode == 2)
        return a.Kp == 64 && a.c_in == 64 && a.n_out[0] == 64 && !a.pool_key && a.ones_col < 0 && !a.extra && a.scale && a.shift && a.relu &&
               a.pre_W && (a.pre_Kp == 8 || a.pre_Kp == 16) && sa1_rows && a.feat_c + 3 + a.act_c <= a.pre_Kp;
    return (a.Kp == 16 || a.Kp == 8) && a.feat_c == 4 && (a.action ? a.act_c == 6 : a.act_c == 0) && a.feat_c + 3 + a.act_c <= a.Kp;
}

extern "C" int gad_gemm_fwd(const gad_gemm_fwd_args* a, void* stream) {
    unsigned long long* ts = gad_take_timing_slot(stream);
    const int rows_hint = gad_take_grid_rows();
    GAD_REQUIRE(a && a->W && (a->zout || a->pool_key || a->stat_sum), GAD_ERR_NULL, "gemm_fwd: null pointer");
    GAD_REQUIRE(a->n_groups >= 1 && a->n_groups <= GAD_MAX_GROUPS, GAD_ERR_SHAPE, "gemm_fwd: n_groups");
    GAD_REQUIRE(a->Kp % 8 == 0 && a->Kp >= 8, GAD_ERR_SHAPE, "gemm_fwd: Kp=%d must be a multiple of 8", a->Kp);
    if (int e = check_input(*a, "gemm_fwd")) return e;
    if (a->n_rows <= 0) return GAD_OK;
    XSrc x = make_xsrc(*a);
    Groups gr = make_groups(a->n_groups, a->zin_off, a->w_off, a->out_off, a->n_out);
    const int nmax = max_nout(gr);
    hipStream_t st = (hipStream_t)stream;
    const int rows = a->n_rows;
    PoolEpi pe;
    pe.key = reinterpret_cast<unsigned long long*>(a->pool_key); pe.row_grp = a->pool_row_grp; pe.gamma = a->pool_gamma;
    pe.C = a->n_out[0];
    if (pe.key) {
        GAD_REQUIRE(pe.row_grp && pe.gamma, GAD_ERR_NULL, "gemm_fwd: fused max-pool needs pool_row_grp and pool_gamma");
        GAD_REQUIRE(a->mode == 0 && a->n_groups == 1 && a->out_off[0] == 0 && a->n_out[0] % 64 == 0 && rows % 4 == 0,
                    GAD_ERR_SHAPE, "gemm_fwd: fused max-pool needs an ACT input, one group, n_out %% 64 == 0, rows %% 4 == 0 (got n_out=%d rows=%d)",
                    a->n_out[0], rows);
    }
    const int grid_rows = (a->n_rows_dev && rows_hint > 0 && rows_hint < rows) ? rows_hint : rows;
    int ncol_stats = 0;
    for (int i = 0; i < gr.n; ++i) ncol_stats = gr.ooff[i] + gr.nout[i] > ncol_stats ? gr.ooff[i] + gr.nout[i] : ncol_stats;
    if (a->in_stat_sum) {
        GAD_REQUIRE(a->mode != 1 && a->n_groups == 1 && a->zin_off[0] == 0 && a->in_stat_sq && a->in_gamma && a->in_beta && a->scale && a->shift,
                    GAD_ERR_NULL, "gemm_fwd: input-layer BatchNorm block needs an ACT input, one group, in_stat_sq, in_gamma, in_beta, scale, shift");
        const bool has_prologue = fwd_wideable(*a) || (fwd_streamable(*a) && a->mode != 1) || (!pe.key && fwd_skinny(*a));
        if (!(has_prologue && g_opt.fwd_bn_prologue)) {
            if (int e = gad_bn_finalize(a->in_stat_sum, a->in_stat_sq, a->in_stat_stride, a->in_gamma, a->in_beta, a->c_in, a->in_count,
                                        a->in_eps, a->in_momentum, a->in_running_mean, a->in_running_var, const_cast<float*>(a->scale),
                                        const_cast<float*>(a->shift), a->in_mean, a->in_istd, stream)) return e;
            x.bn.stat_sum = nullptr;
        }
    }
    if (!pe.key && fwd_skinny(*a)) {
        GAD_REQUIRE(a->zout, GAD_ERR_NULL, "gemm_fwd: zout == NULL is not supported for small-M (skinny) shapes");
        GAD_LAUNCH_SKINNY(gemm_fwd_skinny_kernel, dim3(gad_cdiv(nmax, 32), gad_cdiv(rows, 32), gr.n), st, x, gr, rows, a->row_w, a->W,
                          a->Kp, a->zout, a->zout_pitch, a->stat_sum, a->stat_sq, a->stat_stride, ts);
        GAD_CHECK_LAUNCH("gemm_fwd(skinny)");
        return GAD_OK;
    }
#define LAUNCH_FWD2(WM, WN, TM, TN, XM, POOL)                                                                  \
    do {                                                                                                   \
        constexpr int BM = WM * TM * 32, BN = WN * TN * 32;                                                \
        int gx = gad_cdiv(grid_rows, BM); if (gx > GAD_GX_CAP) gx = GAD_GX_CAP;                                        \
        if (g_opt.deterministic && a->stat_sum) {                                                          \
            double* slots = det_stat_slots(gx, ncol_stats, stream);                                        \
            if (!slots) return GAD_ERR_LAUNCH;                                                             \
            hipLaunchKernelGGL((gemm_fwd_kernel<WM, WN, TM, TN, XM, POOL, true>), dim3(gx, gad_cdiv(nmax, BN), gr.n), dim3(256), \
                               0, st, x, gr, a->n_rows_dev, rows, a->row_w, a->W, a->Kp, a->zout, a->zout_pitch, \
                               slots, slots + (size_t)gx * ncol_stats, ncol_stats, pe, ts);                \
            GAD_CHECK_LAUNCH("gemm_fwd");                                                                  \
            if (int e_ = det_stat_reduce(slots, gx, ncol_stats, a->stat_sum, a->stat_sq, stream)) return e_; \
        } else                                                                                             \
            hipLaunchKernelGGL((gemm_fwd_kernel<WM, WN, TM, TN, XM, POOL>), dim3(gx, gad_cdiv(nmax, BN), gr.n), dim3(256), \
                               0, st, x, gr, a->n_rows_dev, rows, a->row_w, a->W, a->Kp, a->zout, a->zout_pitch, \
                               a->stat_sum, a->stat_sq, a->stat_stride, pe, ts);                           \
    } while (0)
#define LAUNCH_FWD(WM, WN, TM, TN) do { if (a->mode == 0) LAUNCH_FWD2(WM, WN, TM, TN, 0, false); else LAUNCH_FWD2(WM, WN, TM, TN, 1, false); } while (0)
    if (fwd_streamable(*a)) {
        const int slabs = gad_cdiv(rows, 32);
        const int gcap = a->mode == 1 ? g_opt.fwd_stream_l1_wgs : g_opt.fwd_stream_wgs;
        int gx = gad_cdiv(slabs, 8); if (gx > gcap) gx = gcap;
#define LAUNCH_STREAM(KJ, TN, XM, POOL, ...)                                                               \
        hipLaunchKernelGGL((gemm_fwd_stream_kernel<KJ, TN, XM, POOL, ##__VA_ARGS__>), dim3(gx), dim3(512), 0, st, x, a->n_rows_dev, rows, \
                           a->row_w, a->W, a->zout, a->stat_sum, a->stat_sq, a->stat_stride, pe, ts)
        if (split_on(GAD_SPLIT_FWD_STREAM) && a->mode == 0) {
            if (pe.key) LAUNCH_STREAM(8, 4, 0, true, true);
            else if (a->n_out[0] == 64) LAUNCH_STREAM(8, 2, 0, false, true);
            else LAUNCH_STREAM(8, 4, 0, false, true);
        } else if (pe.key) {
            LAUNCH_STREAM(8, 4, 0, true);
        } else {
            if (a->mode == 2) { if (a->pre_Kp == 8) LAUNCH_STREAM(8, 2, 2, false); else LAUNCH_STREAM(8, 2, 3, false); }
            else if (a->mode == 0) { if (a->n_out[0] == 64) LAUNCH_STREAM(8, 2, 0, false); else LAUNCH_STREAM(8, 4, 0, false); }
            else if (a->Kp == 8) { if (a->n_out[0] == 64) LAUNCH_STREAM(1, 2, 1, false); else LAUNCH_STREAM(1, 4, 1, false); }
            else { if (a->n_out[0] == 64) LAUNCH_STREAM(2, 2, 1, false); else LAUNCH_STREAM(2, 4, 1, false); }
        }
#undef LAUNCH_STREAM
        if (split_on(GAD_SPLIT_FWD_STREAM) && a->mode == 0) GAD_CHECK_LAUNCH("gemm_fwd(stream split)"); else GAD_CHECK_LAUNCH("gemm_fwd(stream)");
        return GAD_OK;
    }
    if (fwd_wideable(*a)) {
        int gx = gad_cdiv(grid_rows, 64); if (gx > GAD_GX_CAP) gx = GAD_GX_CAP;
        const dim3 grid(gx, a->n_out[0] / 128);
        const bool sp = split_on(GAD_SPLIT_FWD_WIDE) && a->W_split && a->W_split_pitch == (a->mode == 1 ? a->feat_c : a->Kp) &&
                        a->W_split_plane >= a->n_out[0] * a->W_split_pitch;
#define LAUNCH_WIDE(XM, POOL, SP)                                                                                              \
        hipLaunchKernelGGL((gemm_fwd_wide_kernel<XM, POOL, SP>), grid, dim3(256), 0, st, x, a->n_rows_dev, rows, a->row_w, a->W, a->Kp, \
                           a->n_out[0], a->zout, a->zout_pitch, a->stat_sum, a->stat_sq, a->stat_stride, pe, a->W_split, a->W_split_pitch, \
                           a->W_split_plane, ts)
        if (a->mode == 1) { if (sp) LAUNCH_WIDE(1, false, true); else LAUNCH_WIDE(1, false, false); }
        else if (pe.key) { if (sp) LAUNCH_WIDE(0, true, true); else LAUNCH_WIDE(0, true, false); }
        else { if (sp) LAUNCH_WIDE(0, false, true); else LAUNCH_WIDE(0, false, false); }
#undef LAUNCH_WIDE
        if (sp) GAD_CHECK_LAUNCH("gemm_fwd(wide split)"); else GAD_CHECK_LAUNCH("gemm_fwd(wide)");
        return GAD_OK;
    }
    if (pe.key) LAUNCH_FWD2(2, 2, 1, 1, 0, true);
    else if (nmax <= 32) LAUNCH_FWD(4, 1, 1, 1); else LAUNCH_FWD(2, 2, 1, 1);
#undef LAUNCH_FWD
#undef LAUNCH_FWD2
    GAD_CHECK_LAUNCH("gemm_fwd");
    return GAD_OK;
}
```

ga-ddpg_amd/hip.py:

```python
import ctypes as C
import os

import torch

_HERE = os.path.dirname(os.path.abspath(__file__))
LIB_PATH = os.environ.get("GAD_LIB_PATH") or os.path.join(_HERE, "libgaddpg.so")
MAX_GROUPS = 3
STAT_REPLICAS = 4

_i32, _f32, _f64, _vp = C.c_int32, C.c_float, C.c_double, C.c_void_p


class GemmFwdArgs(C.Structure):
    _fields_ = [("n_rows_dev", _vp), ("n_rows", _i32), ("row_w", _vp), ("mode", _i32),
                ("zin", _vp), ("zin_pitch", _i32), ("c_in", _i32), ("scale", _vp), ("shift", _vp),
                ("relu", _i32), ("extra", _vp), ("ones_col", _i32),
                ("src_xyz", _vp), ("ctr_xyz", _vp), ("feat", _vp), ("feat_c", _i32),
                ("action", _vp), ("act_c", _i32), ("grp_per_sample", _i32),
                ("row_pt", _vp), ("row_grp", _vp),
                ("n_groups", _i32), ("zin_off", _i32 * MAX_GROUPS), ("w_off", _i32 * MAX_GROUPS),
                ("out_off", _i32 * MAX_GROUPS), ("n_out", _i32 * MAX_GROUPS),
                ("W", _vp), ("Kp", _i32), ("zout", _vp), ("zout_pitch", _i32),
                ("stat_sum", _vp), ("stat_sq", _vp), ("stat_stride", _i32),
                ("pool_key", _vp), ("pool_row_grp", _vp), ("pool_gamma", _vp),
                ("in_stat_sum", _vp), ("in_stat_sq", _vp), ("in_stat_stride", _i32), ("in_count", _f64),
                ("in_gamma", _vp), ("in_beta", _vp), ("in_eps", _f32), ("in_momentum", _f32),
                ("in_running_mean", _vp), ("in_running_var", _vp), ("in_mean", _vp), ("in_istd", _vp),
                ("pre_W", _vp), ("pre_Kp", _i32),
                ("W_split", _vp), ("W_split_pitch", _i32), ("W_split_plane", _i32)]


class DzSrc(C.Structure):
    _fields_ = [("z", _vp), ("z_pitch", _i32), ("scale", _vp), ("shift", _vp), ("relu", _i32),
                ("coefP", _vp), ("coefQ", _vp), ("coefS", _vp), ("row_w", _vp), ("gmode", _i32),
                ("G", _vp), ("g_pitch", _i32), ("argmax", _vp), ("dout", _vp), ("row_grp", _vp),
                ("c", _i32), ("premasked", _i32),
                ("bn_dbeta", _vp), ("bn_dgamma", _vp), ("bn_stride", _i32), ("bn_count", _f64), ("bn_mean", _vp), ("bn_istd", _vp),
                ("gacc_gamma", _vp), ("gacc_beta", _vp)]


class GemmDxArgs(C.Structure):
    _fields_ = [("n_rows_dev", _vp), ("n_rows", _i32), ("dz", DzSrc), ("n_groups", _i32),
                ("dz_off", _i32 * MAX_GROUPS), ("w_off", _i32 * MAX_GROUPS), ("n_out", _i32 * MAX_GROUPS),
                ("gout_off", _i32 * MAX_GROUPS), ("accumulate", _i32), ("W", _vp), ("Kp", _i32),
                ("k_valid", _i32), ("epilogue", _i32), ("gout", _vp), ("gout_pitch", _i32),
                ("zprev", _vp), ("zprev_pitch", _i32), ("prev_scale", _vp), ("prev_shift", _vp),
                ("prev_mean", _vp), ("prev_istd", _vp), ("prev_dbeta", _vp), ("prev_dgamma", _vp),
                ("stat_stride", _i32), ("store_masked", _i32), ("dfeat", _vp), ("feat_c", _i32), ("row_pt", _vp), ("row_grp", _vp),
                ("daction", _vp), ("act_c", _i32), ("grp_per_sample", _i32),
                ("W_split_t", _vp), ("W_split_t_pitch", _i32), ("W_split_t_plane", _i32)]


class GemmDwArgs(C.Structure):
    _fields_ = [("inp", GemmFwdArgs), ("dz", DzSrc), ("dz_off", _i32 * MAX_GROUPS), ("gacc", _vp),
                ("row_splits", _i32), ("partial", _vp), ("partial_elems", C.c_int64)]


class ReplayGatherArgs(C.Structure):
    _fields_ = [("B", _i32), ("cloud_elems", _i32), ("idx", _vp), ("nxt", _vp), ("end", _vp), ("point_state", _vp),
                ("action", _vp), ("expert_action", _vp), ("goal", _vp), ("reward", _vp), ("returns", _vp),
                ("terminal", _vp), ("timestep", _vp), ("expert_flags", _vp), ("perturb_flags", _vp),
                ("out_point", _vp), ("out_next_point", _vp), ("out_action", _vp), ("out_expert_action", _vp),
                ("out_goal", _vp), ("out_reward", _vp), ("out_return", _vp), ("out_mask", _vp), ("out_time", _vp),
                ("out_time_m1", _vp), ("out_expert_flag", _vp), ("out_perturb_flag", _vp)]


REPLAY_MAX_SRC = 4


class ReplaySrc(C.Structure):
    _fields_ = [("point_state", _vp), ("action", _vp), ("expert_action", _vp), ("goal", _vp), ("reward", _vp), ("returns", _vp),
                ("terminal", _vp), ("timestep", _vp), ("expert_flags", _vp), ("perturb_flags", _vp)]


class ReplayMixArgs(C.Structure):
    _fields_ = [("B", _i32), ("cloud_elems", _i32), ("n_src", _i32), ("row_start", _i32 * (REPLAY_MAX_SRC + 1)),
                ("src", ReplaySrc * REPLAY_MAX_SRC), ("idx", _vp), ("nxt", _vp), ("end", _vp), ("relabel", _vp),
                ("out_point", _vp), ("out_next_point", _vp), ("out_action", _vp), ("out_expert_action", _vp),
                ("out_goal", _vp), ("out_reward", _vp), ("out_return", _vp), ("out_mask", _vp), ("out_time", _vp),
                ("out_time_m1", _vp), ("out_expert_flag", _vp), ("out_perturb_flag", _vp)]


class ReplayRelabelSrc(C.Structure):
    _fields_ = [("state_pose", _vp), ("expert_flags", _vp)]


class ReplayRelabelArgs(C.Structure):
    _fields_ = [("B", _i32), ("n_src", _i32), ("row_start", _i32 * (REPLAY_MAX_SRC + 1)),
                ("src", ReplayRelabelSrc * REPLAY_MAX_SRC), ("idx", _vp), ("end", _vp), ("out_goal", _vp)]


class OptimJob(C.Structure):
    _fields_ = [("n", _i32), ("p", _vp), ("grad", _vp), ("exp_avg", _vp), ("exp_avg_sq", _vp), ("active", _vp), ("m2p", _vp),
                ("packed", _vp), ("gacc", _vp), ("accumulate", _i32), ("hyper", _vp), ("clip_sumsq", _vp), ("clip_max", _f32),
                ("target", _vp), ("target_sel", _vp), ("target_m2p", _vp), ("target_packed", _vp), ("tau", _f32),
                ("hard_enable", _i32), ("absmax_p", _vp), ("absmax_grad", _vp), ("counter", _vp), ("counter_n", _i32),
                ("counter_add", _i32)]


class CopySeg(C.Structure):
    _fields_ = [("dst", _vp), ("src", _vp), ("bytes", C.c_longlong), ("add", _f32), ("reserved_", _i32)]


COPY_MAX_SEGS = 16


class SplitLayer(C.Structure):
    _fields_ = [("w_off", _i32), ("n_out", _i32), ("Kp", _i32), ("Ks", _i32), ("fwd_off", C.c_int64), ("t_off", C.c_int64)]


MAX_SPLIT_LAYERS = 16
SPLIT_ALL, SPLIT_FWD_STREAM, SPLIT_FWD_WIDE, SPLIT_DX_WIDE, SPLIT_DW_WIDE, SPLIT_BWD_STREAM, SPLIT_DW_STREAM = 1, 2, 4, 8, 16, 32, 64

_lib = None


def lib():
    global _lib
    if _lib is None:
        if not os.path.exists(LIB_PATH):
            raise RuntimeError("libgaddpg.so not found at %s -- build it with "
                               "`python -c 'import __graft_entry__ as g; g.build()'` (hipcc, gfx950). "
                               "The update-step path has no CPU fallback." % LIB_PATH)
        L = C.CDLL(LIB_PATH)
        L.gad_last_error.restype = C.c_char_p
        L.gad_abi_version.restype = C.c_int
        L.gad_last_kernel.restype = C.c_char_p
        L.gad_plan_entry_name.restype = C.c_char_p
        for name, argtypes in _SIGNATURES.items():
            f = getattr(L, name)
            f.argtypes, f.restype = argtypes, _RESTYPES.get(name, C.c_int)
        _lib = L
        for name, v in OPTION_DEFAULTS.items():
            check(L.gad_set_option(name.encode(), int(v)), "gad_set_option(%s)" % name)
        for k, v in os.environ.items():
            if k.startswith("GAD_OPT_"):
                check(L.gad_set_option(k[8:].encode(), int(v)), "gad_set_option(%s)" % k[8:])
        _lib_det[0] = get_option_default("deterministic")
        sync_deterministic()
    return _lib


EXPORTS = (
    "gad_abi_version", "gad_last_kernel", "gad_last_error", "gad_set_option", "gad_timing_slot", "gad_stream_priority", "gad_wall_clock_khz", "gad_grid_rows_hint", "gad_bn_running_update", "gad_replay_gather", "gad_replay_gather_multi", "gad_replay_relabel_goals", "gad_zero_buffers", "gad_furthest_point_sampling", "gad_gather_points",
    "gad_fps_tiled_workspace_bytes", "gad_fps_tiled",
    "gad_gather_points_grad", "gad_ball_query", "gad_ball_query_grid_workspace_bytes", "gad_ball_query_grid",
    "gad_group_points", "gad_group_points_grad",
    "gad_three_nn", "gad_three_nn_grid_workspace_bytes", "gad_three_nn_grid", "gad_three_interpolate", "gad_three_interpolate_grad",
    "gad_backproject_depth_workspace_bytes", "gad_backproject_depth", "gad_cloud_gather_affine", "gad_point_state_pack",
    "gad_query_and_group", "gad_prep_points", "gad_rows_from_ball_query", "gad_rows_group_all",
    "gad_gemm_fwd", "gad_bn_finalize", "gad_bn_eval_affine", "gad_segment_pool", "gad_pool_finalize", "gad_affine_act", "gad_transpose_batched",
    "gad_pool_bwd_stats", "gad_bn_bwd_coef", "gad_gemm_dx", "gad_gemm_dw", "gad_gemm_bwd", "gad_gemm_dw_reduce", "gad_sa_coord_grad", "gad_critic_loss",
    "gad_policy_outputs", "gad_policy_sample", "gad_actor_loss", "gad_actor_critic_loss", "gad_mask_counts", "gad_target_noise",
    "gad_grad_from_arena", "gad_grad_from_arena_sumsq", "gad_optim_jobs", "gad_sumsq", "gad_absmax_segments", "gad_adam_step", "gad_polyak",
    "gad_pack_params", "gad_split_weights", "gad_copy_buffers",
    "gad_plan_create", "gad_plan_destroy", "gad_plan_size", "gad_plan_add_call", "gad_plan_add_wait", "gad_plan_add_record",
    "gad_plan_add_wait_event", "gad_plan_add_memset", "gad_plan_add_memcpy", "gad_plan_patch", "gad_plan_arm_timing", "gad_plan_run",
    "gad_plan_entry_count", "gad_plan_entry_name")


_SIGNATURES = {
    "gad_fps_tiled_workspace_bytes": [C.c_int, C.c_int, C.c_int, C.c_int],
    "gad_fps_tiled": [_vp, C.c_int, C.c_int, C.c_int, C.c_int, _vp, _vp, _vp, _vp],
    "gad_ball_query_grid_workspace_bytes": [C.c_int, C.c_int, C.c_int, C.c_int],
    "gad_ball_query_grid": [_vp, _vp, C.c_int, C.c_int, C.c_int, C.c_float, C.c_int, _vp, _vp, _vp, _vp],
    "gad_three_nn": [_vp, _vp, C.c_int, C.c_int, C.c_int, _vp, _vp, _vp],
    "gad_three_nn_grid_workspace_bytes": [C.c_int, C.c_int, C.c_int],
    "gad_three_nn_grid": [_vp, _vp, C.c_int, C.c_int, C.c_int, _vp, _vp, _vp, _vp, _vp],
    "gad_three_interpolate": [_vp, _vp, _vp, C.c_int, C.c_int, C.c_int, C.c_int, _vp, _vp],
    "gad_three_interpolate_grad": [_vp, _vp, _vp, C.c_int, C.c_int, C.c_int, C.c_int, _vp, _vp],
    "gad_backproject_depth_workspace_bytes": [C.c_int, C.c_int, C.c_int],
    "gad_backproject_depth": [_vp, C.c_int, C.c_float, _vp, _vp, C.c_int, C.c_int, C.c_int, _vp, _vp, _vp, _vp, _vp],
    "gad_cloud_gather_affine": [_vp, C.c_int, _vp, _vp, C.c_int, C.c_int, _vp, C.c_int, _vp],
    "gad_point_state_pack": [_vp, C.c_int, _vp, _vp, _vp, C.c_int, C.c_float, C.c_int, C.c_int, _vp, _vp],
    "gad_sa_coord_grad": [C.POINTER(DzSrc), _vp, C.c_int, C.c_int, C.c_int, _vp, C.c_int, _vp, _vp, _vp, _vp, C.c_int, C.c_int,
                          _vp, _vp, _vp],
}


_RESTYPES = {"gad_fps_tiled_workspace_bytes": C.c_longlong, "gad_ball_query_grid_workspace_bytes": C.c_longlong,
             "gad_three_nn_grid_workspace_bytes": C.c_longlong, "gad_backproject_depth_workspace_bytes": C.c_longlong}


def workspace(name, device, *shape):
    nbytes = getattr(lib(), name + "_workspace_bytes")(*shape)
    if nbytes < 0:
        check(int(nbytes), name + "_workspace_bytes")
    return torch.empty(nbytes, dtype=torch.uint8, device=device)


class Ptr(int):
    """a raw device address (crosses the ABI as void*, never as a 32-bit int)"""


def ptr(t, offset_bytes=0):
    if t is None:
        return None
    if isinstance(t, int):
        return Ptr(t + offset_bytes)
    return Ptr(t.data_ptr() + offset_bytes)


def stream():
    return C.c_void_p(torch.cuda.current_stream().cuda_stream)


def check(status, what):
    if status != 0:
        raise RuntimeError("%s failed (status %d): %s" % (what, status, lib().gad_last_error().decode()))


def _args(*a):
    out = []
    for x in a:
        if x is None:
            out.append(C.c_void_p(None))
        elif torch.is_tensor(x):
            out.append(C.c_void_p(x.data_ptr()))
        elif isinstance(x, Ptr):
            out.append(C.c_void_p(int(x)))
        elif isinstance(x, float):
            out.append(C.c_float(x))
        elif isinstance(x, Dbl):
            out.append(C.c_double(x.v))
        elif isinstance(x, bool):
            out.append(C.c_int(int(x)))
        elif isinstance(x, int):
            out.append(C.c_int(x))
        else:
            out.append(x)
    return out


class Dbl(object):
    def __init__(self, v):
        self.v = float(v)


def call(name, *a):
    f = getattr(lib(), name)
    sync_deterministic()
    check(f(*(_args(*a) + [stream()])), name)


def call_struct(name, s):
    f = getattr(lib(), name)
    sync_deterministic()
    check(f(C.byref(s), stream()), name)


def require_cuda(*tensors):
    for t in tensors:
        if t is not None and (not t.is_cuda):
            raise RuntimeError("CPU tensor passed to a libgaddpg operator (CPU not supported)")
        if t is not None and not t.is_contiguous():
            raise RuntimeError("libgaddpg operators need contiguous tensors")


OPTION_DEFAULTS = {"mfma_split": 1, "deterministic": 0, "tnn_grid": 1}
LIBRARY_DEFAULTS = {"fps_cfg": 0}


def get_option_default(name):
    return int(os.environ.get("GAD_OPT_" + name, OPTION_DEFAULTS.get(name, LIBRARY_DEFAULTS.get(name, 1))))


_options = {}
ROUTES = {}


def set_option(name, value):
    check(lib().gad_set_option(name.encode(), int(value)), "gad_set_option")
    _options[name] = int(value)
    if name == "deterministic":
        _lib_det[0] = int(value)
        sync_deterministic()
    ROUTES.clear()


def get_option(name):
    if name == "deterministic":
        return deterministic()
    return _options.get(name, get_option_default(name))


_lib_det = [0]


def deterministic():
    if torch.are_deterministic_algorithms_enabled():
        return 1
    return int(bool(_options.get("deterministic", get_option_default("deterministic"))))


def sync_deterministic():
    want = deterministic()
    if want != _lib_det[0]:
        check(lib().gad_set_option(b"deterministic", want), "gad_set_option(deterministic)")
        _lib_det[0] = want
        ROUTES.clear()
    return want
```

Measured before the change: 399.2.

## Pick 32-row wide-GEMM tiles for small grids and balance grid to one round

```diff
diff --git a/ga-ddpg_amd/csrc/gemm.hip b/ga-ddpg_amd/csrc/gemm.hip
--- a/ga-ddpg_amd/csrc/gemm.hip
+++ b/ga-ddpg_amd/csrc/gemm.hip
@@ -130,7 +130,31 @@
     {"dw_wide_wgs", &GemmOptions::dw_wide_wgs, 1, 2147483647, 256},
     {"bwd_wide_slab", &GemmOptions::bwd_wide_slab, 1, 2147483647, 4},
     {"skinny_nw", &GemmOptions::skinny_nw, 4, 4, SK_NW},
+    {"wide_bm", &GemmOptions::wide_bm, 32, 64, 0},
+    {"wide_one_round", &GemmOptions::wide_one_round, ANY_LO, ANY_HI, 0},
 };
+
+static int cu_count() {
+    static const int n = [] {
+        int dev = 0, v = 0;
+        if (hipGetDevice(&dev) != hipSuccess || hipDeviceGetAttribute(&v, hipDeviceAttributeMultiprocessorCount, dev) != hipSuccess || v <= 0)
+            v = 256;
+        return v;
+    }();
+    return n;
+}
+WideGrid wide_grid(int grid_rows, int col_blocks) {
+    const int cus = cu_count();
+    const int tiles64 = gad_cdiv(grid_rows, 64);
+    WideGrid g;
+    const bool forced = g_opt.wide_bm == 32 || g_opt.wide_bm == 64;
+    g.bm = forced ? g_opt.wide_bm : ((long long)tiles64 * col_blocks <= cus ? 32 : 64);
+    const int tiles = gad_cdiv(grid_rows, g.bm);
+    g.gx = tiles > GAD_GX_CAP ? GAD_GX_CAP : tiles;
+    const int slots = 2 * cus / col_blocks;
+    if (g_opt.wide_one_round && g.bm == 64 && slots > 0 && tiles > slots) g.gx = gad_cdiv(tiles, gad_cdiv(tiles, slots));
+    return g;
+}
 
 extern "C" int gad_set_option(const char* name, int value) {
     GAD_REQUIRE(name, GAD_ERR_NULL, "set_option: null name");
diff --git a/ga-ddpg_amd/csrc/gemm_common.hpp b/ga-ddpg_amd/csrc/gemm_common.hpp
--- a/ga-ddpg_amd/csrc/gemm_common.hpp
+++ b/ga-ddpg_amd/csrc/gemm_common.hpp
@@ -536,7 +536,8 @@
     *reinterpret_cast<uint2*>(q + APL) = make_uint2(m0, m1);
     *reinterpret_cast<uint2*>(q + 2 * APL) = make_uint2(l0, l1);
 }
-__device__ __forceinline__ void ktile(const unsigned char* stage, int arow, int brow, int fo, f32x16 (&acc)[2], f32x16 (&an)[2]) {
+template <int NT>
+__device__ __forceinline__ void ktile(const unsigned char* stage, int arow, int brow, int fo, f32x16 (&acc)[NT], f32x16 (&an)[NT]) {
 #pragma unroll
     for (int s = 0; s < 2; ++s) {
         const int off = fo ^ (s << 5);
@@ -544,15 +545,15 @@
         const unsigned char* bp = stage + 3 * APL + brow + off;
         const gad_u32x4 AH = *reinterpret_cast<const gad_u32x4*>(ap), AM = *reinterpret_cast<const gad_u32x4*>(ap + APL);
         const gad_u32x4 AL = *reinterpret_cast<const gad_u32x4*>(ap + 2 * APL);
-        gad_u32x4 BH[2], BM[2], BL[2];
-#pragma unroll
-        for (int t = 0; t < 2; ++t) {
+        gad_u32x4 BH[NT], BM[NT], BL[NT];
+#pragma unroll
+        for (int t = 0; t < NT; ++t) {
             BH[t] = *reinterpret_cast<const gad_u32x4*>(bp + t * (32 * 64));
             BM[t] = *reinterpret_cast<const gad_u32x4*>(bp + BPL + t * (32 * 64));
             BL[t] = *reinterpret_cast<const gad_u32x4*>(bp + 2 * BPL + t * (32 * 64));
         }
 #define GAD_SPW(A, B)                                                                                                          \
-        _Pragma("unroll") for (int t = 0; t < 2; ++t) {                                                                        \
+        _Pragma("unroll") for (int t = 0; t < NT; ++t) {                                                                       \
             if (s) an[t] = __builtin_amdgcn_mfma_f32_32x32x16_bf16(gad_as_bf16x8(A), gad_as_bf16x8(B[t]), an[t], 0, 0, 0);     \
             else acc[t] = __builtin_amdgcn_mfma_f32_32x32x16_bf16(gad_as_bf16x8(A), gad_as_bf16x8(B[t]), acc[t], 0, 0, 0);     \
         }
@@ -579,6 +580,8 @@
     int bwd_wide = 0;
     int bwd_wide_slab = 4;
     int dw_wide_wgs = 256;
+    int wide_bm = 0;
+    int wide_one_round = 1;
     int skinny_nw = SK_NW;
     int fwd_skinny = 1, dx_skinny = 1, dx_stream = 1, dw_skinny = 1, dw_stream = 1, fwd_stream = 1;
     int bwd_stream_wgs = DW_STREAM_SPLITS;
@@ -586,6 +589,8 @@
     int fwd_stream_l1_wgs = 256;
 };
 extern GemmOptions g_opt;
+struct WideGrid { int bm, gx; };
+WideGrid wide_grid(int grid_rows, int col_blocks);
 bool split_on(int family);
 
 #define GAD_LAUNCH_SKINNY(kernel, grid, st, ...)                                                                               \
diff --git a/ga-ddpg_amd/csrc/gemm_dx.hip b/ga-ddpg_amd/csrc/gemm_dx.hip
--- a/ga-ddpg_amd/csrc/gemm_dx.hip
+++ b/ga-ddpg_amd/csrc/gemm_dx.hip
@@ -150,21 +150,23 @@
     }
 }
 
-template <int GM, int SC, bool SP = false>
+template <int GM, int SC, bool SP = false, int BM_ = 64>
 __global__ __launch_bounds__(256, 2) void gemm_dx_wide_kernel(DzSrc d, const int32_t* __restrict__ n_rows_dev, int n_rows_static,
                                                               const float* __restrict__ W, int Kp, int n_out, DxEpi e,
                                                               const uint16_t* __restrict__ wsp, int wsp_plane,
                                                               unsigned long long* __restrict__ ts) {
     KTimer kt_(ts);
-    constexpr int BM = 64, BN = 128, P = KT + 4, PB = BN + 4, STAGE = SP ? spw::STAGE / 4 : BM * P + KT * PB, VM = 512;
-    __shared__ __attribute__((aligned(16))) float smem[2 * STAGE + 3 * VM + BM];
-    __shared__ int32_t ptS[BM];
+    constexpr int BM = BM_, AR = 64, NT = BM / 32, BN = 128, P = KT + 4, PB = BN + 4, STAGE = SP ? spw::STAGE / 4 : AR * P + KT * PB, VM = 512;
+    static_assert(BM == 64 || BM == 32, "row tiles of 64 (2 x 2 wavefronts) or 32 (1 x 4)");
+    __shared__ __attribute__((aligned(16))) float smem[2 * STAGE + 3 * VM + AR];
+    __shared__ int32_t ptS[AR];
     float* vP = smem + 2 * STAGE;
     float* wS = vP + 3 * VM;
     int32_t* grS = reinterpret_cast<int32_t*>(wS);
     const int tid = threadIdx.x, lane = tid & 63;
     const int wave = __builtin_amdgcn_readfirstlane(tid >> 6);
-    const int wm = wave >> 1, wn = wave & 1;
+    const int wm = BM == 64 ? wave >> 1 : 0, wn = BM == 64 ? wave & 1 : wave;
+    const int wc = wn * (NT * 32);
     const int l31 = lane & 31, half = lane >> 5;
     const int k0out = blockIdx.y * BN;
     const int n_rows = n_rows_dev ? min(*n_rows_dev, n_rows_static) : n_rows_static;
@@ -195,25 +197,25 @@
         vP[i] = Pc; vP[VM + i] = Qc; vP[2 * VM + i] = Sc;
     }
     (void)grS;
-    float ps[2] = {0.f, 0.f}, pt[2] = {0.f, 0.f}, pm[2] = {0.f, 0.f}, pi[2] = {0.f, 0.f};
-#pragma unroll
-    for (int t = 0; t < 2; ++t) {
-        const int k = k0out + wn * 64 + t * 32 + l31;
+    float ps[NT] = {}, pt[NT] = {}, pm[NT] = {}, pi[NT] = {};
+#pragma unroll
+    for (int t = 0; t < NT; ++t) {
+        const int k = k0out + wc + t * 32 + l31;
         if (!SC) { ps[t] = e.ps[k]; pt[t] = e.pt[k]; pm[t] = e.pm[k]; pi[t] = e.pi[k]; }
     }
-    float cb[2] = {0.f, 0.f}, cg[2] = {0.f, 0.f};
+    float cb[NT] = {}, cg[NT] = {};
     for (int row0 = blockIdx.x * BM; row0 < n_rows; row0 += gridDim.x * BM) {
-        f32x16 acc[2];
-        f32x16 an[2];
-#pragma unroll
-        for (int t = 0; t < 2; ++t)
+        f32x16 acc[NT];
+        f32x16 an[NT];
+#pragma unroll
+        for (int t = 0; t < NT; ++t)
 #pragma unroll
             for (int v = 0; v < 16; ++v) { acc[t][v] = 0.f; if (SP) an[t][v] = 0.f; }
-        int vz[2], vg[2];
-        float wrow[2];
-        bool live[2];
-#pragma unroll
-        for (int u = 0; u < 2; ++u) {
+        int vz[NT], vg[NT];
+        float wrow[NT];
+        bool live[NT];
+#pragma unroll
+        for (int u = 0; u < NT; ++u) {
             const int r = row0 + ur + 32 * u;
             live[u] = r < n_rows;
             const int rr = live[u] ? r : max(n_rows - 1, 0);
@@ -221,12 +223,12 @@
             vz[u] = (rr * d.z_pitch + c4) * 4;
             vg[u] = ((GM == 1 ? d.row_grp[rr] : rr) * gpitch + c4) * 4;
         }
-        float4 rz[2], rg[2], rb[SP ? 1 : 4];
-        gad_u32x4 ra[2];
+        float4 rz[NT], rg[NT], rb[SP ? 1 : 4];
+        gad_u32x4 ra[NT];
         spw::BRegs rbs;
         auto load_regs = [&](int kt) {
 #pragma unroll
-            for (int u = 0; u < 2; ++u) {
+            for (int u = 0; u < NT; ++u) {
                 rz[u] = buf_ld4(zr, vz[u], kt * (KT * 4));
                 rg[u] = buf_ld4(gr_, vg[u], kt * (KT * 4));
                 if (GM == 1) ra[u] = __builtin_amdgcn_raw_buffer_load_b128(ar, vg[u], kt * (KT * 4), 0);
@@ -237,12 +239,12 @@
         };
         auto write_lds = [&](int kt) {
             float* As = smem + (kt & 1) * STAGE;
-            float* Bs = As + BM * P;
+            float* Bs = As + AR * P;
             const int nb = kt * KT + c4;
             const float4 P4 = *reinterpret_cast<const float4*>(vP + nb), Q4 = *reinterpret_cast<const float4*>(vP + VM + nb);
             const float4 S4 = *reinterpret_cast<const float4*>(vP + 2 * VM + nb);
 #pragma unroll
-            for (int u = 0; u < 2; ++u) {
+            for (int u = 0; u < NT; ++u) {
                 float4 g = rg[u];
                 const float4 z = rz[u];
                 if (GM == 1) {
@@ -271,35 +273,40 @@
         __syncthreads();
         for (int kt = 0; kt < nk; ++kt) {
             if (SP) {
-                spw::ktile(smem_b + (kt & 1) * spw::STAGE, (wm * 32 + l31) * 64, (wn * 64 + l31) * 64, sp_fo, acc, an);
+                spw::ktile<NT>(smem_b + (kt & 1) * spw::STAGE, (wm * 32 + l31) * 64, (wc + l31) * 64, sp_fo, acc, an);
                 if (kt + 1 < nk) write_lds(kt + 1);
                 if (kt + 2 < nk) load_regs(kt + 2);
                 __syncthreads();
                 continue;
             }
             const float* As = smem + (kt & 1) * STAGE + (wm * 32 + l31) * P + 4 * half;
-            const float* Bs = smem + (kt & 1) * STAGE + BM * P + (4 * half) * PB + wn * 64 + l31;
+            const float* Bs = smem + (kt & 1) * STAGE + AR * P + (4 * half) * PB + wc + l31;
             float4 a4 = *reinterpret_cast<const float4*>(As);
-            float4 b0 = make_float4(Bs[0], Bs[PB], Bs[2 * PB], Bs[3 * PB]);
-            float4 b1 = make_float4(Bs[32], Bs[PB + 32], Bs[2 * PB + 32], Bs[3 * PB + 32]);
+            float4 b4[NT];
+#pragma unroll
+            for (int t = 0; t < NT; ++t) b4[t] = make_float4(Bs[32 * t], Bs[PB + 32 * t], Bs[2 * PB + 32 * t], Bs[3 * PB + 32 * t]);
 #pragma unroll
             for (int j = 0; j < KT / 8; ++j) {
-                float4 an = a4, bn0 = b0, bn1 = b1;
+                float4 an4 = a4, bn4[NT];
+#pragma unroll
+                for (int t = 0; t < NT; ++t) bn4[t] = b4[t];
                 if (j + 1 < KT / 8) {
-                    an = *reinterpret_cast<const float4*>(As + 8 * (j + 1));
+                    an4 = *reinterpret_cast<const float4*>(As + 8 * (j + 1));
                     const float* bq = Bs + 8 * (j + 1) * PB;
-                    bn0 = make_float4(bq[0], bq[PB], bq[2 * PB], bq[3 * PB]);
-                    bn1 = make_float4(bq[32], bq[PB + 32], bq[2 * PB + 32], bq[3 * PB + 32]);
+#pragma unroll
+                    for (int t = 0; t < NT; ++t) bn4[t] = make_float4(bq[32 * t], bq[PB + 32 * t], bq[2 * PB + 32 * t], bq[3 * PB + 32 * t]);
                 }
-                acc[0] = __builtin_amdgcn_mfma_f32_32x32x2f32(a4.x, b0.x, acc[0], 0, 0, 0);
-                acc[1] = __builtin_amdgcn_mfma_f32_32x32x2f32(a4.x, b1.x, acc[1], 0, 0, 0);
-                acc[0] = __builtin_amdgcn_mfma_f32_32x32x2f32(a4.y, b0.y, acc[0], 0, 0, 0);
-                acc[1] = __builtin_amdgcn_mfma_f32_32x32x2f32(a4.y, b1.y, acc[1], 0, 0, 0);
-                acc[0] = __builtin_amdgcn_mfma_f32_32x32x2f32(a4.z, b0.z, acc[0], 0, 0, 0);
-                acc[1] = __builtin_amdgcn_mfma_f32_32x32x2f32(a4.z, b1.z, acc[1], 0, 0, 0);
-                acc[0] = __builtin_amdgcn_mfma_f32_32x32x2f32(a4.w, b0.w, acc[0], 0, 0, 0);
-                acc[1] = __builtin_amdgcn_mfma_f32_32x32x2f32(a4.w, b1.w, acc[1], 0, 0, 0);
-                a4 = an; b0 = bn0; b1 = bn1;
+#pragma unroll
+                for (int t = 0; t < NT; ++t) acc[t] = __builtin_amdgcn_mfma_f32_32x32x2f32(a4.x, b4[t].x, acc[t], 0, 0, 0);
+#pragma unroll
+                for (int t = 0; t < NT; ++t) acc[t] = __builtin_amdgcn_mfma_f32_32x32x2f32(a4.y, b4[t].y, acc[t], 0, 0, 0);
+#pragma unroll
+                for (int t = 0; t < NT; ++t) acc[t] = __builtin_amdgcn_mfma_f32_32x32x2f32(a4.z, b4[t].z, acc[t], 0, 0, 0);
+#pragma unroll
+                for (int t = 0; t < NT; ++t) acc[t] = __builtin_amdgcn_mfma_f32_32x32x2f32(a4.w, b4[t].w, acc[t], 0, 0, 0);
+                a4 = an4;
+#pragma unroll
+                for (int t = 0; t < NT; ++t) b4[t] = bn4[t];
             }
             if (kt + 1 < nk) write_lds(kt + 1);
             if (kt + 2 < nk) load_regs(kt + 2);
@@ -307,14 +314,14 @@
         }
         if (SP) {
 #pragma unroll
-            for (int t = 0; t < 2; ++t)
+            for (int t = 0; t < NT; ++t)
 #pragma unroll
                 for (int v = 0; v < 16; ++v) acc[t][v] = (v & 1) ? an[t][v] - acc[t][v] : acc[t][v] - an[t][v];
         }
         if (SC) {
 #pragma unroll
-            for (int t = 0; t < 2; ++t) {
-                const int k = k0out + wn * 64 + t * 32 + l31;
+            for (int t = 0; t < NT; ++t) {
+                const int k = k0out + wc + t * 32 + l31;
 #pragma unroll
                 for (int v = 0; v < 16; ++v) {
                     const int il = wm * 32 + acc_row(v, half);
@@ -325,8 +332,8 @@
         }
         const int rb0 = row0 + wm * 32;
 #pragma unroll
-        for (int t = 0; t < 2; ++t) {
-            const int kcol = k0out + wn * 64 + t * 32 + l31;
+        for (int t = 0; t < NT; ++t) {
+            const int kcol = k0out + wc + t * 32 + l31;
             const int vzp = (4 * half * e.zprev_pitch + kcol) * 4, vgo = (4 * half * e.gout_pitch + kcol) * 4;
             float zp[16];
 #pragma unroll
@@ -345,8 +352,8 @@
     }
     if (SC) return;
     const int rep = blockIdx.x % GAD_STAT_REPLICAS;
-    block_column_atomics<2, 2, 2>(smem, cb, cg, lane, wm, wn, k0out, e.k_valid, e.dbeta + (size_t)rep * e.stat_stride,
-                                  e.dgamma + (size_t)rep * e.stat_stride);
+    block_column_atomics<BM / 32, 4 / (BM / 32), NT>(smem, cb, cg, lane, wm, wn, k0out, e.k_valid, e.dbeta + (size_t)rep * e.stat_stride,
+                                                     e.dgamma + (size_t)rep * e.stat_stride);
 }
 
 __global__ __launch_bounds__(256) void dx_action_stream_kernel(DzSrc d, const int32_t* __restrict__ n_rows_dev, int n_rows_static,
@@ -776,17 +783,19 @@
         return GAD_OK;
     }
     if (dx_wideable(*a, vec)) {
-        int gx = gad_cdiv(grid_rows, 64); if (gx > GAD_GX_CAP) gx = GAD_GX_CAP;
-        const dim3 grid(gx, kv / 128);
+        const WideGrid wg = wide_grid(grid_rows, kv / 128);
+        const dim3 grid(wg.gx, kv / 128);
         const bool sp = split_on(GAD_SPLIT_DX_WIDE) && a->W_split_t && a->W_split_t_pitch == a->n_out[0] && a->n_out[0] % 32 == 0 &&
                         a->W_split_t_plane >= kv * a->n_out[0];
-#define LAUNCH_DXW(GM, SC, SP)                                                                                                 \
-        hipLaunchKernelGGL((gemm_dx_wide_kernel<GM, SC, SP>), grid, dim3(256), 0, st, d, a->n_rows_dev, rows, a->W, a->Kp, a->n_out[0], e, \
+#define LAUNCH_DXW_BM(GM, SC, SP, BM)                                                                                          \
+        hipLaunchKernelGGL((gemm_dx_wide_kernel<GM, SC, SP, BM>), grid, dim3(256), 0, st, d, a->n_rows_dev, rows, a->W, a->Kp, a->n_out[0], e, \
                            a->W_split_t, a->W_split_t_plane, ts)
+#define LAUNCH_DXW(GM, SC, SP) do { if (wg.bm == 32) LAUNCH_DXW_BM(GM, SC, SP, 32); else LAUNCH_DXW_BM(GM, SC, SP, 64); } while (0)
         if (a->epilogue == 1 && a->dz.gmode == 0) { if (sp) LAUNCH_DXW(0, 1, true); else LAUNCH_DXW(0, 1, false); }
         else if (a->dz.gmode == 0) { if (sp) LAUNCH_DXW(0, 0, true); else LAUNCH_DXW(0, 0, false); }
         else { if (sp) LAUNCH_DXW(1, 0, true); else LAUNCH_DXW(1, 0, false); }
 #undef LAUNCH_DXW
+#undef LAUNCH_DXW_BM
         if (sp) GAD_CHECK_LAUNCH("gemm_dx(wide split)"); else GAD_CHECK_LAUNCH("gemm_dx(wide)");
         return GAD_OK;
     }
diff --git a/ga-ddpg_amd/csrc/gemm_fwd.hip b/ga-ddpg_amd/csrc/gemm_fwd.hip
--- a/ga-ddpg_amd/csrc/gemm_fwd.hip
+++ b/ga-ddpg_amd/csrc/gemm_fwd.hip
@@ -153,7 +153,7 @@
                                               stat_sq + (size_t)rep * stat_stride + ooff);
     }
 }
-template <int XM, bool POOL, bool SP = false>
+template <int XM, bool POOL, bool SP = false, int BM_ = 64>
 __global__ __launch_bounds__(256, 2) void gemm_fwd_wide_kernel(XSrc x, const int32_t* __restrict__ n_rows_dev, int n_rows_static,
                                                                const float* __restrict__ row_w, const float* __restrict__ W,
                                                                int Kp, int n_out, float* __restrict__ zout, int zout_pitch,
@@ -163,16 +163,18 @@
     KTimer kt_(ts);
     GAD_WPH_DECL;
     GAD_WKL_DECL;
-    constexpr int BM = 64, BN = 128, P = KT + 4, STAGE = SP ? spw::STAGE / 4 : (BM + BN) * P, VM = 512;
+    constexpr int BM = BM_, AR = 64, NT = BM / 32, BN = 128, P = KT + 4, STAGE = SP ? spw::STAGE / 4 : (AR + BN) * P, VM = 512;
+    static_assert(BM == 64 || BM == 32, "row tiles of 64 (2 x 2 wavefronts) or 32 (1 x 4)");
     static_assert(2 * STAGE >= 64 * 129, "the pooled epilogue's tile lives in the operand buffers");
-    __shared__ __attribute__((aligned(16))) float smem[2 * STAGE + 2 * VM + BM + 4 * BM];
+    __shared__ __attribute__((aligned(16))) float smem[2 * STAGE + 2 * VM + AR + 4 * AR];
     float* sv = smem + 2 * STAGE;
     float* tv = sv + VM;
     float* wS = tv + VM;
-    float* dxS = wS + BM;
+    float* dxS = wS + AR;
     const int tid = threadIdx.x, lane = tid & 63;
     const int wave = __builtin_amdgcn_readfirstlane(tid >> 6);
-    const int wm = wave >> 1, wn = wave & 1;
+    const int wm = BM == 64 ? wave >> 1 : 0, wn = BM == 64 ? wave & 1 : wave;
+    const int wc = wn * (NT * 32);
     const int l31 = lane & 31, half = lane >> 5;
     const int n0 = blockIdx.y * BN;
     const int n_rows = n_rows_dev ? min(*n_rows_dev, n_rows_static) : n_rows_static;
@@ -206,12 +208,12 @@
         }
     }
 
-    float csum[2] = {0.f, 0.f}, csq[2] = {0.f, 0.f};
+    float csum[NT] = {}, csq[NT] = {};
     for (int row0 = blockIdx.x * BM; row0 < n_rows; row0 += gridDim.x * BM) {
-        f32x16 acc[2];
-        f32x16 an[2];
-#pragma unroll
-        for (int t = 0; t < 2; ++t)
+        f32x16 acc[NT];
+        f32x16 an[NT];
+#pragma unroll
+        for (int t = 0; t < NT; ++t)
 #pragma unroll
             for (int v = 0; v < 16; ++v) { acc[t][v] = 0.f; if (SP) an[t][v] = 0.f; }
         int pgl = -1, pg_before = -1, pg_after = -1;
@@ -227,12 +229,13 @@
         const int ra0 = min(row0 + ur, max(n_rows - 1, 0)), ra1 = min(row0 + ur + 32, max(n_rows - 1, 0));
         const int va0 = ((XM == 0 ? ra0 * x.zin_pitch : x.row_pt[ra0] * x.feat_c) + c4) * 4;
         const int va1 = ((XM == 0 ? ra1 * x.zin_pitch : x.row_pt[ra1] * x.feat_c) + c4) * 4;
-        float4 ra2[2][2], rb2[2][SP ? 1 : 4];
+        float4 ra2[2][NT], rb2[2][SP ? 1 : 4];
         spw::BRegs rbs[SP ? 2 : 1];
         auto load_regs = [&](int kt, auto setc) {
             constexpr int S = decltype(setc)::value;
             const int k0 = kt * (KT * 4);
-            ra2[S][0] = buf_ld4(ar_, va0, k0); ra2[S][1] = buf_ld4(ar_, va1, k0);
+            ra2[S][0] = buf_ld4(ar_, va0, k0);
+            if (NT == 2) ra2[S][NT - 1] = buf_ld4(ar_, va1, k0);
             if (SP) { spw::load_b(rbs[SP ? S : 0], ws_, vbs, wsp_plane * 2, kt); return; }
 #pragma unroll
             for (int u = 0; u < (SP ? 1 : 4); ++u) rb2[S][u] = buf_ld4(wr_, vb[u], k0);
@@ -242,14 +245,14 @@
             const float4* ra = ra2[S];
             const float4* rb = rb2[S];
             float* As = smem + (kt & 1) * STAGE;
-            float* Bs = As + BM * P;
+            float* Bs = As + AR * P;
             float4 s4 = make_float4(1.f, 1.f, 1.f, 1.f), t4 = f4zero();
             if (XM == 0) {
                 s4 = *reinterpret_cast<const float4*>(sv + kt * KT + c4);
                 t4 = *reinterpret_cast<const float4*>(tv + kt * KT + c4);
             }
 #pragma unroll
-            for (int u = 0; u < 2; ++u) {
+            for (int u = 0; u < NT; ++u) {
                 float4 v = ra[u];
                 if (XM == 0) {
                     v.x = fmaxf(fmaf(v.x, s4.x, t4.x), 0.f); v.y = fmaxf(fmaf(v.y, s4.y, t4.y), 0.f);
@@ -289,7 +292,7 @@
         auto ktile = [&](int kt, auto nxtc) {
             if (SP) {
                 GAD_WKL(0);
-                spw::ktile(smem_b + (kt & 1) * spw::STAGE, (wm * 32 + l31) * 64, (wn * 64 + l31) * 64, sp_fo, acc, an);
+                spw::ktile<NT>(smem_b + (kt & 1) * spw::STAGE, (wm * 32 + l31) * 64, (wc + l31) * 64, sp_fo, acc, an);
                 GAD_WKL(1);
                 if (kt + 1 < nk) write_lds(kt + 1, nxtc);
                 if (kt + 3 < nk) load_regs(kt + 3, nxtc);
@@ -299,26 +302,32 @@
                 return;
             }
             const float* As = smem + (kt & 1) * STAGE + (wm * 32 + l31) * P + 4 * half;
-            const float* Bs = smem + (kt & 1) * STAGE + BM * P + (wn * 64 + l31) * P + 4 * half;
+            const float* Bs = smem + (kt & 1) * STAGE + AR * P + (wc + l31) * P + 4 * half;
             float4 a4 = *reinterpret_cast<const float4*>(As);
-            float4 b0 = *reinterpret_cast<const float4*>(Bs), b1 = *reinterpret_cast<const float4*>(Bs + 32 * P);
+            float4 b4[NT];
+#pragma unroll
+            for (int t = 0; t < NT; ++t) b4[t] = *reinterpret_cast<const float4*>(Bs + t * 32 * P);
 #pragma unroll
             for (int j = 0; j < KT / 8; ++j) {
-                float4 an = a4, bn0 = b0, bn1 = b1;
+                float4 an4 = a4, bn4[NT];
+#pragma unroll
+                for (int t = 0; t < NT; ++t) bn4[t] = b4[t];
                 if (j + 1 < KT / 8) {
-                    an = *reinterpret_cast<const float4*>(As + 8 * (j + 1));
-                    bn0 = *reinterpret_cast<const float4*>(Bs + 8 * (j + 1));
-                    bn1 = *reinterpret_cast<const float4*>(Bs + 32 * P + 8 * (j + 1));
+                    an4 = *reinterpret_cast<const float4*>(As + 8 * (j + 1));
+#pragma unroll
+                    for (int t = 0; t < NT; ++t) bn4[t] = *reinterpret_cast<const float4*>(Bs + t * 32 * P + 8 * (j + 1));
                 }
-                acc[0] = __builtin_amdgcn_mfma_f32_32x32x2f32(a4.x, b0.x, acc[0], 0, 0, 0);
-                acc[1] = __builtin_amdgcn_mfma_f32_32x32x2f32(a4.x, b1.x, acc[1], 0, 0, 0);
-                acc[0] = __builtin_amdgcn_mfma_f32_32x32x2f32(a4.y, b0.y, acc[0], 0, 0, 0);
-                acc[1] = __builtin_amdgcn_mfma_f32_32x32x2f32(a4.y, b1.y, acc[1], 0, 0, 0);
-                acc[0] = __builtin_amdgcn_mfma_f32_32x32x2f32(a4.z, b0.z, acc[0], 0, 0, 0);
-                acc[1] = __builtin_amdgcn_mfma_f32_32x32x2f32(a4.z, b1.z, acc[1], 0, 0, 0);
-                acc[0] = __builtin_amdgcn_mfma_f32_32x32x2f32(a4.w, b0.w, acc[0], 0, 0, 0);
-                acc[1] = __builtin_amdgcn_mfma_f32_32x32x2f32(a4.w, b1.w, acc[1], 0, 0, 0);
-                a4 = an; b0 = bn0; b1 = bn1;
+#pragma unroll
+                for (int t = 0; t < NT; ++t) acc[t] = __builtin_amdgcn_mfma_f32_32x32x2f32(a4.x, b4[t].x, acc[t], 0, 0, 0);
+#pragma unroll
+                for (int t = 0; t < NT; ++t) acc[t] = __builtin_amdgcn_mfma_f32_32x32x2f32(a4.y, b4[t].y, acc[t], 0, 0, 0);
+#pragma unroll
+                for (int t = 0; t < NT; ++t) acc[t] = __builtin_amdgcn_mfma_f32_32x32x2f32(a4.z, b4[t].z, acc[t], 0, 0, 0);
+#pragma unroll
+                for (int t = 0; t < NT; ++t) acc[t] = __builtin_amdgcn_mfma_f32_32x32x2f32(a4.w, b4[t].w, acc[t], 0, 0, 0);
+                a4 = an4;
+#pragma unroll
+                for (int t = 0; t < NT; ++t) b4[t] = bn4[t];
             }
             if (kt + 1 < nk) write_lds(kt + 1, nxtc);
             if (kt + 3 < nk) load_regs(kt + 3, nxtc);
@@ -331,14 +340,14 @@
         GAD_WPH(3);
         if (SP) {
 #pragma unroll
-            for (int t = 0; t < 2; ++t)
+            for (int t = 0; t < NT; ++t)
 #pragma unroll
                 for (int v = 0; v < 16; ++v) acc[t][v] = (v & 1) ? an[t][v] - acc[t][v] : acc[t][v] - an[t][v];
         }
         if (XM == 1) {
 #pragma unroll
-            for (int t = 0; t < 2; ++t) {
-                const float* wx = W + (size_t)(n0 + wn * 64 + t * 32 + l31) * Kp + x.feat_c;
+            for (int t = 0; t < NT; ++t) {
+                const float* wx = W + (size_t)(n0 + wc + t * 32 + l31) * Kp + x.feat_c;
                 const float w0 = wx[0], w1 = wx[1], w2 = wx[2];
 #pragma unroll
                 for (int v = 0; v < 16; ++v) {
@@ -350,17 +359,17 @@
         if (POOL) {
             float* zt = smem;
 #pragma unroll
-            for (int t = 0; t < 2; ++t)
-#pragma unroll
-                for (int v = 0; v < 16; ++v) zt[(wm * 32 + acc_row(v, half)) * 129 + wn * 64 + t * 32 + l31] = acc[t][v];
+            for (int t = 0; t < NT; ++t)
+#pragma unroll
+                for (int v = 0; v < 16; ++v) zt[(wm * 32 + acc_row(v, half)) * 129 + wc + t * 32 + l31] = acc[t][v];
             __syncthreads();
             const int gb = __builtin_amdgcn_readfirstlane(pg_before), ga = __builtin_amdgcn_readfirstlane(pg_after);
-            pool_tile64<2>(zt + lane, 129, 64, pgl, row0, min(64, n_rows - row0), psgn, wave, 4, gb, ga, pe.key + n0 + lane, pe.C);
+            pool_tile64<2>(zt + lane, 129, 64, pgl, row0, min(BM, n_rows - row0), psgn, wave, 4, gb, ga, pe.key + n0 + lane, pe.C);
         }
         if (SP) {
 #pragma unroll
-        for (int t = 0; t < 2; ++t) {
-            const int n = n0 + wn * 64 + t * 32 + l31;
+        for (int t = 0; t < NT; ++t) {
+            const int n = n0 + wc + t * 32 + l31;
             const int vzo = (4 * half * zout_pitch + n) * 4;
 #pragma unroll
             for (int v = 0; v < 16; ++v)
@@ -368,7 +377,7 @@
         }
         __builtin_amdgcn_sched_barrier(0);
 #pragma unroll
-        for (int t = 0; t < 2; ++t) {
+        for (int t = 0; t < NT; ++t) {
             float s1 = 0.f, s2 = 0.f;
 #pragma unroll
             for (int v = 0; v < 16; ++v) {
@@ -382,8 +391,8 @@
         }
         } else {
 #pragma unroll
-        for (int t = 0; t < 2; ++t) {
-            const int n = n0 + wn * 64 + t * 32 + l31;
+        for (int t = 0; t < NT; ++t) {
+            const int n = n0 + wc + t * 32 + l31;
             const int vzo = (4 * half * zout_pitch + n) * 4;
             float s1 = 0.f, s2 = 0.f;
 #pragma unroll
@@ -403,8 +412,8 @@
     }
     if (stat_sum) {
         const int rep = blockIdx.x % GAD_STAT_REPLICAS;
-        block_column_atomics<2, 2, 2>(smem, csum, csq, lane, wm, wn, n0, n_out, stat_sum + (size_t)rep * stat_stride,
-                                      stat_sq + (size_t)rep * stat_stride);
+        block_column_atomics<BM / 32, 4 / (BM / 32), NT>(smem, csum, csq, lane, wm, wn, n0, n_out, stat_sum + (size_t)rep * stat_stride,
+                                                         stat_sq + (size_t)rep * stat_stride);
     }
 #ifdef GAD_W_PHASES
     __asm__ volatile("s_waitcnt vmcnt(0)" ::: "memory");
@@ -1037,18 +1046,20 @@
         return GAD_OK;
     }
     if (fwd_wideable(*a)) {
-        int gx = gad_cdiv(grid_rows, 64); if (gx > GAD_GX_CAP) gx = GAD_GX_CAP;
-        const dim3 grid(gx, a->n_out[0] / 128);
+        const WideGrid wg = wide_grid(grid_rows, a->n_out[0] / 128);
+        const dim3 grid(wg.gx, a->n_out[0] / 128);
         const bool sp = split_on(GAD_SPLIT_FWD_WIDE) && a->W_split && a->W_split_pitch == (a->mode == 1 ? a->feat_c : a->Kp) &&
                         a->W_split_plane >= a->n_out[0] * a->W_split_pitch;
-#define LAUNCH_WIDE(XM, POOL, SP)                                                                                              \
-        hipLaunchKernelGGL((gemm_fwd_wide_kernel<XM, POOL, SP>), grid, dim3(256), 0, st, x, a->n_rows_dev, rows, a->row_w, a->W, a->Kp, \
+#define LAUNCH_WIDE_BM(XM, POOL, SP, BM)                                                                                       \
+        hipLaunchKernelGGL((gemm_fwd_wide_kernel<XM, POOL, SP, BM>), grid, dim3(256), 0, st, x, a->n_rows_dev, rows, a->row_w, a->W, a->Kp, \
                            a->n_out[0], a->zout, a->zout_pitch, a->stat_sum, a->stat_sq, a->stat_stride, pe, a->W_split, a->W_split_pitch, \
                            a->W_split_plane, ts)
+#define LAUNCH_WIDE(XM, POOL, SP) do { if (wg.bm == 32) LAUNCH_WIDE_BM(XM, POOL, SP, 32); else LAUNCH_WIDE_BM(XM, POOL, SP, 64); } while (0)
         if (a->mode == 1) { if (sp) LAUNCH_WIDE(1, false, true); else LAUNCH_WIDE(1, false, false); }
         else if (pe.key) { if (sp) LAUNCH_WIDE(0, true, true); else LAUNCH_WIDE(0, true, false); }
         else { if (sp) LAUNCH_WIDE(0, false, true); else LAUNCH_WIDE(0, false, false); }
 #undef LAUNCH_WIDE
+#undef LAUNCH_WIDE_BM
         if (sp) GAD_CHECK_LAUNCH("gemm_fwd(wide split)"); else GAD_CHECK_LAUNCH("gemm_fwd(wide)");
         return GAD_OK;
     }
diff --git a/ga-ddpg_amd/hip.py b/ga-ddpg_amd/hip.py
--- a/ga-ddpg_amd/hip.py
+++ b/ga-ddpg_amd/hip.py
@@ -258,7 +258,7 @@
 
 
 OPTION_DEFAULTS = {"mfma_split": 1, "deterministic": 0, "tnn_grid": 1}
-LIBRARY_DEFAULTS = {"fps_cfg": 0}
+LIBRARY_DEFAULTS = {"fps_cfg": 0, "wide_bm": 0}
 
 
 def get_option_default(name):
```

Measured after the change: 386.8. -3.1%, worse.
